# src-d/kmcuda

Measured on AMD Instinct MI355X. Metric: point-assignments/sec per Lloyd iter (8Mx256@1024), higher is better.
Workload: dtype f32

## Files before the change

kmcuda_amd/csrc/engine.cpp:

```cpp
#include "engine.hpp"

#include <math.h>
#include <stdio.h>
#include <stdlib.h>
#include <string.h>

#include <mutex>
#include <vector>

#include "../../include/kmcuda_amd.h"

namespace kmx {

int g_verbosity = 0;

namespace {
std::mutex g_stream_pool_mutex;
std::vector<std::vector<hipStream_t>> g_stream_pool;
}

hipStream_t pooled_stream_acquire(int device) {
  {
    std::lock_guard<std::mutex> lock(g_stream_pool_mutex);
    if ((size_t)device < g_stream_pool.size() && !g_stream_pool[device].empty()) {
// ... 8 lines not shown
}
void pooled_stream_release(int device, hipStream_t s) {
  if (!s) return;
  if (hipStreamSynchronize(s) != hipSuccess) {
    (void)hipGetLastError();
    (void)hipStreamDestroy(s);
    return;
  }
  std::lock_guard<std::mutex> lock(g_stream_pool_mutex);
  if (g_stream_pool.size() <= (size_t)device) g_stream_pool.resize(device + 1);
  if (g_stream_pool[device].size() < 32) g_stream_pool[device].push_back(s);
  else (void)hipStreamDestroy(s);
}

void *Engine::alloc_bytes(size_t bytes) {
  const size_t rounded = (bytes + 255u) & ~(size_t)255u;
  if (rounded <= kSlabMaxItem) {
    if (slab_used_ + rounded > kSlabBytes) {
      void *q = nullptr;
      if (hipMalloc(&q, kSlabBytes) != hipSuccess) return nullptr;
      owned_.push_back(q);
      slab_ = static_cast<char *>(q);
      slab_used_ = 0;
    }
    void *r = slab_ + slab_used_;
    slab_used_ += rounded;
    return r;
  }
  void *q = nullptr;
  if (hipMalloc(&q, bytes) != hipSuccess) return nullptr;
  owned_.push_back(q);
  return q;
}

uint32_t *Engine::pinned_words(size_t n, uint32_t **dev_addr) {
  if (!pinned_) {
    if (hipHostMalloc(reinterpret_cast<void **>(&pinned_), kPinnedWords * sizeof(uint32_t), hipHostMallocCoherent) != hipSuccess) {
      pinned_ = nullptr;
      return nullptr;
    }
    memset(pinned_, 0, kPinnedWords * sizeof(uint32_t));
    void *dp = nullptr;
    if (hipHostGetDevicePointer(&dp, pinned_, 0) != hipSuccess || dp == nullptr) {
      (void)hipHostFree(pinned_);
      pinned_ = nullptr;
      pinned_dev_ = nullptr;
      return nullptr;
    }
    pinned_dev_ = static_cast<uint32_t *>(dp);
  }
  n = (n + 3u) & ~(size_t)3u;
  if (pinned_used_ + n > kPinnedWords) return nullptr;
  uint32_t *r = pinned_ + pinned_used_;
  if (dev_addr) *dev_addr = pinned_dev_ + pinned_used_;
  pinned_used_ += n;
  return r;
}

Engine::~Engine() {
  if (device_ >= 0) (void)hipSetDevice(device_);
  for (auto &s : spans_) { (void)hipEventDestroy(s.a); (void)hipEventDestroy(s.b); }
  for (void *p : owned_) (void)hipFree(p);
  if (pinned_) (void)hipHostFree(pinned_);
  if (side_stream_ && own_side_stream_) pooled_stream_release(device_, side_stream_);
  if (ev_fork_) (void)hipEventDestroy(ev_fork_);
  if (ev_join_) (void)hipEventDestroy(ev_join_);
  for (hipEvent_t e : ev_report_)
    if (e) (void)hipEventDestroy(e);
  if (ev_rows_) (void)hipEventDestroy(ev_rows_);
  if (own_stream_ && stream_) {
    if (blocking_stream_) (void)hipStreamDestroy(stream_);
    else pooled_stream_release(device_, stream_);
  }
}

int Engine::init(int device, uint32_t n_rows, uint32_t D, uint32_t K, int metric, int fp16x2, hipStream_t stream) {
  if (getenv("KMCUDA_AMD_DEBUG")) g_verbosity = atoi(getenv("KMCUDA_AMD_DEBUG"));
  if (const char *f = getenv("KMCUDA_AMD_FILTER")) filter_mode_ = strcmp(f, "f32") == 0 ? 1 : 0;
  if (const char *c = getenv("KMCUDA_AMD_ROW_CACHE")) row_cache_allowed_ = atoi(c) != 0;
  carry_pairs_ = true;
  if (const char *c = getenv("KMCUDA_AMD_CARRY_PAIRS")) carry_pairs_ = atoi(c) != 0;
  if (const char *c = getenv("KMCUDA_AMD_SETTLE")) settle_ = atoi(c) != 0;
  if (const char *c = getenv("KMCUDA_AMD_DUO")) { duo_on_ = atoi(c) != 0; duo_always_ = atoi(c) == 2; }
  if (const char *c = getenv("KMCUDA_AMD_COARSE_MFMA")) coarse_mfma_ = atoi(c) == 32 ? 32u : 16u;
  if (const char *c = getenv("KMCUDA_AMD_WIDE")) wide_ok_ = atoi(c) != 0;
  if (const char *c = getenv("KMCUDA_AMD_GEMM")) wide_ok_ = atoi(c) != 0;
  if (const char *u = getenv("KMCUDA_AMD_UPDATE"))
    ms_.force = strcmp(u, "radix") == 0 ? 1 : (strcmp(u, "sync") == 0 ? 2 : (strcmp(u, "bucket") == 0 ? 3 : 0));
  if (D == 0 || K < 1 || K >= 0x7FFFFFFFu) return kInvalidArguments;
  if (fp16x2) return kInvalidArguments;
  int ndev = 0;
  if (hipGetDeviceCount(&ndev) != hipSuccess || device < 0 || device >= ndev) return kNoSuchDevice;
  KMX_HIP(hipSetDevice(device), kNoSuchDevice);
  device_ = device;
  if (stream == (hipStream_t)(intptr_t)-1) {
    KMX_HIP(hipStreamCreateWithFlags(&stream_, hipStreamDefault), kRuntimeError);
    own_stream_ = true;
    blocking_stream_ = true;
  } else if (stream) {
    stream_ = stream;
  } else {
    stream_ = pooled_stream_acquire(device);
    if (!stream_) return kRuntimeError;
    own_stream_ = true;
  }
  N_ = n_rows; D_ = D; K_ = K; metric_ = metric; fp16x2_ = fp16x2;
  K_pad_ = (K + 31) / 32 * 32;
  Kt_ = (K + 63) / 64 * 64;
  DP_ = lloyd_dp_for(D);
  long wide_min_d = 257;
  if (const char *c = getenv("KMCUDA_AMD_WIDE_MIN_D")) {
    const long d = atol(c);
    if (d > 0) wide_min_d = d;
  }
  if (wide_ok_ && (long)D >= wide_min_d) DP_ = 0;
  eps_ = (float)(1.02 * ((double)D + 12.0) * ldexp(1.0, -24));
  tie_slack_ = metric == 0 ? 0.f : 1e-6f;

  wide_dp_ = (DP_ == 0 && wide_ok_) ? (D + 63) / 64 * 64 : 0;
  const uint32_t dp = DP_ ? DP_ : (wide_dp_ ? wide_dp_ : 8);
  int rc;
  if ((rc = alloc(&csqr_, K))) return rc;
  if ((rc = alloc(&bias_, K_pad_))) return rc;
  if ((rc = alloc(&bias2_, K_pad_))) return rc;
  if ((rc = alloc(&cfil_, (size_t)K_pad_ * dp))) return rc;
  if ((rc = alloc(&ct_, (size_t)D * Kt_))) return rc;
  if ((rc = alloc(&stats_base_, 16))) return rc;
  stats_ = stats_base_;
  if ((rc = alloc(&mu_, dp))) return rc;
  if ((rc = alloc(&finite_, Kt_))) return rc;
  if ((rc = alloc(&flagged_, n_rows))) return rc;
  if ((rc = alloc(&pairs_, 3 * (size_t)n_rows))) return rc;
  if ((rc = alloc(&counters_, 16))) return rc;
  if ((rc = alloc(&keys_tmp_, 2 * (size_t)n_rows))) return rc;
  if ((rc = alloc(&vals_tmp_, 2 * (size_t)n_rows))) return rc;
  if ((rc = alloc(&keys_sorted_, 2 * (size_t)n_rows))) return rc;
  if ((rc = alloc(&rows_sorted_, 2 * (size_t)n_rows))) return rc;
  if ((rc = alloc(&offsets2_, 2 * (size_t)K + 2))) return rc;
  if ((rc = alloc(&move_blocks_, (size_t)n_rows / 1024 + 4))) return rc;
  if ((rc = alloc(&bucket_work_, move_bucket_words(K)))) return rc;
  KMX_HIP(hipMemsetAsync(bucket_work_, 0, move_bucket_words(K) * sizeof(uint32_t), stream_), kRuntimeError);
  bucket_cap_ = move_bucket_cap(n_rows, K);
  if ((rc = alloc(&bucket_rows_, 2 * (size_t)K * bucket_cap_))) return rc;
  KMX_HIP(hipMemsetAsync(stats_base_, 0, 16 * sizeof(uint32_t), stream_), kRuntimeError);
  host_move_count_ = pinned_words(5, &ms_.host_dev);
  if (!host_move_count_) return kMemoryAllocationFailure;
  host_move_count_[2] = 0xFFFFFFFFu;
  host_move_count_[4] = 0xFFFFFFFFu;
  ms_.host = host_move_count_;
  KMX_HIP(hipEventCreateWithFlags(&ev_rows_, hipEventDisableTiming), kRuntimeError);
  sort_temp_bytes_ = sort_temp_bytes(2 * (size_t)n_rows, 2 * K);
  {
    const size_t b2 = sort_temp_bytes(n_rows, K);
    if (b2 > sort_temp_bytes_) sort_temp_bytes_ = b2;
  }
  {
    char *t = nullptr;
    if ((rc = alloc(&t, sort_temp_bytes_ + 16))) return rc;
    sort_temp_ = t;
  }
  host_counters_ = pinned_words(8, nullptr);
  if (!host_counters_) return kMemoryAllocationFailure;
  KMX_HIP(hipMemsetAsync(counters_, 0, 16 * sizeof(uint32_t), stream_), kRuntimeError);
  return kSuccess;
}

// ... 96 lines not shown
  KMX_HIP(hipMemcpy(gfirst_, gfirst.data(), gfirst.size() * sizeof(uint32_t), hipMemcpyHostToDevice), kMemoryCopyError);
  KMX_HIP(hipMemcpy(gsecond_, gsecond.data(), gsecond.size() * sizeof(uint32_t), hipMemcpyHostToDevice), kMemoryCopyError);
  const uint32_t k_pad64 = (K_ + 63u) / 64u * 64u;
  if ((rc = alloc(&groups_, k_pad64))) return rc;
  if (!yy_stats_) {
    if ((rc = alloc(&yy_stats_, 64 * 16))) return rc;
    KMX_HIP(hipMemsetAsync(yy_stats_, 0, 64 * 16 * sizeof(uint32_t), stream_), kRuntimeError);
  }
  if ((rc = alloc(&cperm_, cperm.size()))) return rc;
  if ((rc = alloc(&gstart_, G + 1))) return rc;
  if ((rc = alloc(&pids_, pids.size()))) return rc;
  if ((rc = alloc(&pmeta_, pmeta.size()))) return rc;
  const uint32_t dp = DP_ ? DP_ : 8;
  if ((rc = alloc(&pfil_, (size_t)nslots_ * dp))) return rc;
  if ((rc = alloc(&pbias_, nslots_))) return rc;
  {
    std::vector<uint32_t> gp(k_pad64, 0xFFFFFFFFu);
    for (uint32_t c = 0; c < K_; c++) gp[c] = groups_host[c];
    KMX_HIP(hipMemcpy(groups_, gp.data(), k_pad64 * sizeof(uint32_t), hipMemcpyHostToDevice), kMemoryCopyError);
  }
  KMX_HIP(hipMemcpy(cperm_, cperm.data(), cperm.size() * sizeof(uint32_t), hipMemcpyHostToDevice), kMemoryCopyError);
  KMX_HIP(hipMemcpy(gstart_, gstart.data(), (G + 1) * sizeof(uint32_t), hipMemcpyHostToDevice), kMemoryCopyError);
  KMX_HIP(hipMemcpy(pids_, pids.data(), pids.size() * sizeof(uint32_t), hipMemcpyHostToDevice), kMemoryCopyError);
  KMX_HIP(hipMemcpy(pmeta_, pmeta.data(), pmeta.size() * sizeof(uint32_t), hipMemcpyHostToDevice), kMemoryCopyError);
  return kSuccess;
}

static void fill_yy_args(Engine &e, YyArgs &a, const float *samples, const float *centroids) {
  a.samples = samples; a.centroids = centroids;
  a.len = e.N_; a.D = e.D_; a.DP = e.DP_; a.K = e.K_; a.K_pad = e.K_pad_; a.G = e.G_;
  a.cfil = e.cfil_; a.bias = e.bias_; a.mu = e.mu_; a.stats = e.stats_; a.eps = e.eps_;
  a.groups = e.groups_; a.drifts = nullptr; a.gdrifts = nullptr; a.assignments = nullptr; a.bounds = nullptr;
  a.passed = nullptr; a.counters = e.counters_; a.count_ptr = e.counters_ + 2;
  a.panelhi = nullptr; a.hint = nullptr; a.flag_rows = nullptr; a.gfirst = e.gfirst_; a.gsecond = e.gsecond_;
  a.xcache = nullptr; a.xmeta = nullptr; a.stat_stripes = e.yy_stats_;
  a.pfil = e.pfil_; a.pbias = e.pbias_; a.pids = e.pids_; a.pmeta = e.pmeta_; a.cperm = e.cperm_;
  a.gstart = e.gstart_; a.nslots = e.nslots_;
}

int Engine::yy_init(const float *samples, const float *centroids, const uint32_t *assignments, float *bounds) {
  KMX_HIP(hipSetDevice(device_), kNoSuchDevice);
  if (N_ == 0) return kSuccess;
  if (strict_h2_) {
    KMX_HIP(launch_h2_yy_init(metric_, samples, N_, D_, K_, G_, centroids, assignments, groups_, bounds, stream_),
            kRuntimeError);
    return kSuccess;
  }
  if (DP_ && DP_ <= 256 && !yy_exact_) {
    int rc = prepare_centroids(centroids);
    if (rc) return rc;
    YyArgs a;
    fill_yy_args(*this, a, samples, centroids);
    a.assignments = const_cast<uint32_t *>(assignments);
    a.bounds = bounds;
    KMX_HIP(launch_yy_orig_panel(metric_, centroids, D_, DP_, pids_, nslots_, pfil_, pbias_, stream_), kRuntimeError);
    KMX_HIP(launch_yy_init_lds(metric_, a, stream_), kRuntimeError);
    return kSuccess;
  }
  if (!xt_) {
    int rc = alloc(&xt_, (size_t)N_ * D_);
    if (rc) return rc;
  }
  KMX_HIP(launch_transpose(samples, N_, D_, xt_, stream_), kRuntimeError);
  KMX_HIP(launch_yy_init(metric_, xt_, N_, D_, G_, centroids, assignments, cperm_, gstart_, bounds, stream_),
          kRuntimeError);
  return kSuccess;
}

int Engine::yy_drifts(const float *centroids, float *drifts, float *gdrifts) {
  KMX_HIP(hipSetDevice(device_), kNoSuchDevice);
  if (strict_h2_) {
    KMX_HIP(launch_h2_yy_drifts(metric_, centroids, K_, D_, drifts, stream_), kRuntimeError);
    KMX_HIP(launch_yy_group_max(K_, D_, G_, groups_, drifts, gdrifts, stream_), kRuntimeError);
    return kSuccess;
  }
  KMX_HIP(launch_yy_drifts(metric_, centroids, K_, D_, G_, groups_, drifts, gdrifts, stream_), kRuntimeError);
  return kSuccess;
}

int Engine::yy_filters(const float *samples, const float *centroids, const float *drifts, const float *gdrifts,
                       uint32_t *assignments, uint32_t *assignments_prev, float *bounds, uint32_t *passed) {
  KMX_HIP(hipSetDevice(device_), kNoSuchDevice);
  carry_valid_ = false;
  if (N_ == 0) return kSuccess;
  if (strict_h2_) {
    KMX_HIP(launch_h2_yy_global(metric_, samples, N_, D_, K_, G_, centroids, drifts, gdrifts, assignments,
                                assignments_prev, bounds, passed, counters_, stream_),
            kRuntimeError);
    KMX_HIP(launch_h2_yy_local(metric_, samples, N_, D_, K_, G_, passed, centroids, groups_, drifts, gdrifts,
                               assignments, bounds, counters_, stream_),
            kRuntimeError);
    return kSuccess;
  }
  KMX_HIP(launch_yy_global_filter(metric_, samples, N_, D_, K_, G_, centroids, drifts, gdrifts, assignments,
                                  assignments_prev, bounds, passed, counters_, stream_),
          kRuntimeError);
  if (DP_ && DP_ <= 256 && !yy_exact_) {
    int rc = prepare_centroids(centroids);
    if (rc) return rc;
    YyArgs a;
    fill_yy_args(*this, a, samples, centroids);
    a.drifts = drifts; a.gdrifts = gdrifts; a.assignments = assignments; a.bounds = bounds; a.passed = passed;
    if (yy_hint_ && yy_hint_supported(DP_)) {
      if (!yy_hint_buf_) {
        uint16_t *phi = nullptr;
        if ((rc = alloc(&phi, (size_t)((K_pad_ + 63u) / 64u * 64u) * (DP_ + 2)))) return rc;
        if ((rc = alloc(&yy_flag_rows_, N_))) return rc;
        if ((rc = alloc(&yy_hint_buf_, N_))) return rc;
        yy_panelhi_ = phi;
      }
      KMX_HIP(launch_centroid_panelhi(centroids, K_, D_, K_pad_, DP_, finite_, mu_, bias_, yy_panelhi_, stats_,
                                      stream_),
              kRuntimeError);
      KMX_HIP(hipMemsetAsync(counters_ + 5, 0, sizeof(uint32_t), stream_), kRuntimeError);
      a.panelhi = yy_panelhi_; a.hint = yy_hint_buf_; a.flag_rows = yy_flag_rows_;
      if (row_cache_on_ && row_cache_valid_ && mu_frozen_ && xcache_ && metric_ == 0 && D_ == DP_) {
        a.xcache = xcache_;
        a.xmeta = xmeta_;
      }
      KMX_HIP(launch_yy_hint(metric_, a, stream_), kRuntimeError);
      KMX_HIP(launch_yy_local_hint(metric_, a, stream_), kRuntimeError);
      a.passed = yy_flag_rows_;
      a.count_ptr = counters_ + 5;
    }
    KMX_HIP(launch_yy_local_mfma(metric_, a, stream_), kRuntimeError);
    return kSuccess;
  }
  KMX_HIP(launch_yy_local_filter(metric_, samples, N_, D_, K_, G_, centroids, groups_, drifts, gdrifts, assignments,
                                 bounds, passed, counters_, stream_),
          kRuntimeError);
  return kSuccess;
}

int Engine::lloyd_assign(const float *samples, const float *centroids, uint32_t *assignments,
                         uint32_t *assignments_prev, bool exact_only) {
  KMX_HIP(hipSetDevice(device_), kNoSuchDevice);
  const bool carry_was_valid = carry_valid_;
  carry_valid_ = false;
  if (strict_h2_) {
    if (!h2_sq_) {
      int rc = alloc(&h2_sq_, 2 * (size_t)K_);
      if (rc) return rc;
    }
    span_begin(1);
    KMX_HIP(launch_h2_csqr(metric_, centroids, K_, D_, h2_sq_, stream_), kRuntimeError);
    KMX_HIP(launch_h2_assign(metric_, samples, N_, D_, centroids, K_, h2_sq_, assignments, assignments_prev, counters_,
                             stream_),
            kRuntimeError);
    span_end();
    return kSuccess;
  }
  const bool two_stage = !exact_only && DP_ != 0 && filter_mode_ == 0 && lloyd_filter_f16_supported(D_, DP_);
  const bool want_cache = row_cache_on_ && two_stage && N_ != 0;
  const bool build_cache = want_cache && !row_cache_valid_;
  if (build_cache) mu_frozen_ = false;
  if (!side_stream_) {
    side_stream_ = pooled_stream_acquire(device_);
    if (!side_stream_) return kRuntimeError;
    own_side_stream_ = true;
  }
  if (!ev_fork_) {
    KMX_HIP(hipEventCreateWithFlags(&ev_fork_, hipEventDisableTiming), kRuntimeError);
    KMX_HIP(hipEventCreateWithFlags(&ev_join_, hipEventDisableTiming), kRuntimeError);
  }
  if (two_stage && !panelhi_) {
    uint16_t *phi = nullptr;
    int rc = alloc(&phi, (size_t)((K_pad_ + 63u) / 64u * 64u) * (DP_ + 2));
    if (rc) return rc;
    if (!undecided_ && ((rc = alloc(&undecided_, N_)) || (rc = alloc(&und_thr_, N_)))) return rc;
    if (duo_on_ && !duo_ && alloc(&duo_, 4 * (size_t)N_) != kSuccess) {
      (void)hipGetLastError();
      duo_ = nullptr;
      duo_on_ = false;
    }
    panelhi_ = phi;
  }
  const bool steady = steady_state(exact_only);
  const bool wide_sel = !exact_only && DP_ == 0 && wide_dp_ != 0 && !wide_failed_;
  const bool wide_steady = wide_sel && mu_frozen_ && row_cache_on_ && row_cache_valid_ && N_ != 0 && panelhi_ != nullptr &&
                           wide_rows16_ != nullptr && !strict_h2_;
  const bool prepared = steady && prepared_for_ == centroids;
  prepared_for_ = nullptr;
  bool rows_on_side = false;
  if (steady || wide_steady) {
    KMX_HIP(hipEventRecord(ev_fork_, stream_), kRuntimeError);
    KMX_HIP(hipStreamWaitEvent(side_stream_, ev_fork_, 0), kRuntimeError);
    KMX_HIP(launch_centroid_rows(metric_, centroids, K_, D_, Kt_, csqr_, ct_, side_stream_), kRuntimeError);
    KMX_HIP(hipEventRecord(ev_rows_, side_stream_), kRuntimeError);
    rows_on_side = true;
    if (!prepared) {
      uint32_t *next = stats_;
      stats_ = stats_ == stats_base_ ? stats_base_ + 8 : stats_base_;
      KMX_HIP(launch_centroid_prep_frozen(metric_, centroids, K_, D_, K_pad_, DP_ ? DP_ : wide_dp_, mu_, finite_, bias_,
                                          bias2_, cfil_, panelhi_, stats_, next, counters_ + 1, counters_ + 3, counters_ + 4,
                                          carry_on_ ? drift_ : nullptr, carry_on_ && drift_ ? counters_ + kCarryCursor : nullptr,
                                          stream_),
              kRuntimeError);
      carry_preps_++;
    }
  } else {
    int rc = prepare_centroids(centroids);
    if (rc) return rc;
  }
  LloydArgs a;
  a.samples = samples; a.N = N_; a.D = D_; a.K = K_; a.K_pad = K_pad_; a.DP = DP_; a.Kt = Kt_;
  a.cfil = cfil_; a.bias = bias_; a.mu = mu_; a.ct = ct_; a.csqr = csqr_; a.stats = stats_;
  a.eps = eps_; a.tie_slack = tie_slack_;
  a.assignments = assignments; a.assignments_prev = assignments_prev;
  a.flagged = flagged_; a.pairs = pairs_; a.counters = counters_;
  a.coarse_mfma = coarse_mfma_;
  if (N_ == 0) return kSuccess;
  if (wide_sel) {
    const int rc = lloyd_assign_wide(a, centroids, wide_steady, rows_on_side, carry_was_valid);
    if (rc != kNoSuchDevice + 100) return rc;
  }
  if (exact_only || DP_ == 0 || (DP_ > 256 && filter_mode_ != 0)) {
    span_begin(1);
    const uint32_t grid = N_ < 8192u ? N_ : 8192u;
    KMX_HIP(launch_lloyd_exact(metric_, a, nullptr, nullptr, grid, stream_), kRuntimeError);
    span_end();
    return kSuccess;
  }
  span_begin(0);
  if (two_stage) {
    const void *rows = half_rows_ ? half_rows_ : (const void *)samples;
    const bool half = half_rows_ != nullptr;
    bool duo_listed = false;
    if (!steady)
      KMX_HIP(launch_centroid_panelhi(centroids, K_, D_, K_pad_, DP_, finite_, mu_, bias_, panelhi_, stats_, stream_),
              kRuntimeError);
    if (build_cache) {
      const size_t npad = ((size_t)N_ + 255) / 256 * 256;
      if (!xcache_) {
        uint16_t *xc = nullptr;
        float *xm = nullptr;
        if (alloc(&xc, npad * DP_) == kSuccess && alloc(&xm, npad * 3 + 2) == kSuccess) {
          xcache_ = xc;
          xmeta_ = xm;
        } else {
          (void)hipGetLastError();
          row_cache_on_ = false;
        }
      }
      if (xcache_) {
        KMX_HIP(launch_row_cache(rows, half, N_, D_, DP_, mu_, xcache_, xmeta_, stream_), kRuntimeError);
        row_cache_valid_ = true;
        mu_frozen_ = true;
      }
    }
    const bool cached = row_cache_on_ && row_cache_valid_;
    bool carry = carry_on_ && steady && cached;
    if (carry && carry_policy_.paused()) {
      carry = false;
      if (getenv("KMCUDA_AMD_CARRY_TRACE")) fprintf(stderr, "[carry] paused (%u more)\n", carry_policy_.pause);
    }
    if (carry && !ub_) {
      const bool pairs = carry_pairs_;
      if (alloc(&ub_, N_) != kSuccess || alloc(&lb_, N_) != kSuccess ||
          alloc(&drift_, 2 * (size_t)K_) != kSuccess ||
          (pairs && (alloc(&l3_, N_) != kSuccess || alloc(&p1_, N_) != kSuccess || alloc(&p2_, N_) != kSuccess)) ||
          alloc(&carry_list_, N_) != kSuccess || !(host_carry_ = pinned_words(2, &host_carry_dev_))) {
        (void)hipGetLastError();
        carry_on_ = false;
        ub_ = nullptr;
        l3_ = nullptr;
      } else {
        host_carry_[0] = 0xFFFFFFFFu;
        host_carry_[1] = 0;
        if (const char *v = getenv("KMCUDA_AMD_CARRY_MAX")) carry_policy_.list_max = (float)atof(v);
      }
    }
    span_begin(3);
    duo_listed = duo_on_ && duo_;
    if (duo_listed && !duo_always_) {
      const uint32_t und_prev = host_move_count_[2], duo_prev = host_move_count_[4];
      const uint64_t listed_rows = (und_prev != 0xFFFFFFFFu && duo_prev != 0xFFFFFFFFu) ? (uint64_t)und_prev + duo_prev
                                                                                          : (uint64_t)N_ / 16u;
      duo_listed = listed_rows > 512u * 128u;
    }
    CarryArgs cy_refine;
    if (carry && carry_on_) {
      CarryArgs cy;
      cy.ub = ub_; cy.lb = lb_; cy.host_report = host_carry_dev_; cy.seq = ++carry_seq_;
      cy.angular = metric_ != 0;
      cy.l3 = l3_; cy.p1 = p1_; cy.p2 = p2_;
      cy_refine = cy;
      const bool moved = carry_was_valid && carry_preps_ == 1;
      uint32_t hint = 0xFFFFFFFFu;
      bool listed = false;
      if (moved) {
        const uint32_t last = host_carry_[0], last_seq = host_carry_[1];
        listed = carry_policy_.decide(last, last_seq, carry_seq_, N_);
        if (listed) hint = last;
        KMX_HIP(launch_carry_skip(N_, K_, assignments, assignments_prev, cy, xmeta_, drift_, stats_, tie_slack_,
                                  carry_list_, finite_, pairs_, counters_, !listed, stream_),
                kRuntimeError);
        cy.n_list = counters_ + kCarryCursor;
      }
      if (listed) cy.row_list = carry_list_;
      static const bool trace = getenv("KMCUDA_AMD_CARRY_TRACE") != nullptr;
      if (trace) {
        uint32_t w[8] = {0};
        (void)hipStreamSynchronize(stream_);
        (void)hipMemcpy(w, stats_, sizeof(w), hipMemcpyDeviceToHost);
        float f[8];
        memcpy(f, w, sizeof(f));
        fprintf(stderr, "[carry] stats: max ||c'||^2 %g, max |bias| %g, max ||c||^2 %g, max residual^2 %g, max drift %g, max bias change %g; "
                "stage 2 took %u rows of an earlier pass\n", f[0], f[1], f[2], f[5], f[6], f[7], host_move_count_[2]);
      }
      if (trace)
        fprintf(stderr, "[carry] pass %u: bounds %s, %u preparation(s) since, last reported list %u (pass %u), %s\n",
                carry_seq_, carry_was_valid ? "valid" : "void", carry_preps_, host_carry_[0], host_carry_[1],
                listed ? "listed pass" : (moved ? "whole pass, list counted" : "whole pass"));
      KMX_HIP(launch_lloyd_coarse_carry(a, rows, half, xcache_, xmeta_, panelhi_, undecided_, und_thr_, cy, hint,
                                        duo_listed ? duo_ : nullptr, stream_),
              kRuntimeError);
      carry_valid_ = true;
    } else {
      KMX_HIP(launch_lloyd_coarse(a, rows, half, cached ? xcache_ : nullptr, xmeta_, panelhi_, undecided_, und_thr_,
                                  duo_listed ? duo_ : nullptr, stream_),
              kRuntimeError);
    }
    if (duo_listed) {
      KMX_HIP(hipEventRecord(ev_fork_, stream_), kRuntimeError);
      KMX_HIP(hipStreamWaitEvent(side_stream_, ev_fork_, 0), kRuntimeError);
      KMX_HIP(launch_lloyd_duo(a, duo_, side_stream_, cy_refine.l3 ? &cy_refine : nullptr), kRuntimeError);
      KMX_HIP(hipEventRecord(ev_join_, side_stream_), kRuntimeError);
    }
    carry_preps_ = 0;
    span_end();
    last_undecided_ = host_move_count_[2];
    if (cy_refine.l3) {
      KMX_HIP(launch_lloyd_refine_carry(a, rows, half, panelhi_, undecided_, und_thr_, counters_ + 4, last_undecided_,
                                        cy_refine, stream_),
              kRuntimeError);
    } else {
      KMX_HIP(launch_lloyd_refine(a, rows, half, panelhi_, undecided_, und_thr_, counters_ + 4, last_undecided_,
                                  stream_),
              kRuntimeError);
    }
    if (duo_listed) KMX_HIP(hipStreamWaitEvent(stream_, ev_join_, 0), kRuntimeError);
  } else {
    KMX_HIP(launch_lloyd_filter(a, stream_), kRuntimeError);
  }
  span_end();
  span_begin(1);
  if (settle_ && lloyd_settle_supported(a, centroids)) {
    if (rows_on_side) KMX_HIP(hipStreamWaitEvent(stream_, ev_rows_, 0), kRuntimeError);
    KMX_HIP(launch_lloyd_settle(metric_, a, centroids, stream_), kRuntimeError);
    span_end();
    return kSuccess;
  }
  KMX_HIP(hipEventRecord(ev_fork_, stream_), kRuntimeError);
  KMX_HIP(hipStreamWaitEvent(side_stream_, ev_fork_, 0), kRuntimeError);
  const uint32_t grid = N_ < 4096u ? N_ : 4096u;
  KMX_HIP(launch_lloyd_exact(metric_, a, flagged_, counters_ + 1, grid, side_stream_), kRuntimeError);
  KMX_HIP(hipEventRecord(ev_join_, side_stream_), kRuntimeError);
  if (rows_on_side) KMX_HIP(hipStreamWaitEvent(stream_, ev_rows_, 0), kRuntimeError);
  KMX_HIP(launch_lloyd_pair(metric_, a, centroids, (N_ + 127) / 128 < 2048u ? (N_ + 127) / 128 : 2048u, stream_),
          kRuntimeError);
  KMX_HIP(hipStreamWaitEvent(stream_, ev_join_, 0), kRuntimeError);
  span_end();
  return kSuccess;
}

int Engine::lloyd_assign_wide(const LloydArgs &a0, const float *centroids, bool steady, bool rows_on_side,
                              bool carry_was_valid) {
  constexpr int kNoFilter = kNoSuchDevice + 100;
  LloydArgs a = a0;
  const uint32_t DG = wide_dp_;
  const uint32_t k_pad64 = (K_pad_ + 63u) / 64u * 64u;
  auto no_memory = [&]() {
    (void)hipGetLastError();
    if (g_verbosity > 0) printf("rows wider than 256 features: no memory for the streamed filter's buffers -- exact kernels\n");
    wide_failed_ = true;
    return kNoFilter;
  };
  if (!panelhi_) {
    uint16_t *phi = nullptr;
    if (alloc(&phi, (size_t)k_pad64 * (DG + 2))) return no_memory();
    panelhi_ = phi;
  }
  if (!wide_cont_) {
    if ((!undecided_ && (alloc(&undecided_, N_) || alloc(&und_thr_, N_))) || alloc(&wide_cont_, wide_cont_words(N_))) {
      wide_cont_ = nullptr;
      return no_memory();
    }
  }
  if (!wide_rows16_) {
    uint16_t *xg = nullptr;
    if (alloc(&xg, (size_t)N_ * DG) || alloc(&wide_meta_, ((size_t)N_ + 1) * 4)) return no_memory();
    wide_rows16_ = xg;
  }
  span_begin(0);
  if (!steady)
    KMX_HIP(launch_centroid_panelhi(centroids, K_, D_, K_pad_, DG, finite_, mu_, bias_, panelhi_, stats_, stream_),
            kRuntimeError);
  if (!(row_cache_on_ && row_cache_valid_)) {
    const void *rows = half_rows_ ? half_rows_ : (const void *)a.samples;
    KMX_HIP(launch_row_halves(rows, half_rows_ != nullptr, N_, D_, DG, mu_, wide_rows16_, wide_meta_, stream_), kRuntimeError);
    if (row_cache_on_) {
      row_cache_valid_ = true;
      mu_frozen_ = true;
    }
  }
  bool carry = carry_on_ && steady && DG <= 4096u;
  if (carry && carry_policy_.paused()) {
    carry = false;
    if (getenv("KMCUDA_AMD_CARRY_TRACE")) fprintf(stderr, "[carry] paused (%u more)\n", carry_policy_.pause);
  }
  if (carry && !ub_) {
    if (alloc(&ub_, N_) != kSuccess || alloc(&lb_, N_) != kSuccess || alloc(&drift_, 2 * (size_t)K_) != kSuccess ||
        alloc(&carry_list_, N_) != kSuccess || !(host_carry_ = pinned_words(2, &host_carry_dev_))) {
      (void)hipGetLastError();
      carry_on_ = false;
      ub_ = nullptr;
    } else {
      host_carry_[0] = 0xFFFFFFFFu;
      host_carry_[1] = 0;
      if (const char *v = getenv("KMCUDA_AMD_CARRY_MAX")) carry_policy_.list_max = (float)atof(v);
    }
  }
  span_begin(3);
  if (carry && carry_on_) {
    CarryArgs cy;
    cy.ub = ub_; cy.lb = lb_; cy.host_report = host_carry_dev_; cy.seq = ++carry_seq_;
    cy.angular = metric_ != 0;
    const bool moved = carry_was_valid && carry_preps_ == 1;
    bool listed = false;
    if (moved) {
      const uint32_t last = host_carry_[0], last_seq = host_carry_[1];
      listed = carry_policy_.decide(last, last_seq, carry_seq_, N_);
      KMX_HIP(launch_carry_skip(N_, K_, a.assignments, a.assignments_prev, cy, wide_meta_, drift_, stats_, tie_slack_,
                                carry_list_, finite_, pairs_, counters_, !listed, stream_, DG),
              kRuntimeError);
      cy.n_list = counters_ + kCarryCursor;
    }
    if (listed) cy.row_list = carry_list_;
    if (getenv("KMCUDA_AMD_CARRY_TRACE"))
      fprintf(stderr, "[carry] streamed pass %u: bounds %s, %u preparation(s) since, last reported list %u (pass %u), %s\n",
              carry_seq_, carry_was_valid ? "valid" : "void", carry_preps_, host_carry_[0], host_carry_[1],
              listed ? "listed pass" : (moved ? "whole pass, list counted" : "whole pass"));
    KMX_HIP(launch_lloyd_wide(a, wide_rows16_, wide_meta_, DG, panelhi_, undecided_, und_thr_, wide_cont_, stream_, &cy),
            kRuntimeError);
    carry_valid_ = true;
  } else {
    KMX_HIP(launch_lloyd_wide(a, wide_rows16_, wide_meta_, DG, panelhi_, undecided_, und_thr_, wide_cont_, stream_), kRuntimeError);
  }
  carry_preps_ = 0;
  span_end();
  if (rows_on_side) KMX_HIP(hipStreamWaitEvent(stream_, ev_rows_, 0), kRuntimeError);
  KMX_HIP(launch_wide_contenders(metric_, a, centroids, DG, undecided_, wide_cont_, stream_), kRuntimeError);
  span_end();
  span_begin(1);
  if (settle_ && lloyd_settle_supported(a, centroids)) {
    KMX_HIP(launch_lloyd_settle(metric_, a, centroids, stream_), kRuntimeError);
  } else {
    KMX_HIP(launch_lloyd_pair(metric_, a, centroids, (N_ + 127) / 128 < 2048u ? (N_ + 127) / 128 : 2048u, stream_),
            kRuntimeError);
    const uint32_t grid = N_ < 4096u ? N_ : 4096u;
    KMX_HIP(launch_lloyd_exact(metric_, a, flagged_, counters_ + 1, grid, stream_), kRuntimeError);
  }
  span_end();
  return kSuccess;
}

int Engine::move_deltas(const float *samples, const uint32_t *prev, const uint32_t *cur, double *delta,
                        int32_t *dcount, double *tail) {
  KMX_HIP(hipSetDevice(device_), kNoSuchDevice);
  span_begin(2);
  const MoveWeights mw{weights_, tail ? tail + K_ + 4 : wtail_, win_};
  KMX_HIP(launch_move_deltas(samples, N_, D_, K_, prev, cur, keys_tmp_, vals_tmp_, keys_sorted_, rows_sorted_,
                             offsets2_, sort_temp_, sort_temp_bytes_, bucket_rows_, bucket_cap_, delta, dcount, tail,
                             counters_, move_blocks_, bucket_work_, &ms_, stream_, weights_ ? &mw : nullptr),
          kRuntimeError);
  span_end();
  return kSuccess;
}

int Engine::apply_delta(const double *delta, const int32_t *dcount, const double *dcount_d, float *centroids,
                        uint32_t *ccounts, float stop_threshold, bool report, uint32_t seq) {
  KMX_HIP(hipSetDevice(device_), kNoSuchDevice);
  prepared_for_ = nullptr;
  StopCtl ctl;
  if (stop_threshold >= 0.f || report) {
    if (!dcount_d) return kInvalidArguments;
    int rc = stop_ctl(stop_threshold, report, seq, &ctl);
    if (rc) return rc;
  }
  span_begin(2);
  const double *wtail = weights_ ? (dcount_d ? dcount_d + K_ + 4 : wtail_) : nullptr;
  KMX_HIP(launch_apply_delta(metric_, delta, dcount, dcount_d, K_, D_, centroids, ccounts, ctl, stream_, wtail, cweights_),
          kRuntimeError);
  span_end();
  if (report) KMX_HIP(hipEventRecord(ev_report_[seq & 1u], stream_), kRuntimeError);
  return kSuccess;
}

int Engine::stop_ctl(float stop_threshold, bool report, uint32_t seq, StopCtl *ctl) {
  ctl->threshold = stop_threshold;
  ctl->counters = counters_;
  ctl->seq = seq;
  if (report) {
    if (!host_report_) {
      host_report_ = pinned_words(16, &host_report_dev_);
      if (!host_report_) return kMemoryAllocationFailure;
      memset(host_report_, 0xFF, 16 * sizeof(uint32_t));
      for (hipEvent_t &e : ev_report_) KMX_HIP(hipEventCreateWithFlags(&e, hipEventDisableTiming), kRuntimeError);
    }
    ctl->host_tail = host_report_dev_ + 8 * (seq & 1u);
  }
  return kSuccess;
}

int Engine::stop_report(uint32_t seq, uint32_t *host_out6) {
  KMX_HIP(hipSetDevice(device_), kNoSuchDevice);
  if (!host_report_) return kInvalidArguments;
  KMX_HIP(hipEventSynchronize(ev_report_[seq & 1u]), kRuntimeError);
  const volatile uint32_t *t = host_report_ + 8 * (seq & 1u);
  for (int i = 0; i < 6; i++) host_out6[i] = t[i];
  return host_out6[5] == seq ? kSuccess : kRuntimeError;
}

bool Engine::steady_state(bool exact_only) const {
  const bool two_stage = !exact_only && DP_ != 0 && filter_mode_ == 0 && lloyd_filter_f16_supported(D_, DP_) && !strict_h2_;
  return two_stage && mu_frozen_ && row_cache_on_ && row_cache_valid_ && N_ != 0 && panelhi_ != nullptr;
}

int Engine::apply_prepare(const double *delta, const double *dcount_d, float *centroids, uint32_t *ccounts,
                          float stop_threshold, bool report, uint32_t seq) {
  if (!(metric_ == 0 && steady_state(false) && dcount_d) || weights_) {
    prepared_for_ = nullptr;
    return apply_delta(delta, nullptr, dcount_d, centroids, ccounts, stop_threshold, report, seq);
  }
  KMX_HIP(hipSetDevice(device_), kNoSuchDevice);
  StopCtl ctl;
  if (stop_threshold >= 0.f || report) {
    int rc = stop_ctl(stop_threshold, report, seq, &ctl);
    if (rc) return rc;
  }
  uint32_t *next = stats_;
  stats_ = stats_ == stats_base_ ? stats_base_ + 8 : stats_base_;
  span_begin(2);
  KMX_HIP(launch_apply_prep_frozen(delta, dcount_d, centroids, ccounts, ctl, K_, D_, K_pad_, DP_, mu_, finite_, bias_,
                                   bias2_, cfil_, panelhi_, stats_, next, counters_ + 1, counters_ + 3, counters_ + 4,
                                   carry_on_ ? drift_ : nullptr, carry_on_ && drift_ ? counters_ + kCarryCursor : nullptr,
                                   stream_),
          kRuntimeError);
  carry_preps_++;
  span_end();
  if (report) KMX_HIP(hipEventRecord(ev_report_[seq & 1u], stream_), kRuntimeError);
  prepared_for_ = centroids;
  return kSuccess;
}

int Engine::carry_stats(unsigned long long *rows_spared, uint32_t *last_list) {
  KMX_HIP(hipSetDevice(device_), kNoSuchDevice);
// ... 317 lines not shown
```

kmcuda_amd/csrc/engine.hpp:

```cpp
#pragma once
#include <hip/hip_runtime.h>
#include <stdint.h>

#include <vector>

#include "kernels.hpp"

namespace kmx {

enum Result {
  kSuccess = 0, kInvalidArguments, kNoSuchDevice, kMemoryAllocationFailure, kRuntimeError, kMemoryCopyError
};

#define KMX_HIP(call, ret)                                                                   \
  do {                                                                                       \
    hipError_t e__ = (call);                                                                 \
    if (e__ != hipSuccess) {                                                                 \
      if (kmx::g_verbosity > 0)                                                              \
        printf("%s:%d -> %s (%s)\n", __FILE__, __LINE__, hipGetErrorString(e__), #call);     \
      return ret;                                                                            \
    }                                                                                        \
  } while (0)

extern int g_verbosity;
// ... 38 lines not shown
        hopeless = 0;
        backoff = 4;
        episode_list = 0;
      }
    }
    return listed;
  }
};

class Engine {
 public:
  Engine() = default;
  ~Engine();
  Engine(const Engine &) = delete;
  Engine &operator=(const Engine &) = delete;

  int init(int device, uint32_t n_rows, uint32_t D, uint32_t K, int metric, int fp16x2, hipStream_t stream);

  int lloyd_assign(const float *samples, const float *centroids, uint32_t *assignments,
                   uint32_t *assignments_prev, bool exact_only);
  int move_deltas(const float *samples, const uint32_t *prev, const uint32_t *cur, double *delta, int32_t *dcount,
                  double *tail);
  int apply_delta(const double *delta, const int32_t *dcount, const double *dcount_d, float *centroids,
                  uint32_t *ccounts, float stop_threshold = -1.f, bool report = false, uint32_t seq = 0);
  int apply_prepare(const double *delta, const double *dcount_d, float *centroids, uint32_t *ccounts,
                    float stop_threshold = -1.f, bool report = false, uint32_t seq = 0);
  int set_weights(const float *weights);
  const float *weights_ = nullptr;
  double weight_total_ = 0.0;
  double *cweights_ = nullptr;
  double *wtail_ = nullptr;
  double *win_ = nullptr;
  double *wcheck_ = nullptr;
  size_t reduce_len() const { return (size_t)K_ * D_ + K_ + 4 + (weights_ ? (size_t)K_ + 1 : 0); }
  bool steady_state(bool exact_only) const;
  int stop_ctl(float stop_threshold, bool report, uint32_t seq, StopCtl *ctl);
  const float *prepared_for_ = nullptr;
  int stop_clear();
  int stop_report(uint32_t seq, uint32_t *host_out6);
  int adjust_exact(const float *samples, const uint32_t *prev, const uint32_t *cur, float *centroids,
                   uint32_t *ccounts);
  int prepare_centroids(const float *centroids);
  int yy_configure(uint32_t G, const uint32_t *groups_host);
  int yy_init(const float *samples, const float *centroids, const uint32_t *assignments, float *bounds);
  int yy_drifts(const float *centroids, float *drifts, float *gdrifts);
  int yy_filters(const float *samples, const float *centroids, const float *drifts, const float *gdrifts,
                 uint32_t *assignments, uint32_t *assignments_prev, float *bounds, uint32_t *passed);
  int counters_read(uint32_t *host4);
  int counters_reset(int which);
  int sync();

  template <typename T>
  int alloc(T **p, size_t count) {
    void *q = alloc_bytes(count ? count * sizeof(T) : sizeof(T));
    if (!q) return kMemoryAllocationFailure;
    *p = static_cast<T *>(q);
    return kSuccess;
  }
  void *alloc_bytes(size_t bytes);
  uint32_t *pinned_words(size_t n, uint32_t **dev_addr);

  int device_ = -1;
  hipStream_t stream_ = nullptr;
  bool own_stream_ = false, blocking_stream_ = false;
  hipStream_t side_stream_ = nullptr;
  bool own_side_stream_ = false;
  hipEvent_t ev_fork_ = nullptr, ev_join_ = nullptr;
  hipEvent_t ev_rows_ = nullptr;
  uint32_t N_ = 0, D_ = 0, K_ = 0, K_pad_ = 0, Kt_ = 0, DP_ = 0;
  int metric_ = 0, fp16x2_ = 0;
  bool strict_h2_ = false;
  float *h2_sq_ = nullptr;
  float eps_ = 0, tie_slack_ = 0;

  float *csqr_ = nullptr, *bias_ = nullptr, *bias2_ = nullptr, *cfil_ = nullptr, *ct_ = nullptr, *mu_ = nullptr;
  uint32_t *finite_ = nullptr;
  const void *half_rows_ = nullptr;
  void *panelhi_ = nullptr;
  uint32_t *undecided_ = nullptr;
  float *und_thr_ = nullptr;
  uint32_t *duo_ = nullptr;
  bool duo_on_ = true;
  bool duo_always_ = false;
  uint32_t coarse_mfma_ = 16;
  int filter_mode_ = 0;
  bool settle_ = true;
  uint32_t wide_dp_ = 0;
  bool wide_ok_ = true;
  bool wide_failed_ = false;
  void *wide_rows16_ = nullptr;
  float *wide_meta_ = nullptr;
  uint32_t *wide_cont_ = nullptr;
  int lloyd_assign_wide(const LloydArgs &a, const float *centroids, bool steady, bool rows_on_side, bool carry_was_valid);
  bool row_cache_allowed_ = true;
  bool row_cache_on_ = false, row_cache_valid_ = false, mu_frozen_ = false;
  void *xcache_ = nullptr;
  float *xmeta_ = nullptr;
  bool carry_on_ = false;
  bool carry_valid_ = false;
  uint32_t carry_preps_ = 0;
  uint32_t carry_seq_ = 0;
  CarryPolicy carry_policy_;
  float *ub_ = nullptr, *lb_ = nullptr, *drift_ = nullptr;
  bool carry_pairs_ = true;
  float *l3_ = nullptr;
  uint32_t *p1_ = nullptr, *p2_ = nullptr;
  uint32_t *carry_list_ = nullptr;
  uint32_t *host_carry_ = nullptr, *host_carry_dev_ = nullptr;
  bool carry_usable() const;
  int carry_stats(unsigned long long *rows_spared, uint32_t *last_list);
  int carry_pair_stats(unsigned long long *rows_paired);
  int duo_rows(uint32_t *rows);
  uint32_t *stats_base_ = nullptr, *stats_ = nullptr, *flagged_ = nullptr, *pairs_ = nullptr, *counters_ = nullptr;
  uint32_t *keys_tmp_ = nullptr, *vals_tmp_ = nullptr, *keys_sorted_ = nullptr, *rows_sorted_ = nullptr,
           *offsets2_ = nullptr, *move_blocks_ = nullptr, *bucket_work_ = nullptr, *bucket_rows_ = nullptr;
  uint32_t bucket_cap_ = 0;
  uint32_t last_undecided_ = 0xFFFFFFFFu;
  MoveState ms_;
  uint32_t *host_move_count_ = nullptr;
  void *sort_temp_ = nullptr;
  size_t sort_temp_bytes_ = 0;
  uint32_t G_ = 0, nslots_ = 0;
  bool yy_exact_ = false;
  bool yy_hint_ = true;
  uint32_t *gfirst_ = nullptr, *gsecond_ = nullptr, *yy_flag_rows_ = nullptr;
  float *yy_hint_buf_ = nullptr;
  void *yy_panelhi_ = nullptr;
  int yy_hint_stats(uint32_t *host6);
  uint32_t *groups_ = nullptr, *cperm_ = nullptr, *gstart_ = nullptr, *pids_ = nullptr, *pmeta_ = nullptr;
  float *pfil_ = nullptr, *pbias_ = nullptr, *xt_ = nullptr;
  float *exact_work_ = nullptr;
  uint32_t *host_counters_ = nullptr;
  uint32_t *host_report_ = nullptr;
  uint32_t *host_report_dev_ = nullptr;
  hipEvent_t ev_report_[2] = {nullptr, nullptr};
  uint32_t *yy_stats_ = nullptr;

  bool profile_ = false;
  double filter_ms_ = 0, exact_ms_ = 0, update_ms_ = 0, coarse_ms_ = 0;
  uint32_t filter_launches_ = 0;
  struct Span { hipEvent_t a, b; int kind; };
  std::vector<Span> spans_;
  std::vector<size_t> open_spans_;
  void span_begin(int kind);
  void span_end();
  void profile_collect();
  void profile_reset();

 private:
  std::vector<void *> owned_;
  static constexpr size_t kSlabBytes = 4u << 20, kSlabMaxItem = 512u << 10;
  char *slab_ = nullptr;
  size_t slab_used_ = kSlabBytes;
  static constexpr size_t kPinnedWords = 64;
  uint32_t *pinned_ = nullptr, *pinned_dev_ = nullptr;
  size_t pinned_used_ = 0;
};

}
```

kmcuda_amd/csrc/filter_common.hpp:

```cpp
#pragma once
#include <hip/hip_runtime.h>
#include <stdint.h>

namespace kmx {

__device__ __forceinline__ bool commit_row(uint32_t s, uint32_t nearest, uint32_t *__restrict__ assignments,
                                           uint32_t *__restrict__ assignments_prev) {
  const uint32_t old = assignments[s];
  assignments_prev[s] = old;
  if (old != nearest) {
    assignments[s] = nearest;
    return true;
  }
  return false;
}


struct ClampLimits {
  float hi, lo;
};
__device__ __forceinline__ ClampLimits clamp_limits(bool angular, float xm, float exm, float ehalf) {
  ClampLimits l;
  if (!angular) {
    l.hi = INFINITY;
    l.lo = -INFINITY;
    return l;
  }
  const float m = (ehalf + exm) * 1.001f + 2.0e-6f + 3.0e-7f * fabsf(xm);
  l.hi = (1.0f - m) - xm;
  l.lo = (m - 1.0f) - xm;
  return l;
}
__device__ __forceinline__ float dot_error(int n, float mass) { return 6.1e-8f * (float)(n + 8) * mass; }

template <typename T>
__device__ __forceinline__ void row_dot_mu(const T *__restrict__ xr, const float *__restrict__ mu, uint32_t f0,
                                           uint32_t f1, float &dot, float &mass) {
  float d = 0.f, m = 0.f;
#pragma unroll 4
  for (uint32_t f = f0; f < f1; f++) {
    const float x = (float)xr[f], u = mu[f];
    d = fmaf(x, u, d);
    m = fmaf(fabsf(x), fabsf(u), m);
  }
  dot = d;
  mass = m;
}

__device__ __forceinline__ void filter_finish(float v1, float v2, float v3, uint32_t c1, uint32_t c2, int h, int lane,
                                              uint32_t s, uint32_t N, uint32_t K, bool insane, float thr,
                                              ClampLimits lim, uint32_t *__restrict__ assignments,
                                              uint32_t *__restrict__ assignments_prev,
                                              uint32_t *__restrict__ flagged, uint32_t *__restrict__ pairs,
                                              uint32_t *__restrict__ counters) {
  auto decode = [&](uint32_t code, int half) -> uint32_t {
    if (code == 0xFFFFFFFFu) return 0xFFFFFFFFu;
    const uint32_t r = code & 15u;
    return (code >> 4) * 32u + (r & 3u) + 8u * (r >> 2) + 4u * half;
  };
  uint32_t i1 = decode(c1, h), i2 = decode(c2, h);
  {
    const float pv1 = __shfl_xor(v1, 32), pv2 = __shfl_xor(v2, 32), pv3 = __shfl_xor(v3, 32);
    const uint32_t pi1 = __shfl_xor(i1, 32), pi2 = __shfl_xor(i2, 32);
    auto insert = [&](float v, uint32_t idx) {
      const bool g1 = v > v1, g2 = v > v2, g3 = v > v3;
      v3 = g2 ? v2 : (g3 ? v : v3);
      i2 = g1 ? i1 : (g2 ? idx : i2);
      v2 = g1 ? v1 : (g2 ? v : v2);
      i1 = g1 ? idx : i1;
      v1 = g1 ? v : v1;
    };
    insert(pv1, pi1);
    insert(pv2, pi2);
    insert(pv3, 0xFFFFFFFFu);
  }
  const bool certain = insane || (((v1 - v2) > thr) && (v2 < lim.hi) && (v1 > lim.lo));
  const bool two = !certain && ((v1 - v3) > thr) && (v3 < lim.hi) && (v1 > lim.lo) && i2 != 0xFFFFFFFFu;
  const bool mine = (h == 0) && (s < N);
  const bool commit_now = mine && certain;
  const bool pair_now = mine && two;
  const bool flag_now = mine && !certain && !two;
  bool changed = false;
  if (commit_now) changed = commit_row(s, insane ? K : i1, assignments, assignments_prev);
  const unsigned long long cm = __ballot(changed);
  const unsigned long long pm = __ballot(pair_now);
  const unsigned long long fm = __ballot(flag_now);
  if (lane == 0 && cm) atomicAdd(&counters[0], (uint32_t)__popcll(cm));
  if (pm) {
    uint32_t base = 0;
    if (lane == 0) base = atomicAdd(&counters[3], (uint32_t)__popcll(pm));
    base = __shfl(base, 0);
    if (pair_now) {
      const uint32_t slot = base + (uint32_t)__popcll(pm & ((1ull << lane) - 1ull));
      pairs[3 * (size_t)slot + 0] = s;
      pairs[3 * (size_t)slot + 1] = i1;
      pairs[3 * (size_t)slot + 2] = i2;
    }
  }
  if (fm) {
// ... 9 lines not shown
```

kmcuda_amd/csrc/kernels.hpp:

```cpp
#pragma once
#include <hip/hip_runtime.h>
#include <stdint.h>

namespace kmx {

struct LloydArgs {
  const float *samples;
  uint32_t N, D, K;
  uint32_t K_pad;
  uint32_t DP;
  uint32_t Kt;
  const float *cfil;
  const float *bias;
  const float *mu;
  const float *ct;
  const float *csqr;
  const uint32_t *stats;
  float eps;
  float tie_slack;
  uint32_t *assignments, *assignments_prev;
  uint32_t *flagged;
  uint32_t *pairs;
  uint32_t *counters;
  uint32_t coarse_mfma = 16;
};
constexpr uint32_t kWaveRowGridMax = 1u << 20;
inline uint32_t wave_row_grid(uint32_t n_rows) {
  const uint32_t g = (n_rows + 3u) / 4u;
  return g < kWaveRowGridMax ? (g ? g : 1u) : kWaveRowGridMax;
}
constexpr uint32_t kStopFlag = 8;
constexpr uint32_t kCarryCursor = 9, kCarrySkipped = 10;
constexpr uint32_t kCarryPaired = 12;
constexpr uint32_t kDuoCount = 14;
struct CarryArgs {
  float *ub = nullptr, *lb = nullptr;
  const uint32_t *row_list = nullptr;
  const uint32_t *n_list = nullptr;
  uint32_t *host_report = nullptr;
  uint32_t seq = 0;
  int angular = 0;
  float *l3 = nullptr;
  uint32_t *p1 = nullptr, *p2 = nullptr;
};
struct StopCtl {
  float threshold = -1.f;
  uint32_t *counters = nullptr;
  uint32_t *host_tail = nullptr;
  uint32_t seq = 0;
};

uint32_t filter_dp_for(uint32_t D);
uint32_t lloyd_dp_for(uint32_t D);
hipError_t launch_centroid_prep(int metric, const float *centroids, uint32_t K, uint32_t D, uint32_t K_pad,
                                uint32_t DP, uint32_t Kt, float *csqr, float *bias, float *bias2, float *cfil,
                                float *ct, float *mu, bool freeze_mu, uint32_t *finite, uint32_t *stats, uint32_t *zero_a,
                                uint32_t *zero_b, uint32_t *zero_c, hipStream_t st);
hipError_t launch_lloyd_filter(const LloydArgs &a, hipStream_t st);
hipError_t launch_lloyd_pair(int metric, const LloydArgs &a, const float *centroids, uint32_t grid, hipStream_t st);
hipError_t launch_lloyd_exact(int metric, const LloydArgs &a, const uint32_t *rows, const uint32_t *nrows,
                              uint32_t grid, hipStream_t st);
bool lloyd_settle_supported(const LloydArgs &a, const float *centroids);
hipError_t launch_lloyd_settle(int metric, const LloydArgs &a, const float *centroids, hipStream_t st);

bool lloyd_filter_f16_supported(uint32_t D, uint32_t DP);
hipError_t launch_centroid_panelhi(const float *centroids, uint32_t K, uint32_t D, uint32_t K_pad, uint32_t DP,
                                   const uint32_t *finite, const float *mu, const float *bias, void *panelhi,
                                   uint32_t *stats, hipStream_t st);
hipError_t launch_centroid_prep_frozen(int metric, const float *centroids, uint32_t K, uint32_t D, uint32_t K_pad,
                                       uint32_t DP, const float *mu, uint32_t *finite, float *bias, float *bias2,
                                       float *cfil, void *panelhi, uint32_t *stats, uint32_t *stats_next,
                                       uint32_t *zero_a, uint32_t *zero_b, uint32_t *zero_c,
                                       float *drift ,
                                       uint32_t *zero_d , hipStream_t st);
hipError_t launch_apply_prep_frozen(const double *delta, const double *dcount_d, float *centroids, uint32_t *ccounts,
                                    const StopCtl &stop, uint32_t K, uint32_t D, uint32_t K_pad, uint32_t DP,
                                    const float *mu, uint32_t *finite, float *bias, float *bias2, float *cfil,
                                    void *panelhi, uint32_t *stats, uint32_t *stats_next, uint32_t *zero_a,
                                    uint32_t *zero_b, uint32_t *zero_c, float *drift, uint32_t *zero_d, hipStream_t st);
hipError_t launch_lloyd_coarse_carry(const LloydArgs &a, const void *rows, bool half_rows, const void *xcache,
                                     const float *xmeta, const void *panelhi, uint32_t *undecided, float *und_thr,
                                     const CarryArgs &cy, uint32_t rows_hint, uint32_t *duo, hipStream_t st);
hipError_t launch_carry_skip(uint32_t N, uint32_t K, const uint32_t *assignments, uint32_t *assignments_prev,
                             const CarryArgs &cy, const float *xmeta, const float *drift, const uint32_t *stats,
                             float tie_slack, uint32_t *row_list, const uint32_t *finite, uint32_t *pairs,
                             uint32_t *counters, bool probe, hipStream_t st, uint32_t wide_dg = 0);
hipError_t launch_centroid_rows(int metric, const float *centroids, uint32_t K, uint32_t D, uint32_t Kt, float *csqr,
                                float *ct, hipStream_t st);
hipError_t launch_lloyd_coarse(const LloydArgs &a, const void *rows, bool half_rows, const void *xcache,
                               const float *xmeta, const void *panelhi, uint32_t *undecided, float *und_thr,
                               uint32_t *duo, hipStream_t st);
hipError_t launch_lloyd_duo(const LloydArgs &a, const uint32_t *duo, hipStream_t st, const CarryArgs *cy = nullptr);
hipError_t launch_lloyd_refine(const LloydArgs &a, const void *rows, bool half_rows, const void *panelhi,
                               const uint32_t *row_list, const float *thr_list, const uint32_t *n_list,
                               uint32_t rows_hint , hipStream_t st);
hipError_t launch_lloyd_refine_carry(const LloydArgs &a, const void *rows, bool half_rows, const void *panelhi,
                                     const uint32_t *row_list, const float *thr_list, const uint32_t *n_list,
                                     uint32_t rows_hint, const CarryArgs &cy, hipStream_t st);
hipError_t launch_row_cache(const void *rows, bool half_rows, uint32_t N, uint32_t D, uint32_t DP, const float *mu,
                            void *xcache, float *xmeta, hipStream_t st);

hipError_t launch_row_halves(const void *rows, bool half_rows, uint32_t N, uint32_t D, uint32_t DG, const float *mu,
                             void *xg, float *meta , hipStream_t st);
size_t wide_cont_words(uint32_t N);
hipError_t launch_lloyd_wide(const LloydArgs &a, const void *xg, const float *meta, uint32_t DG ,
                             const void *panelhi, uint32_t *undecided, float *und_thr, uint32_t *und_cont, hipStream_t st,
                             const CarryArgs *cy = nullptr);
hipError_t launch_wide_contenders(int metric, const LloydArgs &a, const float *centroids, uint32_t DG,
                                  const uint32_t *und_rows, const uint32_t *und_cont, hipStream_t st);

size_t sort_temp_bytes(size_t n, uint32_t max_key);
uint32_t move_bucket_stride(uint32_t K);
size_t move_bucket_words(uint32_t K);
uint32_t move_bucket_cap(uint32_t N, uint32_t K);
hipError_t launch_inverse_assignments(const uint32_t *assignments, uint32_t N, uint32_t K, uint32_t *keys_tmp,
                                      uint32_t *vals_tmp, uint32_t *keys_sorted, uint32_t *inv,
                                      uint32_t *offsets, void *temp, size_t temp_bytes, hipStream_t st);
struct MoveState {
  uint32_t *host = nullptr;
  uint32_t *host_dev = nullptr;
  uint32_t last_events = 0xFFFFFFFFu;
  int force = 0;
  uint32_t n_radix = 0, n_direct = 0;
};
struct MoveWeights {
  const float *weights;
  double *dweight;
  double *win;
};
hipError_t launch_move_deltas(const float *samples, uint32_t N, uint32_t D, uint32_t K, const uint32_t *prev,
                              const uint32_t *cur, uint32_t *keys_tmp, uint32_t *vals_tmp, uint32_t *keys_sorted,
                              uint32_t *rows_sorted, uint32_t *offsets2, void *temp, size_t temp_bytes,
                              uint32_t *bucket_rows, uint32_t cap, double *delta, int32_t *dcount ,
                              double *tail ,
                              const uint32_t *counters, uint32_t *blockoff, uint32_t *bucket_work, MoveState *ms,
                              hipStream_t st, const MoveWeights *mw = nullptr);
hipError_t launch_adjust_exact(int metric, const float *samples, uint32_t N, uint32_t D, uint32_t K,
                               const uint32_t *prev, const uint32_t *cur, uint32_t *keys_tmp, uint32_t *vals_tmp,
                               uint32_t *keys_sorted, uint32_t *rows_sorted, uint32_t *offsets2, void *temp,
                               size_t temp_bytes, float *work, float *centroids, uint32_t *ccounts, hipStream_t st);
hipError_t launch_apply_delta(int metric, const double *delta, const int32_t *dcount ,
                              const double *dcount_d , uint32_t K, uint32_t D,
                              float *centroids, uint32_t *ccounts, const StopCtl &stop, hipStream_t st,
                              const double *wtail = nullptr ,
                              double *cweights = nullptr );
size_t weights_check_doubles();
hipError_t launch_weights_check(const float *weights, uint32_t N, double *work, hipStream_t st);
hipError_t launch_sum_buffers(double *const *bufs_dev, uint32_t nbuf, size_t len, hipStream_t st);

hipError_t preload_update_code();
hipError_t preload_lloyd_f16_code();
hipError_t preload_lloyd_code();
hipError_t preload_lloyd_carry_code();
hipError_t preload_lloyd_duo_code();
hipError_t launch_gather_rows(const float *samples, const uint32_t *idx, uint32_t K, uint32_t D, float *out, hipStream_t st);
hipError_t launch_kmpp_step(int metric, const float *samples, uint32_t N, uint32_t D, const float *centroid,
                            uint32_t cc, float *dists, hipStream_t st);
struct KmppOutlierBuf {
  uint32_t *ecut = nullptr;
  void *outl = nullptr;
  uint32_t *outl_count = nullptr;
};
size_t kmpp_outlier_bytes();
size_t kmpp_totals_bytes();
hipError_t launch_kmpp_step2(int metric, const float *samples, uint32_t N, uint32_t D, const float *centroid,
                             uint32_t cc, float *dists, void *block_stats, double *bpre, void *totals,
                             const uint32_t *fail, const KmppOutlierBuf &out, hipStream_t st,
                             const float *weights = nullptr, float *terms = nullptr);
hipError_t launch_kmpp_weigh(const float *dists, const float *weights, uint32_t N, float *terms, const uint32_t *fail,
                             hipStream_t st);
constexpr int kKmppMaxShards = 16;
struct KmppShardPtrs {
  const float *dists;
  const double *bpre;
  void *totals;
  const float *samples;
  float *centroids;
  uint32_t *fail;
  uint32_t offset, length;
  KmppOutlierBuf out;
};
hipError_t launch_kmpp_choose(const KmppShardPtrs *shards, uint32_t nshards, uint32_t N, double choice, uint32_t log2n,
                              uint32_t step, uint32_t D, hipStream_t st);
hipError_t launch_kmpp_cache(const float *samples, uint32_t N, uint32_t D, uint32_t DP, double *part, float *mu,
                             void *xs8, float *meta, uint32_t *stats, hipStream_t st);
hipError_t launch_kmpp_step_filtered(int metric, const float *samples, uint32_t N, uint32_t D, uint32_t DP,
                                     const void *xs8, const float *meta, const float *mu, uint32_t *stats,
                                     uint32_t *list, const float *centroid, uint32_t cc, float *dists,
                                     void *block_stats, double *bpre, void *totals, const uint32_t *fail,
                                     const KmppOutlierBuf &out, hipStream_t st, const float *weights = nullptr,
                                     float *terms = nullptr);
size_t kmpp_block_stat_bytes(uint32_t N);
size_t kmpp_blocks(uint32_t N);
size_t kmpp_prefix_doubles(uint32_t N);
hipError_t launch_afk_qdist(int metric, const float *samples, uint32_t N, uint32_t D, const float *c1, float *dists,
                            hipStream_t st);
hipError_t launch_afk_q(float *q, uint32_t N, float dsum, hipStream_t st);
hipError_t launch_afk_draws(unsigned long long seed, unsigned long long offset, uint32_t threads, uint32_t n, uint32_t *out,
                            hipStream_t st);
hipError_t launch_afk_random_step(uint32_t m, uint64_t seed, uint64_t seq, const float *q, uint32_t N,
                                  uint32_t *choices, float *rand_a, hipStream_t st);
hipError_t launch_afk_min_dist(int metric, uint32_t m, uint32_t k, const float *samples, uint32_t D,
                               const uint32_t *choices, const float *centroids, float *min_dists, hipStream_t st);
hipError_t launch_member_distances(int metric, const float *samples, uint32_t N, uint32_t D,
                                   const float *centroids, const uint32_t *assignments, uint32_t K,
                                   float *dists, hipStream_t st);

hipError_t launch_yy_init(int metric, const float *xt, uint32_t len, uint32_t D, uint32_t G, const float *centroids,
                          const uint32_t *assignments, const uint32_t *cperm, const uint32_t *gstart, float *bounds,
                          hipStream_t st);
hipError_t launch_yy_group_max(uint32_t K, uint32_t D, uint32_t G, const uint32_t *groups, const float *drifts,
                               float *gdrifts, hipStream_t st);
hipError_t launch_yy_drifts(int metric, const float *centroids, uint32_t K, uint32_t D, uint32_t G,
                            const uint32_t *groups, float *drifts, float *gdrifts, hipStream_t st);

struct YyArgs {
  const float *samples;
  const float *centroids;
  uint32_t len, D, DP, K, K_pad, G;
// ... 145 lines not shown
```

kmcuda_amd/csrc/lloyd.hip:

```cpp
#include "exact.hpp"
#include "filter_common.hpp"
#include "kernels.hpp"

namespace kmx {

typedef float f32x16 __attribute__((ext_vector_type(16)));
typedef float f32x4 __attribute__((ext_vector_type(4)));

template <int METRIC>
__global__ void centroid_rows_kernel(const float *__restrict__ centroids, uint32_t K, uint32_t D, uint32_t Kt,
                                     float *__restrict__ csqr, float *__restrict__ ct,
                                     uint32_t *__restrict__ finite, uint32_t *__restrict__ stats) {
  const uint32_t c = blockIdx.x * blockDim.x + threadIdx.x;
  float plain_max = 0.f;
  if (c < Kt && c < K) {
    const float *row = centroids + (size_t)c * D;
    float ssqr = 0.f, corr = 0.f, plain = 0.f;
    uint32_t f = 0;
    if ((D & 3u) == 0 && (((uintptr_t)row) & 15u) == 0) {
      for (; f < D; f += 4) {
        const float4 v4 = *reinterpret_cast<const float4 *>(row + f);
        const float vs[4] = {v4.x, v4.y, v4.z, v4.w};
#pragma unroll
        for (int q = 0; q < 4; q++) {
// ... 228 lines not shown
  uint32_t c1 = 0xFFFFFFFFu, c2 = 0xFFFFFFFFu;

  for (uint32_t t = 0; t < ntiles; t++) {
    const int buf = t & 1;
    if (t + 1 < ntiles) stage_load(t + 1);

    f32x16 acc;
    {
      const float *bb = bias_ptr(buf) + 4 * h;
#pragma unroll
      for (int g = 0; g < 4; g++) {
        const f32x4 b4 = *reinterpret_cast<const f32x4 *>(bb + 8 * g);
        acc[4 * g + 0] = b4.x;
        acc[4 * g + 1] = b4.y;
        acc[4 * g + 2] = b4.z;
        acc[4 * g + 3] = b4.w;
      }
    }
    const float *arow = tile_ptr(buf) + col * LDW + h * NK;
    constexpr int NG = NK / 8 > 0 ? NK / 8 : 1;
    if constexpr (NK >= 16) {
      f32x4 c0 = *reinterpret_cast<const f32x4 *>(arow), c1 = *reinterpret_cast<const f32x4 *>(arow + 4);
#pragma unroll
      for (int g = 0; g < NG; g++) {
        f32x4 n0 = c0, n1 = c1;
        if (g + 1 < NG) {
          n0 = *reinterpret_cast<const f32x4 *>(arow + 8 * (g + 1));
          n1 = *reinterpret_cast<const f32x4 *>(arow + 8 * (g + 1) + 4);
        }
        __builtin_amdgcn_sched_barrier(0);
        acc = __builtin_amdgcn_mfma_f32_32x32x2f32(c0.x, xb[8 * g + 0], acc, 0, 0, 0);
        acc = __builtin_amdgcn_mfma_f32_32x32x2f32(c0.y, xb[8 * g + 1], acc, 0, 0, 0);
        acc = __builtin_amdgcn_mfma_f32_32x32x2f32(c0.z, xb[8 * g + 2], acc, 0, 0, 0);
        acc = __builtin_amdgcn_mfma_f32_32x32x2f32(c0.w, xb[8 * g + 3], acc, 0, 0, 0);
        acc = __builtin_amdgcn_mfma_f32_32x32x2f32(c1.x, xb[8 * g + 4], acc, 0, 0, 0);
        acc = __builtin_amdgcn_mfma_f32_32x32x2f32(c1.y, xb[8 * g + 5], acc, 0, 0, 0);
        acc = __builtin_amdgcn_mfma_f32_32x32x2f32(c1.z, xb[8 * g + 6], acc, 0, 0, 0);
        acc = __builtin_amdgcn_mfma_f32_32x32x2f32(c1.w, xb[8 * g + 7], acc, 0, 0, 0);
        __builtin_amdgcn_sched_barrier(0);
        c0 = n0;
        c1 = n1;
      }
    } else {
#pragma unroll
      for (int j = 0; j < NK / 4; j++) {
        const f32x4 a4 = *reinterpret_cast<const f32x4 *>(arow + 4 * j);
        acc = __builtin_amdgcn_mfma_f32_32x32x2f32(a4.x, xb[4 * j + 0], acc, 0, 0, 0);
        acc = __builtin_amdgcn_mfma_f32_32x32x2f32(a4.y, xb[4 * j + 1], acc, 0, 0, 0);
        acc = __builtin_amdgcn_mfma_f32_32x32x2f32(a4.z, xb[4 * j + 2], acc, 0, 0, 0);
        acc = __builtin_amdgcn_mfma_f32_32x32x2f32(a4.w, xb[4 * j + 3], acc, 0, 0, 0);
      }
    }
#pragma unroll
    for (int r = 0; r < 16; r++) {
      const float v = acc[r];
      const uint32_t code = t * 16u + r;
      const bool g1 = v > v1, g2 = v > v2;
      v3 = __builtin_amdgcn_fmed3f(v2, v3, v);
      c2 = g1 ? c1 : (g2 ? code : c2);
      v2 = __builtin_amdgcn_fmed3f(v1, v2, v);
      c1 = g1 ? code : c1;
      v1 = fmaxf(v1, v);
    }
    if (t + 1 < ntiles) stage_store(buf ^ 1);
    __syncthreads();
  }

  const float cmaxc = sqrtf(__uint_as_float(stats[0])) * 1.000001f;
  const float bmaxc = __uint_as_float(stats[1]);
  const float cmaxo = sqrtf(__uint_as_float(stats[2])) * 1.000001f;
  const float xn = sqrtf(xn2) * 1.0001f, xo = sqrtf(xo2) * 1.0001f;
  const float e_mfma = 2.0f * eps * (xn * cmaxc + bmaxc);
  const float e_ref = 5.9604645e-8f * (12.0f * xo * cmaxo + 4.0f * cmaxo * cmaxo);
  const float thr = 2.0f * (e_mfma + e_ref) * 1.001f + tie_slack;
  const ClampLimits lim = clamp_limits(tie_slack > 0.f, xm, dot_error(DP, xma), 0.5f * thr);
  filter_finish(v1, v2, v3, c1, c2, h, lane, s, N, K, insane, thr, lim, assignments, assignments_prev, flagged, pairs,
                counters);
}

template <int METRIC>
__global__ __launch_bounds__(128) void lloyd_pair_kernel(
    const float *__restrict__ samples, uint32_t D, const float *__restrict__ centroids,
    const float *__restrict__ csqr, const uint32_t *__restrict__ pairs, const uint32_t *__restrict__ npairs,
    uint32_t *__restrict__ assignments, uint32_t *__restrict__ assignments_prev, uint32_t *__restrict__ counters) {
  const uint32_t total = *npairs;
  for (uint32_t pi = blockIdx.x * blockDim.x + threadIdx.x; pi < total; pi += gridDim.x * blockDim.x) {
    const uint32_t s = pairs[3 * (size_t)pi], ia = pairs[3 * (size_t)pi + 1], ib = pairs[3 * (size_t)pi + 2];
    const uint32_t lo = ia < ib ? ia : ib, hi = ia < ib ? ib : ia;
    const float *x = samples + (size_t)s * D;
    const float *ca = centroids + (size_t)lo * D, *cb = centroids + (size_t)hi * D;
    float acc[4] = {0.f, 0.f, 0.f, 0.f}, corr[4] = {0.f, 0.f, 0.f, 0.f};
    uint32_t f = 0;
    const bool aligned16 = ((((uintptr_t)x) | ((uintptr_t)ca) | ((uintptr_t)cb)) & 15u) == 0;
    if ((D & 7u) == 0 && aligned16) {
      auto load8 = [&](uint32_t f0, float4 (&xv)[2], float4 (&av)[2], float4 (&bv)[2]) {
#pragma unroll
        for (int t = 0; t < 2; t++) {
          xv[t] = *reinterpret_cast<const float4 *>(x + f0 + 4 * t);
          av[t] = *reinterpret_cast<const float4 *>(ca + f0 + 4 * t);
          bv[t] = *reinterpret_cast<const float4 *>(cb + f0 + 4 * t);
        }
      };
      auto fold8 = [&](const float4 (&xv)[2], const float4 (&av)[2], const float4 (&bv)[2]) {
#pragma unroll
        for (int t = 0; t < 2; t++) {
          const float xs[4] = {xv[t].x, xv[t].y, xv[t].z, xv[t].w}, as[4] = {av[t].x, av[t].y, av[t].z, av[t].w},
                      bs[4] = {bv[t].x, bv[t].y, bv[t].z, bv[t].w};
#pragma unroll
          for (int q = 0; q < 4; q++) {
            const float cv[4] = {as[q], bs[q], 0.f, 0.f};
            float y[4];
            fma_rd4(xs[q], cv, corr, y);
            kahan_fold(y[0], acc[0], corr[0]);
            kahan_fold(y[1], acc[1], corr[1]);
          }
        }
      };
      float4 x0[2], a0[2], b0[2], x1[2], a1[2], b1[2];
      load8(0, x0, a0, b0);
      for (; f + 16 <= D; f += 16) {
        load8(f + 8, x1, a1, b1);
        fold8(x0, a0, b0);
        if (f + 24 <= D) load8(f + 16, x0, a0, b0);
        fold8(x1, a1, b1);
      }
      if (f + 8 <= D) {
        fold8(x0, a0, b0);
        f += 8;
      }
    } else if ((D & 3u) == 0 && aligned16) {
      for (; f < D; f += 4) {
        const float4 xv = *reinterpret_cast<const float4 *>(x + f);
        const float4 av = *reinterpret_cast<const float4 *>(ca + f), bv = *reinterpret_cast<const float4 *>(cb + f);
        const float xs[4] = {xv.x, xv.y, xv.z, xv.w}, as[4] = {av.x, av.y, av.z, av.w}, bs[4] = {bv.x, bv.y, bv.z, bv.w};
#pragma unroll
        for (int q = 0; q < 4; q++) {
          const float cv[4] = {as[q], bs[q], 0.f, 0.f};
          float y[4];
          fma_rd4(xs[q], cv, corr, y);
          kahan_fold(y[0], acc[0], corr[0]);
          kahan_fold(y[1], acc[1], corr[1]);
        }
      }
    }
    for (; f < D; f++) {
      const float cv[4] = {ca[f], cb[f], 0.f, 0.f};
      float y[4];
      fma_rd4(x[f], cv, corr, y);
      kahan_fold(y[0], acc[0], corr[0]);
      kahan_fold(y[1], acc[1], corr[1]);
    }
    const float da = lloyd_distance<METRIC>(csqr[lo], acc[0]);
    const float db = lloyd_distance<METRIC>(csqr[hi], acc[1]);
    float min_dist = 3.402823466e+38f;
    uint32_t nearest = 0xFFFFFFFFu;
    if (da < min_dist) { min_dist = da; nearest = lo; }
    if (db < min_dist) { min_dist = db; nearest = hi; }
    if (nearest != 0xFFFFFFFFu && commit_row(s, nearest, assignments, assignments_prev)) atomicAdd(&counters[0], 1u);
  }
}

template <int METRIC>
__global__ __launch_bounds__(256) void lloyd_exact_kernel(
    const float *__restrict__ samples, uint32_t N, uint32_t D, const float *__restrict__ ct,
    const float *__restrict__ csqr, uint32_t K, uint32_t Kt, const uint32_t *__restrict__ rows,
    const uint32_t *__restrict__ nrows, uint32_t *__restrict__ assignments,
    uint32_t *__restrict__ assignments_prev, uint32_t *__restrict__ counters) {
  constexpr int CH = 4;
  __shared__ float sh_dist[4];
  __shared__ uint32_t sh_idx[4];
  const int lane = threadIdx.x & 63, wave = threadIdx.x >> 6;
  if (counters[kStopFlag] != 0u) return;
  const uint32_t total = rows ? *nrows : N;
  for (uint32_t ri = blockIdx.x; ri < total; ri += gridDim.x) {
    const uint32_t s = rows ? rows[ri] : ri;
    const float *x = samples + (size_t)s * D;
    const bool insane = (x[0] != x[0]);
    float min_dist = 3.402823466e+38f;
    uint32_t nearest = 0xFFFFFFFFu;
    if (!insane) {
      for (uint32_t cbase = wave * 64 * CH; cbase < K; cbase += 4 * 64 * CH) {
        float acc[CH], corr[CH];
#pragma unroll
        for (int j = 0; j < CH; j++) { acc[j] = 0.f; corr[j] = 0.f; }
        const float *cp[CH];
#pragma unroll
        for (int j = 0; j < CH; j++) cp[j] = ct + ((cbase + 64 * j + lane < Kt) ? cbase + 64 * j + lane : (uint32_t)lane);
        uint32_t f = 0;
        constexpr int GF = 8;
        auto load_group = [&](uint32_t f0, float (&xf)[GF], float (&cv)[GF][CH]) {
#pragma unroll
          for (int q = 0; q < GF; q++) {
            xf[q] = x[f0 + q];
#pragma unroll
            for (int j = 0; j < CH; j++) cv[q][j] = cp[j][(size_t)(f0 + q) * Kt];
          }
        };
        auto fold_group = [&](const float (&xf)[GF], float (&cv)[GF][CH]) {
#pragma unroll
          for (int q = 0; q < GF; q++) {
            float y[CH];
            fma_rd4(xf[q], cv[q], corr, y);
#pragma unroll
            for (int j = 0; j < CH; j++) kahan_fold(y[j], acc[j], corr[j]);
          }
        };
        if (D >= GF) {
          float xa[GF], ca[GF][CH], xb[GF], cb[GF][CH];
          load_group(0, xa, ca);
          for (; f + 2 * GF <= D; f += 2 * GF) {
            load_group(f + GF, xb, cb);
            fold_group(xa, ca);
            if (f + 3 * GF <= D) load_group(f + 2 * GF, xa, ca);
            fold_group(xb, cb);
          }
          if (f + GF <= D) {
            fold_group(xa, ca);
            f += GF;
          }
        }
        for (; f < D; f++) {
          const float xf = x[f];
          float cv[CH], y[CH];
#pragma unroll
          for (int j = 0; j < CH; j++) cv[j] = cp[j][(size_t)f * Kt];
          fma_rd4(xf, cv, corr, y);
#pragma unroll
          for (int j = 0; j < CH; j++) kahan_fold(y[j], acc[j], corr[j]);
        }
#pragma unroll
        for (int j = 0; j < CH; j++) {
          const uint32_t c = cbase + 64 * j + lane;
          if (c < K) {
            const float dist = lloyd_distance<METRIC>(csqr[c], acc[j]);
            if (dist < min_dist) { min_dist = dist; nearest = c; }
          }
        }
      }
#pragma unroll
      for (int off = 32; off > 0; off >>= 1) {
        const float od = __shfl_xor(min_dist, off);
        const uint32_t oi = __shfl_xor(nearest, off);
        const bool take = (oi != 0xFFFFFFFFu) &&
                          (nearest == 0xFFFFFFFFu || od < min_dist || (od == min_dist && oi < nearest));
        if (take) { min_dist = od; nearest = oi; }
      }
    }
    if (lane == 0) {
      sh_dist[wave] = min_dist;
      sh_idx[wave] = nearest;
    }
    __syncthreads();
    if (threadIdx.x == 0) {
      for (int w = 1; w < 4; w++) {
        const float od = sh_dist[w];
        const uint32_t oi = sh_idx[w];
        const bool take = (oi != 0xFFFFFFFFu) &&
                          (nearest == 0xFFFFFFFFu || od < min_dist || (od == min_dist && oi < nearest));
        if (take) { min_dist = od; nearest = oi; }
      }
      if (nearest == 0xFFFFFFFFu && insane) nearest = K;
      if (nearest != 0xFFFFFFFFu) {
        if (commit_row(s, nearest, assignments, assignments_prev)) atomicAdd(&counters[0], 1u);
      }
    }
    __syncthreads();
  }
}

constexpr int kSettleFC = 64;
constexpr int kSettleLD = kSettleFC + 4;
constexpr int kSettleRows = 96;
constexpr uint32_t kSettlePairBlocks = 256, kSettleScanBlocks = 256;
constexpr size_t kSettleLds = (size_t)4 * (kSettleRows * kSettleLD + kSettleRows) * sizeof(float);

template <int METRIC>
__global__ __launch_bounds__(256) void lloyd_settle_kernel(
    const float *__restrict__ samples, uint32_t N, uint32_t D, const float *__restrict__ centroids,
    const float *__restrict__ ct, const float *__restrict__ csqr, uint32_t K, uint32_t Kt,
    const uint32_t *__restrict__ pairs, const uint32_t *__restrict__ npairs, const uint32_t *__restrict__ flagged,
    const uint32_t *__restrict__ nflagged, uint32_t *__restrict__ assignments,
    uint32_t *__restrict__ assignments_prev, uint32_t *__restrict__ counters) {
  extern __shared__ __attribute__((aligned(16))) float settle_lds[];
  const int lane = threadIdx.x & 63, wave = threadIdx.x >> 6;
  if (blockIdx.x < kSettlePairBlocks) {
    const uint32_t total = *npairs;
    float *tile = settle_lds + (size_t)wave * (kSettleRows * kSettleLD + kSettleRows);
    uint32_t *rowid = reinterpret_cast<uint32_t *>(tile + kSettleRows * kSettleLD);
    const uint32_t nch = (D + kSettleFC - 1) / kSettleFC;
    for (uint32_t base0 = blockIdx.x * 128u; base0 < total; base0 += kSettlePairBlocks * 128u) {
      const uint32_t p = base0 + wave * 32u + (lane & 31);
      const bool live = p < total;
      uint32_t s = 0, lo = 0, hi = 0;
      if (live) {
        s = pairs[3 * (size_t)p];
        const uint32_t ia = pairs[3 * (size_t)p + 1], ib = pairs[3 * (size_t)p + 2];
        lo = ia < ib ? ia : ib;
        hi = ia < ib ? ib : ia;
      }
      const uint32_t mine = lane < 32 ? lo : hi;
      __syncthreads();
      if (lane < 32) rowid[lane] = s;
      rowid[32 + lane] = mine;
      __syncthreads();
      float4 stage[kSettleRows / 4];
      auto fetch = [&](uint32_t ch) {
#pragma unroll
        for (int it = 0; it < kSettleRows / 4; it++) {
          const uint32_t r = it * 4 + (lane >> 4), f = ch * kSettleFC + (lane & 15) * 4;
          const float *src = (r < 32 ? samples : centroids) + (size_t)rowid[r] * D + f;
          stage[it] = f < D ? *reinterpret_cast<const float4 *>(src) : make_float4(0.f, 0.f, 0.f, 0.f);
        }
      };
      float acc = 0.f, corr = 0.f;
      fetch(0);
      for (uint32_t ch = 0; ch < nch; ch++) {
        __syncthreads();
#pragma unroll
        for (int it = 0; it < kSettleRows / 4; it++) {
          const uint32_t r = it * 4 + (lane >> 4);
          *reinterpret_cast<float4 *>(&tile[r * kSettleLD + (lane & 15) * 4]) = stage[it];
        }
        __syncthreads();
        if (ch + 1 < nch) fetch(ch + 1);
        const uint32_t fmax = D - ch * kSettleFC < (uint32_t)kSettleFC ? D - ch * kSettleFC : (uint32_t)kSettleFC;
        const float *xr = tile + (lane & 31) * kSettleLD, *cr = tile + (32 + lane) * kSettleLD;
        for (uint32_t c4 = 0; c4 * 4 < fmax; c4++) {
          const float4 xv = *reinterpret_cast<const float4 *>(xr + c4 * 4);
          const float4 cv = *reinterpret_cast<const float4 *>(cr + c4 * 4);
          kahan_fold(fma_rd(xv.x, cv.x, corr), acc, corr);
          kahan_fold(fma_rd(xv.y, cv.y, corr), acc, corr);
          kahan_fold(fma_rd(xv.z, cv.z, corr), acc, corr);
          kahan_fold(fma_rd(xv.w, cv.w, corr), acc, corr);
        }
      }
      const float dist = lloyd_distance<METRIC>(csqr[mine], acc);
      const float db = __shfl(dist, (lane & 31) + 32);
      bool changed = false;
      if (live && lane < 32) {
        float min_dist = 3.402823466e+38f;
        uint32_t nearest = 0xFFFFFFFFu;
        if (dist < min_dist) { min_dist = dist; nearest = lo; }
        if (db < min_dist) { min_dist = db; nearest = hi; }
        if (nearest != 0xFFFFFFFFu) changed = commit_row(s, nearest, assignments, assignments_prev);
      }
      const unsigned long long cm = __ballot(changed);
      if (lane == 0 && cm) atomicAdd(&counters[0], (uint32_t)__popcll(cm));
    }
    return;
  }
  constexpr int CH = 4, GF = 8, NB = 4;
  float *sh_dist = settle_lds;
  uint32_t *sh_idx = reinterpret_cast<uint32_t *>(settle_lds + 4);
  const uint32_t total = *nflagged;
  for (uint32_t ri = blockIdx.x - kSettlePairBlocks; ri < total; ri += gridDim.x - kSettlePairBlocks) {
    const uint32_t s = flagged[ri];
    const float *x = samples + (size_t)s * D;
    const bool insane = (x[0] != x[0]);
    float min_dist = 3.402823466e+38f;
    uint32_t nearest = 0xFFFFFFFFu;
    if (!insane) {
      for (uint32_t cbase = wave * 64 * CH; cbase < K; cbase += 4 * 64 * CH) {
        float acc[CH], corr[CH];
#pragma unroll
        for (int j = 0; j < CH; j++) { acc[j] = 0.f; corr[j] = 0.f; }
        const float *cp[CH];
#pragma unroll
        for (int j = 0; j < CH; j++) cp[j] = ct + ((cbase + 64 * j + lane < Kt) ? cbase + 64 * j + lane : (uint32_t)lane);
        float xg[NB][GF], cg[NB][GF][CH];
        const uint32_t ngroups = D / GF;
        auto load_group = [&](uint32_t g, float (&xf)[GF], float (&cv)[GF][CH]) {
#pragma unroll
          for (int q = 0; q < GF; q++) {
            xf[q] = x[g * GF + q];
#pragma unroll
            for (int j = 0; j < CH; j++) cv[q][j] = cp[j][(size_t)(g * GF + q) * Kt];
          }
        };
        auto fold_group = [&](const float (&xf)[GF], float (&cv)[GF][CH]) {
#pragma unroll
          for (int q = 0; q < GF; q++) {
            float y[CH];
            fma_rd4(xf[q], cv[q], corr, y);
#pragma unroll
            for (int j = 0; j < CH; j++) kahan_fold(y[j], acc[j], corr[j]);
          }
        };
#pragma unroll
        for (int b = 0; b < NB - 1; b++)
          if ((uint32_t)b < ngroups) load_group(b, xg[b], cg[b]);
        for (uint32_t g0 = 0; g0 < ngroups; g0 += NB) {
#pragma unroll
          for (int b = 0; b < NB; b++) {
            const uint32_t g = g0 + b;
            if (g < ngroups) {
              if (g + NB - 1 < ngroups) load_group(g + NB - 1, xg[(b + NB - 1) % NB], cg[(b + NB - 1) % NB]);
              fold_group(xg[b], cg[b]);
            }
          }
        }
        for (uint32_t f = ngroups * GF; f < D; f++) {
          const float xf = x[f];
          float cv[CH], y[CH];
#pragma unroll
          for (int j = 0; j < CH; j++) cv[j] = cp[j][(size_t)f * Kt];
          fma_rd4(xf, cv, corr, y);
#pragma unroll
          for (int j = 0; j < CH; j++) kahan_fold(y[j], acc[j], corr[j]);
        }
#pragma unroll
        for (int j = 0; j < CH; j++) {
          const uint32_t c = cbase + 64 * j + lane;
          if (c < K) {
            const float dist = lloyd_distance<METRIC>(csqr[c], acc[j]);
            if (dist < min_dist) { min_dist = dist; nearest = c; }
          }
        }
      }
#pragma unroll
      for (int off = 32; off > 0; off >>= 1) {
        const float od = __shfl_xor(min_dist, off);
        const uint32_t oi = __shfl_xor(nearest, off);
        const bool take = (oi != 0xFFFFFFFFu) &&
                          (nearest == 0xFFFFFFFFu || od < min_dist || (od == min_dist && oi < nearest));
        if (take) { min_dist = od; nearest = oi; }
      }
    }
    if (lane == 0) {
      sh_dist[wave] = min_dist;
      sh_idx[wave] = nearest;
    }
    __syncthreads();
    if (threadIdx.x == 0) {
      for (int w = 1; w < 4; w++) {
        const float od = sh_dist[w];
        const uint32_t oi = sh_idx[w];
        const bool take = (oi != 0xFFFFFFFFu) &&
                          (nearest == 0xFFFFFFFFu || od < min_dist || (od == min_dist && oi < nearest));
        if (take) { min_dist = od; nearest = oi; }
      }
      if (nearest == 0xFFFFFFFFu && insane) nearest = K;
      if (nearest != 0xFFFFFFFFu) {
        if (commit_row(s, nearest, assignments, assignments_prev)) atomicAdd(&counters[0], 1u);
      }
    }
    __syncthreads();
  }
}

bool lloyd_settle_supported(const LloydArgs &a, const float *centroids) {
  return (a.D & 3u) == 0 && (((uintptr_t)a.samples | (uintptr_t)centroids) & 15u) == 0;
}

hipError_t launch_lloyd_settle(int metric, const LloydArgs &a, const float *centroids, hipStream_t st) {
  static bool attr_set[2] = {false, false};
  const void *fn = metric == 0 ? (const void *)lloyd_settle_kernel<0> : (const void *)lloyd_settle_kernel<1>;
  hipError_t e = hipFuncSetAttribute(fn, hipFuncAttributeMaxDynamicSharedMemorySize, (int)kSettleLds);
  if (e != hipSuccess) return e;
  (void)attr_set;
  const dim3 grid(kSettlePairBlocks + kSettleScanBlocks);
  if (metric == 0)
    hipLaunchKernelGGL((lloyd_settle_kernel<0>), grid, dim3(256), kSettleLds, st, a.samples, a.N, a.D, centroids, a.ct,
                       a.csqr, a.K, a.Kt, a.pairs, a.counters + 3, a.flagged, a.counters + 1, a.assignments,
                       a.assignments_prev, a.counters);
  else
    hipLaunchKernelGGL((lloyd_settle_kernel<1>), grid, dim3(256), kSettleLds, st, a.samples, a.N, a.D, centroids, a.ct,
                       a.csqr, a.K, a.Kt, a.pairs, a.counters + 3, a.flagged, a.counters + 1, a.assignments,
                       a.assignments_prev, a.counters);
  return hipGetLastError();
}

uint32_t filter_dp_for(uint32_t D);
uint32_t lloyd_dp_for(uint32_t D) { return (D > 256 && D <= 512) ? 512u : filter_dp_for(D); }

uint32_t filter_dp_for(uint32_t D) {
  static const uint32_t sizes[] = {8, 16, 32, 64, 128, 256};
  for (uint32_t v : sizes)
    if (D <= v) return v;
  return 0;
}

template <int DP>
static hipError_t launch_filter_dp(const LloydArgs &a, hipStream_t st) {
  const bool fast = (a.D == (uint32_t)DP);
  const size_t lds_bytes = (2 * 32 * (DP + 4) + 64) * sizeof(float);
  const uint32_t grid = (a.N + 127) / 128;
  if (fast) {
    hipLaunchKernelGGL((lloyd_filter_kernel<DP, true>), dim3(grid), dim3(256), lds_bytes, st, a.samples, a.N,
                       a.D, a.cfil, a.bias, a.mu, a.K_pad, a.K, a.stats, a.eps, a.tie_slack, a.assignments,
                       a.assignments_prev, a.flagged, a.pairs, a.counters);
  } else {
    hipLaunchKernelGGL((lloyd_filter_kernel<DP, false>), dim3(grid), dim3(256), lds_bytes, st, a.samples, a.N,
                       a.D, a.cfil, a.bias, a.mu, a.K_pad, a.K, a.stats, a.eps, a.tie_slack, a.assignments,
                       a.assignments_prev, a.flagged, a.pairs, a.counters);
  }
  return hipGetLastError();
}

hipError_t launch_lloyd_filter(const LloydArgs &a, hipStream_t st) {
  switch (a.DP) {
    case 8: return launch_filter_dp<8>(a, st);
    case 16: return launch_filter_dp<16>(a, st);
    case 32: return launch_filter_dp<32>(a, st);
    case 64: return launch_filter_dp<64>(a, st);
    case 128: return launch_filter_dp<128>(a, st);
    case 256: return launch_filter_dp<256>(a, st);
    default: return hipErrorInvalidValue;
  }
}

hipError_t launch_centroid_prep(int metric, const float *centroids, uint32_t K, uint32_t D, uint32_t K_pad,
                                uint32_t DP, uint32_t Kt, float *csqr, float *bias, float *bias2, float *cfil,
                                float *ct, float *mu, bool freeze_mu, uint32_t *finite, uint32_t *stats,
                                uint32_t *zero_a, uint32_t *zero_b, uint32_t *zero_c, hipStream_t st) {
  const dim3 block(64);
  if (metric == 0)
    hipLaunchKernelGGL((centroid_rows_kernel<0>), dim3((Kt + 63) / 64), block, 0, st, centroids, K, D, Kt, csqr, ct,
                       finite, stats);
  else
    hipLaunchKernelGGL((centroid_rows_kernel<1>), dim3((Kt + 63) / 64), block, 0, st, centroids, K, D, Kt, csqr, ct,
                       finite, stats);
  hipLaunchKernelGGL(centroid_mean_kernel, dim3((DP + 63) / 64), dim3(1024), 0, st, centroids, K, D, DP, finite, mu,
                     freeze_mu, zero_a, zero_b, zero_c);
  if (metric == 0)
    hipLaunchKernelGGL((centroid_panel_kernel<0>), dim3((K_pad + 15) / 16), dim3(256), 0, st, centroids, K, D, K_pad, DP,
                       finite, mu, bias, bias2, cfil, stats);
  else
    hipLaunchKernelGGL((centroid_panel_kernel<1>), dim3((K_pad + 15) / 16), dim3(256), 0, st, centroids, K, D, K_pad, DP,
                       finite, mu, bias, bias2, cfil, stats);
  return hipGetLastError();
}

hipError_t launch_centroid_rows(int metric, const float *centroids, uint32_t K, uint32_t D, uint32_t Kt, float *csqr,
                                float *ct, hipStream_t st) {
  if (metric == 0)
    hipLaunchKernelGGL((centroid_rows_kernel<0>), dim3((Kt + 63) / 64), dim3(64), 0, st, centroids, K, D, Kt, csqr, ct,
                       (uint32_t *)nullptr, (uint32_t *)nullptr);
  else
    hipLaunchKernelGGL((centroid_rows_kernel<1>), dim3((Kt + 63) / 64), dim3(64), 0, st, centroids, K, D, Kt, csqr, ct,
                       (uint32_t *)nullptr, (uint32_t *)nullptr);
  return hipGetLastError();
}

hipError_t launch_lloyd_pair(int metric, const LloydArgs &a, const float *centroids, uint32_t grid, hipStream_t st) {
  if (grid == 0) return hipSuccess;
  if (metric == 0)
    hipLaunchKernelGGL((lloyd_pair_kernel<0>), dim3(grid), dim3(128), 0, st, a.samples, a.D, centroids, a.csqr,
                       a.pairs, a.counters + 3, a.assignments, a.assignments_prev, a.counters);
  else
    hipLaunchKernelGGL((lloyd_pair_kernel<1>), dim3(grid), dim3(128), 0, st, a.samples, a.D, centroids, a.csqr,
                       a.pairs, a.counters + 3, a.assignments, a.assignments_prev, a.counters);
  return hipGetLastError();
}

hipError_t launch_lloyd_exact(int metric, const LloydArgs &a, const uint32_t *rows, const uint32_t *nrows,
                              uint32_t grid, hipStream_t st) {
  if (grid == 0) return hipSuccess;
  if (metric == 0)
    hipLaunchKernelGGL((lloyd_exact_kernel<0>), dim3(grid), dim3(256), 0, st, a.samples, a.N, a.D, a.ct, a.csqr,
                       a.K, a.Kt, rows, nrows, a.assignments, a.assignments_prev, a.counters);
  else
    hipLaunchKernelGGL((lloyd_exact_kernel<1>), dim3(grid), dim3(256), 0, st, a.samples, a.N, a.D, a.ct, a.csqr,
                       a.K, a.Kt, rows, nrows, a.assignments, a.assignments_prev, a.counters);
  return hipGetLastError();
}

hipError_t preload_lloyd_code() {
  hipFuncAttributes at;
  return hipFuncGetAttributes(&at, reinterpret_cast<const void *>(&centroid_rows_kernel<0>));
}

}
```

kmcuda_amd/csrc/lloyd_carry.hip:

```cpp
#include <cstdlib>

#include "lloyd_coarse.hpp"
#include "lloyd_refine.hpp"

namespace kmx {

constexpr int kSkipRowsPerThread = 8, kSkipBlock = 256;
template <bool WIDE>
__global__ __launch_bounds__(kSkipBlock) void carry_skip_kernel(
    uint32_t N, uint32_t K, const uint32_t *__restrict__ assignments, uint32_t *__restrict__ assignments_prev,
    CarryArgs cy, const float2 *__restrict__ xmeta, const float *__restrict__ drift, const uint32_t *__restrict__ stats,
    float tie_slack, uint32_t *__restrict__ row_list, const uint32_t *__restrict__ finite, uint32_t *__restrict__ pairs,
    uint32_t *__restrict__ counters, int probe, float terms) {
  if (counters[kStopFlag] != 0u) return;
  float *__restrict__ ub = cy.ub, *__restrict__ lb = cy.lb, *__restrict__ l3 = cy.l3;
  const int angular = cy.angular;
  const float maxdrift = __uint_as_float(stats[6]);
  const float cmaxo = sqrtf(__uint_as_float(stats[2])) * 1.000001f;
  const float4 *__restrict__ wmeta = reinterpret_cast<const float4 *>(xmeta);
  const float mu_norm = WIDE ? wmeta[N].x : reinterpret_cast<const float *>(xmeta)[2 * (((size_t)N + 255) / 256 * 256)];
  const float u = 5.9604645e-8f;
  const float maxdb = __uint_as_float(stats[7]);
  const float cmaxc = sqrtf(__uint_as_float(stats[0])) * 1.000001f;
  const float eb = 4.0f * terms * u * mu_norm * (cmaxc + maxdrift);
// ... 59 lines not shown
                if (pair && !probe) {
                  ub[s] = up;
                  l3[s] = lp;
                }
              }
            }
          }
        }
      }
    }
    const bool list = live && !keep && !pair;
    const unsigned long long lm = __ballot(list), pm = __ballot(pair);
    if (list) listbits |= 1u << it;
    if (pair) pairbits |= 1u << it;
    if (lane == 0) {
      wave_cnt[it][wave] = (uint32_t)__popcll(lm);
      pair_cnt[it][wave] = (uint32_t)__popcll(pm);
    }
  }
  __syncthreads();
  if (threadIdx.x == 0) {
    uint32_t t = 0, tp = 0;
#pragma unroll
    for (int it = 0; it < kSkipRowsPerThread; it++)
#pragma unroll
      for (int w = 0; w < kSkipBlock / 64; w++) {
        const uint32_t c = wave_cnt[it][w], cp = pair_cnt[it][w];
        wave_cnt[it][w] = t;
        pair_cnt[it][w] = tp;
        t += c;
        tp += cp;
      }
    blk_base = t ? atomicAdd(&counters[kCarryCursor], t) : 0u;
    blk_pair_base = (tp && !probe) ? atomicAdd(&counters[3], tp) : 0u;
  }
  if (probe) return;
  __syncthreads();
#pragma unroll
  for (int it = 0; it < kSkipRowsPerThread; it++) {
    const bool list = (listbits >> it) & 1u, pair = (pairbits >> it) & 1u;
    const unsigned long long lm = __ballot(list), pm = __ballot(pair);
    const unsigned long long below = (1ull << lane) - 1ull;
    const uint32_t s = base + it * kSkipBlock + threadIdx.x;
    if (list) row_list[blk_base + wave_cnt[it][wave] + (uint32_t)__popcll(lm & below)] = s;
    if (pair) {
      const size_t at = blk_pair_base + pair_cnt[it][wave] + (uint32_t)__popcll(pm & below);
      pairs[3 * at + 0] = s;
      pairs[3 * at + 1] = cy.p1[s];
      pairs[3 * at + 2] = cy.p2[s];
    }
  }
}

hipError_t launch_carry_skip(uint32_t N, uint32_t K, const uint32_t *assignments, uint32_t *assignments_prev,
                             const CarryArgs &cy, const float *xmeta, const float *drift, const uint32_t *stats,
                             float tie_slack, uint32_t *row_list, const uint32_t *finite, uint32_t *pairs,
                             uint32_t *counters, bool probe, hipStream_t st, uint32_t wide_dg) {
  const uint32_t chunk = kSkipBlock * kSkipRowsPerThread;
  if (wide_dg)
    hipLaunchKernelGGL(carry_skip_kernel<true>, dim3((N + chunk - 1) / chunk), dim3(kSkipBlock), 0, st, N, K, assignments,
                       assignments_prev, cy, reinterpret_cast<const float2 *>(xmeta), drift, stats, tie_slack, row_list,
                       finite, pairs, counters, probe ? 1 : 0, (float)(wide_dg + 8u));
  else
    hipLaunchKernelGGL(carry_skip_kernel<false>, dim3((N + chunk - 1) / chunk), dim3(kSkipBlock), 0, st, N, K, assignments,
                       assignments_prev, cy, reinterpret_cast<const float2 *>(xmeta), drift, stats, tie_slack, row_list,
                       finite, pairs, counters, probe ? 1 : 0, 520.0f);
  return hipGetLastError();
}

template <int DP>
static hipError_t launch_coarse_carry_dp(const LloydArgs &a, const void *rows, bool half_rows, const void *xcache,
                                         const float *xmeta, const void *panelhi, uint32_t *undecided, float *und_thr,
                                         const CarryArgs &cy, uint32_t rows_hint, uint32_t *duo, hipStream_t st) {
  constexpr int NSET = DP <= 256 ? 2 : 1;
  const size_t lds_bytes = 2 * 64 * (size_t)(DP * 2) + 512 + 64 + (size_t)DP * 4;
  const uint32_t rows_per_block = 128u * NSET;
  uint32_t grid = (a.N + rows_per_block - 1) / rows_per_block;
  const bool fast = a.D == (uint32_t)DP;
  constexpr bool kS16 = NSET == 2 && DP >= 32;
  const bool s16 = kS16 && a.coarse_mfma != 32;
#define KMX_CARRY_LAUNCH_S(H, F, C, MODE, SRC, SHAPE)                                                                       \
  hipLaunchKernelGGL((lloyd_coarse2_kernel<DP, H, F, C, NSET, MODE, SHAPE>), dim3(grid), dim3(256), lds_bytes, st, SRC,     \
                     xmeta, a.N, a.D, reinterpret_cast<const float *>(panelhi), a.bias, a.mu, a.K_pad, a.K, a.stats,        \
                     a.eps, a.tie_slack, a.assignments, a.assignments_prev, undecided, und_thr, a.counters, cy, duo)
#define KMX_CARRY_LAUNCH(H, F, C, MODE, SRC)                           \
  do {                                                                 \
    if (s16) KMX_CARRY_LAUNCH_S(H, F, C, MODE, SRC, (kS16 && !(MODE == 2 && DP >= 256)) ? 16 : 32); \
    else KMX_CARRY_LAUNCH_S(H, F, C, MODE, SRC, 32);                   \
  } while (0)
  if (!cy.row_list) {
    KMX_CARRY_LAUNCH(false, true, true, 1, xcache);
    return hipGetLastError();
  }
  if (rows_hint != 0xFFFFFFFFu) {
    const uint32_t want = rows_hint / rows_per_block + rows_hint / (4 * rows_per_block) + 64;
    if (want < grid) grid = want;
  }
  if (const char *v = getenv("KMCUDA_AMD_CARRY_GRID")) {
    const long cap = atol(v);
    if (cap > 0 && (uint32_t)cap < grid) grid = (uint32_t)cap;
  }
  if (half_rows) {
    if (fast) KMX_CARRY_LAUNCH(true, true, false, 2, rows); else KMX_CARRY_LAUNCH(true, false, false, 2, rows);
  } else {
    if (fast) KMX_CARRY_LAUNCH(false, true, false, 2, rows); else KMX_CARRY_LAUNCH(false, false, false, 2, rows);
  }
#undef KMX_CARRY_LAUNCH
#undef KMX_CARRY_LAUNCH_S
  return hipGetLastError();
}

hipError_t launch_lloyd_coarse_carry(const LloydArgs &a, const void *rows, bool half_rows, const void *xcache,
                                     const float *xmeta, const void *panelhi, uint32_t *undecided, float *und_thr,
                                     const CarryArgs &cy, uint32_t rows_hint, uint32_t *duo, hipStream_t st) {
  switch (a.DP) {
#define KMX_CARRY_CASE(dp) \
    case dp: return launch_coarse_carry_dp<dp>(a, rows, half_rows, xcache, xmeta, panelhi, undecided, und_thr, cy, rows_hint, duo, st)
    KMX_CARRY_CASE(16); KMX_CARRY_CASE(32); KMX_CARRY_CASE(64); KMX_CARRY_CASE(128); KMX_CARRY_CASE(256); KMX_CARRY_CASE(512);
#undef KMX_CARRY_CASE
    default: return hipErrorInvalidValue;
  }
}

hipError_t launch_lloyd_refine_carry(const LloydArgs &a, const void *rows, bool half_rows, const void *panelhi,
                                     const uint32_t *row_list, const float *thr_list, const uint32_t *n_list,
                                     uint32_t rows_hint, const CarryArgs &cy, hipStream_t st) {
  return launch_lloyd_refine_t<true>(a, rows, half_rows, panelhi, row_list, thr_list, n_list, rows_hint, cy, st);
}

hipError_t preload_lloyd_carry_code() {
  hipFuncAttributes at;
  return hipFuncGetAttributes(&at, reinterpret_cast<const void *>(&carry_skip_kernel<false>));
}

}
```

kmcuda_amd/csrc/lloyd_coarse.hpp:

```cpp
#pragma once
#include <hip/hip_fp16.h>

#include "exact.hpp"
#include "filter_common.hpp"
#include "kernels.hpp"

#ifndef KMX_ABL
#define KMX_ABL 0
#endif

namespace kmx {

typedef float f32x16 __attribute__((ext_vector_type(16)));
typedef float f32x4 __attribute__((ext_vector_type(4)));
typedef _Float16 f16x8 __attribute__((ext_vector_type(8)));

template <int P>
struct TileParity { static constexpr int value = P; };
__device__ __forceinline__ f16x8 lds_frag_issue(uint32_t addr) {
  f16x8 f;
  asm volatile("ds_read_b128 %0, %1" : "=v"(f) : "v"(addr) : "memory");
  return f;
}
template <int OFF>
__device__ __forceinline__ f16x8 lds_frag_issue_off(uint32_t addr) {
  f16x8 f;
  asm volatile("ds_read_b128 %0, %1 offset:%2" : "=v"(f) : "v"(addr), "n"(OFF) : "memory");
  return f;
}
template <int N>
__device__ __forceinline__ void lds_frag_wait(f16x8 &f) {
  asm volatile("s_waitcnt lgkmcnt(%1)" : "+v"(f) : "n"(N));
}
__device__ __forceinline__ void frag_swap16(f16x8 &p, f16x8 &q) {
  typedef uint32_t u32x4 __attribute__((ext_vector_type(4)));
  u32x4 a = __builtin_bit_cast(u32x4, p), b = __builtin_bit_cast(u32x4, q);
#pragma unroll
  for (int d = 0; d < 4; d++) {
    const auto r = __builtin_amdgcn_permlane16_swap(a[d], b[d], false, false);
    a[d] = r[0];
    b[d] = r[1];
  }
  p = __builtin_bit_cast(f16x8, a);
  q = __builtin_bit_cast(f16x8, b);
}

template <int DP, bool HALF_ROWS, bool FAST, bool CACHED, int NSET, int CARRY = 0, int SHAPE = 32>
__global__ __launch_bounds__(256, 2) void lloyd_coarse2_kernel(
    const void *__restrict__ rows, const float *__restrict__ xmeta, uint32_t N, uint32_t D, const float *__restrict__ panelhi,
    const float *__restrict__ bias, const float *__restrict__ mu, uint32_t K_pad, uint32_t K,
    const uint32_t *__restrict__ stats, float eps, float tie_slack, uint32_t *__restrict__ assignments,
    uint32_t *__restrict__ assignments_prev, uint32_t *__restrict__ undecided, float *__restrict__ und_thr,
    uint32_t *__restrict__ counters, CarryArgs cy, uint32_t *__restrict__ duo = nullptr) {
  static_assert(CARRY == 0 || CARRY == 1 || CARRY == 2, "CARRY");
  static_assert(CARRY != 2 || !CACHED, "listed rows are gathered from the rows, not streamed from the row cache");
  static_assert(SHAPE == 32 || (SHAPE == 16 && NSET == 2 && DP >= 32), "16x16x32: two row sets, 32 features per k-step");
  constexpr bool S16 = SHAPE == 16;
  constexpr int NKH = DP / 2;
  constexpr int KS = NKH / 8;
  constexpr int ROWB = DP * 2;
  constexpr int SUPB = 64 * ROWB;
  constexpr int NP = SUPB / 1024;
  constexpr int SWM = (KS < 16 ? KS : 16) - 1;
  typedef __attribute__((address_space(3))) unsigned char lds_byte;
  extern __shared__ __attribute__((aligned(1024))) unsigned char lds2[];
  if (counters[kStopFlag] != 0u) return;
  const uint32_t lds0 = (uint32_t)(uintptr_t)(lds_byte *)lds2;
  if (lds0 & 1023u) __builtin_trap();
  const uint32_t bias0 = lds0 + 2 * SUPB;
  constexpr uint32_t BIASB = 512u;

  const int tid = threadIdx.x, lane = tid & 63, wave = __builtin_amdgcn_readfirstlane(tid >> 6), col = lane & 31, h = lane >> 5;
  constexpr int WV = 4;
  constexpr bool TWO = NSET == 2;
  uint32_t total = N;
  if constexpr (CARRY == 2) total = __builtin_amdgcn_readfirstlane(*cy.n_list);
  if constexpr (CARRY != 0) {
    if (blockIdx.x == 0 && threadIdx.x == 0) {
      if (cy.host_report) {
        volatile uint32_t *hr = cy.host_report;
        hr[0] = cy.n_list ? *cy.n_list : 0xFFFFFFFFu;
        hr[1] = cy.seq;
      }
      if constexpr (CARRY == 2) {
        const uint32_t paired = cy.l3 ? counters[3] : 0u;
        *reinterpret_cast<unsigned long long *>(counters + kCarrySkipped) += (unsigned long long)(N - total - paired);
        *reinterpret_cast<unsigned long long *>(counters + kCarryPaired) += (unsigned long long)paired;
      }
    }
  }
  if constexpr (CARRY == 2) {
    if (blockIdx.x * (128u * NSET) >= total) return;
  }
  for (uint32_t blk = blockIdx.x;;) {
  blk = __builtin_amdgcn_readfirstlane(blk);
  const uint32_t posA = blk * (128u * NSET) + wave * (32u * NSET) + col, posB = posA + 32u;
  const bool liveA = posA < total, liveB = TWO && posB < total;
  uint32_t sA = posA, sB = posB;
  if constexpr (CARRY == 2) {
    sA = liveA ? cy.row_list[posA] : 0u;
    sB = liveB ? cy.row_list[posB] : 0u;
  }

  f16x8 xa[KS], xb[TWO ? KS : 1];
  float xn2a = 0.f, x0a = 0.f, xn2b = 0.f, x0b = 0.f;
  float xdma = 0.f, xdmb = 0.f, xaba = 0.f, xabb = 0.f;
  auto load_chunk = [&](uint32_t s, bool live, int j, float (&xv)[8]) {
    const size_t row = (size_t)(live ? s : 0);
    if (FAST && HALF_ROWS) {
      const f16x8 raw = reinterpret_cast<const f16x8 *>(reinterpret_cast<const _Float16 *>(rows) + row * DP + h * NKH)[j];
#pragma unroll
      for (int q = 0; q < 8; q++) xv[q] = (float)raw[q];
    } else if (FAST) {
      const f32x4 *src = reinterpret_cast<const f32x4 *>(reinterpret_cast<const float *>(rows) + row * DP + h * NKH);
      const f32x4 a = src[2 * j], b = src[2 * j + 1];
      xv[0] = a.x; xv[1] = a.y; xv[2] = a.z; xv[3] = a.w;
      xv[4] = b.x; xv[5] = b.y; xv[6] = b.z; xv[7] = b.w;
    } else {
#pragma unroll
      for (int q = 0; q < 8; q++) {
        const uint32_t f = h * NKH + 8 * j + q;
        float v = 0.f;
        if (f < D) v = HALF_ROWS ? (float)reinterpret_cast<const _Float16 *>(rows)[row * D + f]
                                 : reinterpret_cast<const float *>(rows)[row * D + f];
        xv[q] = v;
      }
    }
  };
  auto centre = [&](const float (&xv)[8], const float (&mm)[8], f16x8 &hi, float &xn2) {
#pragma unroll
    for (int q = 0; q < 8; q++) {
      const float xc = xv[q] - mm[q];
      hi[q] = (_Float16)xc;
      xn2 = fmaf(xc, xc, xn2);
    }
  };
// ... 200 lines not shown
      if constexpr (TWO) accB = __builtin_amdgcn_mfma_f32_32x32x16_f16(f, xb[j], accB, 0, 0, 0);
      stage_after(j, stage, sp_next, buf_next);
    }
    const float v1a_in = v1a[PAR], v1b_in = v1b[PAR];
    if (KMX_ABL & 4) {
      v1a[PAR] = fmaxf(v1a[PAR], accA[0]); v2a[PAR] = fmaxf(v2a[PAR], accA[15]);
      if constexpr (TWO) { v1b[PAR] = fmaxf(v1b[PAR], accB[0]); v2b[PAR] = fmaxf(v2b[PAR], accB[15]); }
    } else {
#pragma unroll
      for (int r = 0; r < 16; r += 2) {
        book2(accA[r], accA[r + 1], r, v1a[PAR], v2a[PAR]);
        if constexpr (TWO) book2(accB[r], accB[r + 1], r, v1b[PAR], v2b[PAR]);
      }
    }
    tba[PAR] = (v1a[PAR] != v1a_in) ? t : tba[PAR];
    tbb[PAR] = (v1b[PAR] != v1b_in) ? t : tbb[PAR];
  };

  for (uint32_t sp = 0; sp < nsuper; sp++) {
    const int buf = sp & 1;
    const bool stage = sp + 1 < nsuper;
    const uint32_t base = buf * SUPB, bb = mybias + buf * 256;
    tile_pass(base, bb, 2 * sp, stage, sp + 1, buf ^ 1, TileParity<0>());
    tile_pass(base + 32 * ROWB, bb + 128, 2 * sp + 1, false, sp + 1, buf ^ 1, TileParity<1>());
    asm volatile("s_waitcnt vmcnt(0)" ::: "memory");
    if (!(KMX_ABL & 16)) __syncthreads();
  }
  if (KMX_ABL & 8) {
    float keep = 0.f;
    uint32_t keept = 0;
#pragma unroll
    for (int q = 0; q < (S16 ? 4 : 1); q++) { keep += w1[q] + w2[q]; keept += wt[q]; }
    if (v1a[0] + v2a[0] + v1b[0] + v2b[0] + v1a[1] + v2a[1] + v1b[1] + v2b[1] + keep == 1.2345f) assignments[0] = tba[0] + tbb[0] + tba[1] + tbb[1] + keept;
    return;
  }

  const float cmaxc = sqrtf(__uint_as_float(stats[0])) * 1.000001f;
  const float bmaxc = __uint_as_float(stats[1]);
  const float cmaxo = sqrtf(__uint_as_float(stats[2])) * 1.000001f;
  const float mu_norm = (CACHED || CARRY == 2) ? xmeta[2 * (((size_t)N + 255) / 256 * 256)] : cmaxo;
  const float dcmax = sqrtf(__uint_as_float(stats[5])) * 1.000001f;
  const float u = 5.9604645e-8f;
  uint32_t und_count = 0, changed_count = 0, duo_count = 0;
  unsigned long long uma = 0, umb = 0, dma = 0, dmb = 0;
  bool unda = false, undb = false, duoa = false, duob = false;
  uint32_t d1a = 0, d2a = 0, d1b = 0, d2b = 0;
  float dra = 0.f, drb = 0.f;
  const bool want_duo = duo != nullptr;
  const bool angular = tie_slack > 0.f;
  auto quarters32 = [&](const float (&q1)[2], const float (&q2)[2], const uint32_t (&qt)[2], float (&kq)[4],
                        uint32_t (&jq)[4], float &others) {
    auto index_of = [&](float v, uint32_t tb, uint32_t hh) {
      const uint32_t r = __float_as_uint(v) & 15u;
      return tb * 32u + (r & 3u) + 8u * (r >> 2) + 4u * hh;
    };
    kq[0] = q1[0]; kq[1] = q1[1]; kq[2] = __shfl_xor(q1[0], 32); kq[3] = __shfl_xor(q1[1], 32);
    jq[0] = index_of(kq[0], qt[0], h); jq[1] = index_of(kq[1], qt[1], h);
    jq[2] = __shfl_xor(jq[0], 32); jq[3] = __shfl_xor(jq[1], 32);
    const float mine2 = fmaxf(q2[0], q2[1]);
    others = fmaxf(mine2, __shfl_xor(mine2, 32));
  };
  auto quarters16 = [&](float (&kq)[4], uint32_t (&jq)[4], float &others) {
    const int g = lane >> 4;
    float o[4];
#pragma unroll
    for (int r = 0; r < 4; r++) {
      const int gq = g ^ r;
      auto pick = [&](const auto (&a)[4]) {
        const auto lo = (gq & 1) ? a[1] : a[0], hi = (gq & 1) ? a[3] : a[2];
        return (gq & 2) ? hi : lo;
      };
      float v = pick(w1), v2 = pick(w2);
      uint32_t tb = pick(wt);
      if (r) { v = __shfl_xor(v, 16 * r); v2 = __shfl_xor(v2, 16 * r); tb = __shfl_xor(tb, 16 * r); }
      const uint32_t ri = __float_as_uint(v) & 15u;
      kq[r] = v;
      o[r] = v2;
      jq[r] = tb * 32u + 16u * (ri >> 2) + 4u * (uint32_t)gq + (ri & 3u);
    }
    others = fmaxf(fmaxf(o[0], o[1]), fmaxf(o[2], o[3]));
  };
  auto finish = [&](uint32_t s, bool mine, const float (&kq)[4], const uint32_t (&jq)[4], float others, float xn2,
                    float x0, float dx2, float xdm, float xab, bool &und, unsigned long long &um, float &cut, bool &is_duo,
                    unsigned long long &dm, uint32_t &dc1, uint32_t &dc2, float &drest) {
    const bool insane = (x0 != x0);
    float k0 = kq[0], k1 = kq[1], k2 = kq[2], k3 = kq[3];
    uint32_t j0 = jq[0], j1 = jq[1], j2 = jq[2], j3 = jq[3];
    auto order = [](float &a, uint32_t &ia, float &b, uint32_t &ib) {
      const bool g = b > a;
      const float ta = g ? b : a, tb2 = g ? a : b;
      const uint32_t ja = g ? ib : ia, jb = g ? ia : ib;
      a = ta; b = tb2; ia = ja; ib = jb;
    };
    order(k0, j0, k1, j1); order(k2, j2, k3, j3); order(k0, j0, k2, j2); order(k1, j1, k3, j3); order(k1, j1, k2, j2);
    float v1 = k0;
    const uint32_t i1 = j0;
    const float v2 = fmaxf(k1, others);
    const float xn = sqrtf(xn2) * 1.0001f, xo = (xn + mu_norm) * 1.0001f;
    const float dx = dx2 >= 0.f ? sqrtf(dx2) * 1.0001f : 4.8829e-4f * xn;
    const float e_c = 2.0f * eps * (xn * cmaxc + bmaxc) + (xn * dcmax + dx * cmaxc + dx * dcmax) * 1.001f +
                      6e-8f * sqrtf((float)DP) * (xn + cmaxc) + 2.0e-6f * (1.001f * xn * cmaxc + bmaxc);
    const float e_ref = u * (12.0f * xo * cmaxo + 4.0f * cmaxo * cmaxo);
    const float thr = 2.0f * (e_c + e_ref) * 1.001f + tie_slack;
    const bool in_range = (xn < 6.0e4f) && (cmaxc < 6.0e4f) && (v1 > -1.0e38f) && (i1 < K);
    const ClampLimits lim = clamp_limits(angular, xdm, dot_error(DP, xab >= 0.f ? xab : xo * mu_norm), 0.5f * thr);
    const bool certain = insane || (in_range && ((v1 - v2) > thr) && (v2 < lim.hi) && (v1 > lim.lo));
    bool changed = false;
    if (mine && certain) changed = commit_row(s, insane ? K : i1, assignments, assignments_prev);
    und = mine && !certain;
    is_duo = false;
    {
      float c0 = in_range ? v1 - thr : __builtin_nanf("");
      if (angular) c0 = (lim.hi == lim.hi) ? fminf(c0, lim.hi) : __builtin_nanf("");
      is_duo = want_duo && und && (k1 >= c0) && (k2 < c0) && (others < c0) && (j1 < K);
      if (is_duo) und = false;
      dc1 = j0; dc2 = j1; drest = fmaxf(k2, others);
    }
    if constexpr (CARRY != 0) {
      if (mine && cy.angular) {
        const float e = e_c * 1.001f;
        float gapv = (certain && !insane && in_range)
                         ? fminf(fminf((v1 - e) - (v2 + e), lim.hi - v2), v1 - lim.lo) * 0.999999f : -INFINITY;
        if (!(gapv == gapv)) gapv = -INFINITY;
        cy.ub[s] = gapv;
        if (cy.l3) cy.l3[s] = 0.f;
      } else if (mine) {
        float ubv = INFINITY, lbv = 0.f;
        if (!insane && in_range) {
          const float e = e_c * 1.001f;
          const float d2u = fmaxf(xn2 * (1.0f + 2.0f * eps) - 2.0f * (v1 - e), 0.f);
          const float d2l = xn2 * (1.0f - 2.0f * eps) - 2.0f * (v2 + e);
          const float geo = 2.4e-7f * (xn + cmaxc);
          ubv = sqrtf(d2u) * 1.000001f + geo;
          if (certain && d2l > 0.f) lbv = fmaxf(sqrtf(d2l) * 0.999999f - geo, 0.f);
          if (!(ubv == ubv)) ubv = INFINITY;
          if (!(lbv == lbv)) lbv = 0.f;
        }
        cy.ub[s] = ubv;
        cy.lb[s] = lbv;
        if (cy.l3) cy.l3[s] = 0.f;
      }
    }
    cut = in_range ? v1 - thr : __builtin_nanf("");
    if (angular) cut = (lim.hi == lim.hi) ? fminf(cut, lim.hi) : __builtin_nanf("");
    const unsigned long long cm = __ballot(changed);
    um = __ballot(und);
    dm = __ballot(is_duo);
    changed_count += (uint32_t)__popcll(cm);
    und_count += (uint32_t)__popcll(um);
    duo_count += (uint32_t)__popcll(dm);
  };
  float dx2a = -2.f, dx2b = -2.f;
  if constexpr (CACHED || CARRY == 2) {
    const float2 ma = reinterpret_cast<const float2 *>(xmeta)[sA], mb = reinterpret_cast<const float2 *>(xmeta)[TWO ? sB : sA];
    xn2a = ma.x; dx2a = ma.y; xn2b = mb.x; dx2b = mb.y;
    x0a = (ma.y == -1.f) ? __builtin_nanf("") : 0.f;
    x0b = (mb.y == -1.f) ? __builtin_nanf("") : 0.f;
    xaba = xabb = -1.f;
    if (angular) {
      const float *xdot = xmeta + 2 * (((size_t)N + 255) / 256 * 256) + 2;
      xdma = xdot[sA];
      xdmb = xdot[TWO ? sB : sA];
    }
  } else if (angular) {
    const uint32_t fb = (uint32_t)(h * NKH), fe = min(fb + (uint32_t)NKH, D);
    if (fb < fe) {
      if constexpr (HALF_ROWS) {
        row_dot_mu(reinterpret_cast<const _Float16 *>(rows) + (size_t)(liveA ? sA : 0u) * D, mu, fb, fe, xdma, xaba);
        if constexpr (TWO) row_dot_mu(reinterpret_cast<const _Float16 *>(rows) + (size_t)(liveB ? sB : 0u) * D, mu, fb, fe, xdmb, xabb);
      } else {
        row_dot_mu(reinterpret_cast<const float *>(rows) + (size_t)(liveA ? sA : 0u) * D, mu, fb, fe, xdma, xaba);
        if constexpr (TWO) row_dot_mu(reinterpret_cast<const float *>(rows) + (size_t)(liveB ? sB : 0u) * D, mu, fb, fe, xdmb, xabb);
      }
    }
    xdma += __shfl_xor(xdma, 32); xaba += __shfl_xor(xaba, 32);
    xdmb += __shfl_xor(xdmb, 32); xabb += __shfl_xor(xabb, 32);
  }
  float cuta, cutb = 0.f;
  float kq[4], oth;
  uint32_t jq[4];
  if constexpr (S16) {
    quarters16(kq, jq, oth);
    const bool mine = h ? liveB : liveA;
    sA = h ? sB : sA;
    finish(sA, mine, kq, jq, oth, h ? xn2b : xn2a, h ? x0b : x0a, h ? dx2b : dx2a, h ? xdmb : xdma, h ? xabb : xaba, unda, uma,
           cuta, duoa, dma, d1a, d2a, dra);
  } else {
    quarters32(v1a, v2a, tba, kq, jq, oth);
    finish(sA, h == 0 && liveA, kq, jq, oth, xn2a, x0a, dx2a, xdma, xaba, unda, uma, cuta, duoa, dma, d1a, d2a, dra);
    if constexpr (TWO) {
      quarters32(v1b, v2b, tbb, kq, jq, oth);
      finish(sB, h == 0 && liveB, kq, jq, oth, xn2b, x0b, dx2b, xdmb, xabb, undb, umb, cutb, duob, dmb, d1b, d2b, drb);
    }
  }
  __shared__ uint32_t blk_und[WV], blk_changed[WV], blk_duo[WV], blk_base, blk_duo_base;
  if (lane == 0) {
    blk_und[wave] = und_count;
    blk_changed[wave] = changed_count;
    blk_duo[wave] = duo_count;
  }
  __syncthreads();
  if (threadIdx.x == 0) {
    uint32_t tu = 0, tc = 0, td = 0;
#pragma unroll
    for (int w = 0; w < WV; w++) {
      tu += blk_und[w];
      tc += blk_changed[w];
      td += blk_duo[w];
    }
    if (tc) atomicAdd(&counters[0], tc);
    blk_base = tu ? atomicAdd(&counters[4], tu) : 0u;
    blk_duo_base = td ? atomicAdd(&counters[kDuoCount], td) : 0u;
  }
  __syncthreads();
  if (duo_count) {
    uint32_t base = blk_duo_base;
    for (int w = 0; w < wave; w++) base += blk_duo[w];
    const unsigned long long below = (1ull << lane) - 1ull;
    if (duoa) {
      const uint32_t at = base + (uint32_t)__popcll(dma & below);
      reinterpret_cast<uint4 *>(duo)[at] = make_uint4(sA, d1a, d2a, __float_as_uint(dra));
    }
    if (duob) {
      const uint32_t at = base + (uint32_t)__popcll(dma) + (uint32_t)__popcll(dmb & below);
      reinterpret_cast<uint4 *>(duo)[at] = make_uint4(sB, d1b, d2b, __float_as_uint(drb));
    }
  }
  if (und_count) {
    uint32_t base = blk_base;
    for (int w = 0; w < wave; w++) base += blk_und[w];
    const unsigned long long below = (1ull << lane) - 1ull;
    if (unda) {
      const uint32_t at = base + (uint32_t)__popcll(uma & below);
      undecided[at] = sA;
      und_thr[at] = cuta;
    }
    if (undb) {
      const uint32_t at = base + (uint32_t)__popcll(uma) + (uint32_t)__popcll(umb & below);
      undecided[at] = sB;
      und_thr[at] = cutb;
    }
  }
  if constexpr (CARRY != 2) {
    break;
  } else {
    blk += gridDim.x;
    if ((uint64_t)blk * (128u * NSET) >= total) break;
    __syncthreads();
  }
  }
}

}
```

kmcuda_amd/csrc/lloyd_duo.hip:

```cpp
#include <hip/hip_runtime.h>

#include "filter_common.hpp"
#include "kernels.hpp"

namespace kmx {

typedef float f32x4 __attribute__((ext_vector_type(4)));

__device__ __forceinline__ float row16_sum(float v) {
  v += __int_as_float(__builtin_amdgcn_update_dpp(0, __float_as_int(v), 0xB1, 0xF, 0xF, true));
  v += __int_as_float(__builtin_amdgcn_update_dpp(0, __float_as_int(v), 0x4E, 0xF, 0xF, true));
  v += __int_as_float(__builtin_amdgcn_update_dpp(0, __float_as_int(v), 0x141, 0xF, 0xF, true));
  v += __int_as_float(__builtin_amdgcn_update_dpp(0, __float_as_int(v), 0x140, 0xF, 0xF, true));
  return v;
}

constexpr uint32_t kDuoPend = 64;

template <int NI, bool FAST, bool BOUNDS = false>
__global__ __launch_bounds__(256, NI >= 4 ? 2 : 4) void lloyd_duo_kernel(
    const float *__restrict__ samples, uint32_t D, uint32_t DP, uint32_t K, const float *__restrict__ cfil,
    const float *__restrict__ bias, const float *__restrict__ mu, const uint32_t *__restrict__ stats, float eps,
    float tie_slack, const uint4 *__restrict__ duo, uint32_t *__restrict__ assignments,
    uint32_t *__restrict__ assignments_prev, uint32_t *__restrict__ flagged, uint32_t *__restrict__ pairs,
    uint32_t *__restrict__ counters, CarryArgs cy) {
  if (counters[kStopFlag] != 0u) return;
  constexpr int SLOTS = NI >= 8 ? 1 : 2;
  const uint32_t total = counters[kDuoCount];
  const uint32_t lane = threadIdx.x & 63, wave = threadIdx.x >> 6, g = lane >> 4, l = lane & 15;
  const float cmaxc = sqrtf(__uint_as_float(stats[0])) * 1.000001f;
  const float bmaxc = __uint_as_float(stats[1]);
  const float cmaxo = sqrtf(__uint_as_float(stats[2])) * 1.000001f;
  const float u = 5.9604645e-8f;
  const bool angular = tie_slack > 0.f;
  float mreg[NI][4];
#pragma unroll
  for (int i = 0; i < NI; i++) {
    const uint32_t f = 64u * i + 4u * l;
#pragma unroll
    for (int e = 0; e < 4; e++) mreg[i][e] = f + e < DP ? mu[f + e] : 0.f;
  }
  __shared__ uint32_t pbuf[4][kDuoPend * 3], fbuf[4][kDuoPend], blk_n[4][3], blk_base[2];
  uint32_t *mypairs = pbuf[wave], *myflags = fbuf[wave];
  uint32_t np = 0, nf = 0, nchg = 0;
  auto flush = [&](uint32_t *list_counter, uint32_t *list, const uint32_t *buf, uint32_t words_each, uint32_t &n) {
    if (n == 0) return;
    uint32_t base = 0;
    if (lane == 0) base = atomicAdd(list_counter, n);
    base = __shfl(base, 0);
    for (uint32_t i = lane; i < n * words_each; i += 64) list[words_each * (size_t)base + i] = buf[i];
    n = 0;
  };
    const uint32_t per_iter = 4u * SLOTS;
  uint4 rec_next[SLOTS];
  auto request = [&](uint32_t base) {
#pragma unroll
    for (int k = 0; k < SLOTS; k++) {
      const uint32_t p = base + 4u * k + g;
      rec_next[k] = p < total ? duo[p] : make_uint4(0u, 0u, 0u, 0u);
    }
  };
  request((blockIdx.x * 4u + wave) * per_iter);
  for (uint32_t base = (blockIdx.x * 4u + wave) * per_iter; base < total; base += gridDim.x * 4u * per_iter) {
    uint4 rec[SLOTS];
    bool live[SLOTS];
    f32x4 xv[SLOTS][NI], c1v[SLOTS][NI], c2v[SLOTS][NI];
    uint32_t old_asg[SLOTS];
    float bias_a[SLOTS], bias_b[SLOTS];
#pragma unroll
    for (int k = 0; k < SLOTS; k++) {
      live[k] = base + 4u * k + g < total;
      rec[k] = rec_next[k];
    }
    request(base + gridDim.x * 4u * per_iter);
#pragma unroll
    for (int k = 0; k < SLOTS; k++) {
      old_asg[k] = assignments[rec[k].x];
      bias_a[k] = bias[rec[k].y];
      bias_b[k] = bias[rec[k].z];
    }
#pragma unroll
    for (int k = 0; k < SLOTS; k++) {
      const float *xr = samples + (size_t)rec[k].x * D;
      const float *r1 = cfil + (size_t)rec[k].y * DP, *r2 = cfil + (size_t)rec[k].z * DP;
#pragma unroll
      for (int i = 0; i < NI; i++) {
        const uint32_t f = 64u * i + 4u * l;
        f32x4 x = {0.f, 0.f, 0.f, 0.f}, a = x, b = x;
        if (f < DP) {
          if (FAST) {
            x = __builtin_nontemporal_load(reinterpret_cast<const f32x4 *>(xr + f));
          } else {
            x.x = f + 0 < D ? xr[f + 0] : 0.f; x.y = f + 1 < D ? xr[f + 1] : 0.f;
            x.z = f + 2 < D ? xr[f + 2] : 0.f; x.w = f + 3 < D ? xr[f + 3] : 0.f;
          }
          a = *reinterpret_cast<const f32x4 *>(r1 + f);
          b = *reinterpret_cast<const f32x4 *>(r2 + f);
        }
        xv[k][i] = x; c1v[k][i] = a; c2v[k][i] = b;
      }
    }
#pragma unroll
    for (int k = 0; k < SLOTS; k++) {
      float xn2 = 0.f, xo2 = 0.f, p1 = 0.f, p2 = 0.f, xdm = 0.f, xab = 0.f, nan0 = 0.f;
#pragma unroll
      for (int i = 0; i < NI; i++) {
        const float x4[4] = {xv[k][i].x, xv[k][i].y, xv[k][i].z, xv[k][i].w};
        const float a4[4] = {c1v[k][i].x, c1v[k][i].y, c1v[k][i].z, c1v[k][i].w};
        const float b4[4] = {c2v[k][i].x, c2v[k][i].y, c2v[k][i].z, c2v[k][i].w};
#pragma unroll
        for (int e = 0; e < 4; e++) {
          const float xc = x4[e] - mreg[i][e];
          xn2 = fmaf(xc, xc, xn2);
          xo2 = fmaf(x4[e], x4[e], xo2);
          p1 = fmaf(xc, a4[e], p1);
          p2 = fmaf(xc, b4[e], p2);
          if (angular) {
            xdm = fmaf(x4[e], mreg[i][e], xdm);
            xab = fmaf(fabsf(x4[e]), fabsf(mreg[i][e]), xab);
          }
        }
        if (i == 0 && l == 0 && x4[0] != x4[0]) nan0 = 1.f;
      }
      xn2 = row16_sum(xn2); xo2 = row16_sum(xo2); p1 = row16_sum(p1); p2 = row16_sum(p2); nan0 = row16_sum(nan0);
      if (angular) { xdm = row16_sum(xdm); xab = row16_sum(xab); }
      const uint32_t s = rec[k].x, ca = rec[k].y, cb = rec[k].z;
      const float va = p1 + bias_a[k], vb = p2 + bias_b[k];
      float v1 = va, v2 = -INFINITY;
      const float v3 = -INFINITY;
      uint32_t i1 = ca, i2 = 0xFFFFFFFFu;
      if (!(va > -INFINITY)) { v1 = -INFINITY; i1 = 0xFFFFFFFFu; }
      {
        const bool g1 = vb > v1, g2 = vb > v2;
        i2 = g1 ? i1 : (g2 ? cb : i2);
        v2 = g1 ? v1 : (g2 ? vb : v2);
        i1 = g1 ? cb : i1;
        v1 = g1 ? vb : v1;
      }
      const bool insane = nan0 > 0.f;
      const float xn = sqrtf(xn2) * 1.0001f, xo = sqrtf(xo2) * 1.0001f;
      const float e_mfma = 2.0f * eps * (xn * cmaxc + bmaxc);
      const float e_ref = u * (12.0f * xo * cmaxo + 4.0f * cmaxo * cmaxo);
      const float thr = 2.0f * (e_mfma + e_ref) * 1.001f + tie_slack;
      const bool in_range = (xn < 6.0e4f) && (cmaxc < 6.0e4f) && i1 < K;
      const ClampLimits lim = clamp_limits(angular, xdm, dot_error((int)DP, xab), 0.5f * thr);
      const bool certain = insane || (in_range && ((v1 - v2) > thr) && (v2 < lim.hi) && (v1 > lim.lo));
      const bool two = !certain && in_range && ((v1 - v3) > thr) && (v3 < lim.hi) && (v1 > lim.lo) && i2 < K;
      const bool mine = live[k] && l == 0;
      const bool pair_now = mine && two, flag_now = mine && !certain && !two;
      if (mine && certain) {
        const uint32_t nearest = insane ? K : i1;
        assignments_prev[s] = old_asg[k];
        if (old_asg[k] != nearest) {
          assignments[s] = nearest;
          nchg++;
        }
      }
      if constexpr (BOUNDS) {
        if (mine) {
          const float rest = __uint_as_float(rec[k].w);
          const bool ok = !insane && in_range && (certain || two);
          const float e = e_mfma * 1.001f;
          const float dcmax = sqrtf(__uint_as_float(stats[5])) * 1.000001f, dxw = 4.8829e-4f * xn;
          const float e_c = 2.0f * eps * (xn * cmaxc + bmaxc) + (xn * dcmax + dxw * cmaxc + dxw * dcmax) * 1.001f +
                            6e-8f * sqrtf((float)DP) * (xn + cmaxc) + 2.0e-6f * (1.001f * xn * cmaxc + bmaxc);
          const float w = fmaxf(rest + e_c * 1.001f, v3 + e);
          if (cy.angular) {
            float pairg = 0.f;
            if (ok && i2 < K) pairg = fminf(fminf((v2 - e) - w, lim.hi - w), v2 - lim.lo) * 0.999999f;
            if (!(pairg > 0.f)) pairg = 0.f;
            cy.ub[s] = -INFINITY;
            cy.l3[s] = pairg;
            if (pairg > 0.f) { cy.p1[s] = i1; cy.p2[s] = i2; }
          } else {
            float ubv = INFINITY, l3v = 0.f;
            if (ok) {
              const float geo = 2.4e-7f * (xn + cmaxc);
              const float d2l = xn2 * (1.0f - 2.0f * eps) - 2.0f * w;
              float low = d2l > 0.f ? fmaxf(sqrtf(d2l) * 0.999999f - geo, 0.f) : 0.f;
              if (!(low == low)) low = 0.f;
              ubv = sqrtf(fmaxf(xn2 * (1.0f + 2.0f * eps) - 2.0f * (v2 - e), 0.f)) * 1.000001f + geo;
              if (!(ubv == ubv)) ubv = INFINITY;
              if (i2 < K) l3v = low;
            }
            cy.ub[s] = ubv;
            cy.lb[s] = 0.f;
            cy.l3[s] = l3v;
            if (l3v > 0.f) { cy.p1[s] = i1; cy.p2[s] = i2; }
          }
        }
      }
      const unsigned long long pm = __ballot(pair_now), fm = __ballot(flag_now);
      if (pm) {
        if (np + 4 > kDuoPend) flush(&counters[3], pairs, mypairs, 3, np);
        if (pair_now) {
          const uint32_t at = np + (uint32_t)__popcll(pm & ((1ull << lane) - 1ull));
          mypairs[3 * at + 0] = s; mypairs[3 * at + 1] = i1; mypairs[3 * at + 2] = i2;
        }
        np += (uint32_t)__popcll(pm);
      }
      if (fm) {
        if (nf + 4 > kDuoPend) flush(&counters[1], flagged, myflags, 1, nf);
        if (flag_now) myflags[nf + (uint32_t)__popcll(fm & ((1ull << lane) - 1ull))] = s;
        nf += (uint32_t)__popcll(fm);
      }
    }
  }
#pragma unroll
  for (int off = 32; off > 0; off >>= 1) nchg += __shfl_xor(nchg, off);
  if (lane == 0) { blk_n[wave][0] = np; blk_n[wave][1] = nf; blk_n[wave][2] = nchg; }
  __syncthreads();
  if (threadIdx.x == 0) {
    uint32_t tp = 0, tf = 0, tc = 0;
    for (int w = 0; w < 4; w++) { tp += blk_n[w][0]; tf += blk_n[w][1]; tc += blk_n[w][2]; }
    blk_base[0] = tp ? atomicAdd(&counters[3], tp) : 0u;
    blk_base[1] = tf ? atomicAdd(&counters[1], tf) : 0u;
    if (tc) atomicAdd(&counters[0], tc);
  }
  __syncthreads();
  uint32_t bp = blk_base[0], bf = blk_base[1];
  for (uint32_t w = 0; w < wave; w++) { bp += blk_n[w][0]; bf += blk_n[w][1]; }
  for (uint32_t i = lane; i < np * 3; i += 64) pairs[3 * (size_t)bp + i] = mypairs[i];
  for (uint32_t i = lane; i < nf; i += 64) flagged[bf + i] = myflags[i];
}

template <int NI>
static hipError_t launch_duo_ni(const LloydArgs &a, const uint32_t *duo, hipStream_t st, const CarryArgs *cy) {
  const bool fast = a.D == a.DP && (((uintptr_t)a.samples) & 15u) == 0 && a.DP % 4 == 0;
  const uint32_t want = (a.N + 31u) / 32u, full = NI >= 4 ? 512u : 1024u;
  const dim3 grid(want < full ? (want ? want : 1u) : full);
#define KMX_DUO_LAUNCH(F, B, CY)                                                                                      \
  hipLaunchKernelGGL((lloyd_duo_kernel<NI, F, B>), grid, dim3(256), 0, st, a.samples, a.D, a.DP, a.K, a.cfil, a.bias,    \
                     a.mu, a.stats, a.eps, a.tie_slack, reinterpret_cast<const uint4 *>(duo), a.assignments,          \
                     a.assignments_prev, a.flagged, a.pairs, a.counters, CY)
  if (cy && cy->l3) {
    if (fast) KMX_DUO_LAUNCH(true, true, *cy); else KMX_DUO_LAUNCH(false, true, *cy);
  } else {
    if (fast) KMX_DUO_LAUNCH(true, false, CarryArgs()); else KMX_DUO_LAUNCH(false, false, CarryArgs());
  }
#undef KMX_DUO_LAUNCH
  return hipGetLastError();
}

hipError_t launch_lloyd_duo(const LloydArgs &a, const uint32_t *duo, hipStream_t st, const CarryArgs *cy) {
  if (a.N == 0) return hipSuccess;
  switch (a.DP) {
    case 16: case 32: case 64: return launch_duo_ni<1>(a, duo, st, cy);
    case 128: return launch_duo_ni<2>(a, duo, st, cy);
    case 256: return launch_duo_ni<4>(a, duo, st, cy);
    case 512: return launch_duo_ni<8>(a, duo, st, cy);
    default: return hipErrorInvalidValue;
  }
}

hipError_t preload_lloyd_duo_code() {
  hipFuncAttributes at;
  return hipFuncGetAttributes(&at, reinterpret_cast<const void *>(&lloyd_duo_kernel<4, true>));
}

}
```

kmcuda_amd/csrc/lloyd_f16.hip:

```cpp
#include <hip/hip_fp16.h>

#include "exact.hpp"
#include "filter_common.hpp"
#include "kernels.hpp"
#include "lloyd_coarse.hpp"
#include "lloyd_refine.hpp"

namespace kmx {

__global__ __launch_bounds__(256) void centroid_panelhi_kernel(
    const float *__restrict__ centroids, uint32_t K, uint32_t D, uint32_t K_pad, uint32_t DP,
    const uint32_t *__restrict__ finite, const float *__restrict__ mu, const float *__restrict__ bias,
    _Float16 *__restrict__ panelhi, uint32_t K_pad64, uint32_t *__restrict__ stats) {
  const uint32_t lane = threadIdx.x & 63, wave = threadIdx.x >> 6;
  const uint32_t c = blockIdx.x * 4 + wave;
  uint32_t res_bits = 0;
  if (c < K_pad64) {
    const bool real = c < K_pad;
    const bool ok = c < K && finite[c];
    float res2 = 0.f;
    for (uint32_t f = lane; f < DP; f += 64) {
      float v = 0.f;
      if (ok && f < D) v = centroids[(size_t)c * D + f] - mu[f];
      const _Float16 hi = (_Float16)v;
// ... 122 lines not shown
      s2 = max(s2, __float_as_uint(plain * 1.0001f));
      s3 = max(s3, __float_as_uint(m2 * 1.0001f));
      s4 = max(s4, __float_as_uint(mag2 * 1.0001f));
    }
    s5 = max(s5, ((res2 - res2) == 0.f) ? __float_as_uint(res2 * 1.0001f) : 0x7F800000u);
    if (lane == 0) {
      if (METRIC != 0 && drift && c < K) {
        const float db = b - bias[c];
        drift[K + c] = db;
        if (ok && (db - db) == 0.f && db > 0.f) s7 = max(s7, __float_as_uint(db * 1.000001f));
        else if (ok && !((db - db) == 0.f)) s7 = 0x7F800000u;
      }
      if (real) { bias[c] = b; bias2[c] = b2; }
      reinterpret_cast<float *>(panelhi + (size_t)K_pad64 * DP)[c] = real ? fmaxf(b, -3.0e38f) : -3.0e38f;
    }
  }
  __shared__ uint32_t red[4][8];
  if (lane == 0) { red[wave][0] = s0; red[wave][1] = s1; red[wave][2] = s2; red[wave][3] = s3; red[wave][4] = s4; red[wave][5] = s5; red[wave][6] = s6; red[wave][7] = s7; }
  __syncthreads();
  if (threadIdx.x < 8) {
    const uint32_t m = max(max(red[0][threadIdx.x], red[1][threadIdx.x]), max(red[2][threadIdx.x], red[3][threadIdx.x]));
    if (m) atomicMax(&stats[threadIdx.x], m);
  }
}

hipError_t launch_centroid_prep_frozen(int metric, const float *centroids, uint32_t K, uint32_t D, uint32_t K_pad,
                                       uint32_t DP, const float *mu, uint32_t *finite, float *bias, float *bias2,
                                       float *cfil, void *panelhi, uint32_t *stats, uint32_t *stats_next,
                                       uint32_t *zero_a, uint32_t *zero_b, uint32_t *zero_c, float *drift,
                                       uint32_t *zero_d, hipStream_t st) {
  const uint32_t K_pad64 = (K_pad + 63u) / 64u * 64u;
  float *cen = const_cast<float *>(centroids);
  if (metric == 0)
    hipLaunchKernelGGL((centroid_prep_frozen_kernel<0, false>), dim3(K_pad64 / 16), dim3(256), 0, st, cen, K, D, K_pad,
                       DP, K_pad64, mu, finite, bias, bias2, cfil, reinterpret_cast<_Float16 *>(panelhi), stats,
                       stats_next, zero_a, zero_b, zero_c, (const double *)nullptr, (const double *)nullptr,
                       (uint32_t *)nullptr, StopCtl(), drift, zero_d);
  else
    hipLaunchKernelGGL((centroid_prep_frozen_kernel<1, false>), dim3(K_pad64 / 16), dim3(256), 0, st, cen, K, D, K_pad,
                       DP, K_pad64, mu, finite, bias, bias2, cfil, reinterpret_cast<_Float16 *>(panelhi), stats,
                       stats_next, zero_a, zero_b, zero_c, (const double *)nullptr, (const double *)nullptr,
                       (uint32_t *)nullptr, StopCtl(), drift, zero_d);
  return hipGetLastError();
}

hipError_t launch_apply_prep_frozen(const double *delta, const double *dcount_d, float *centroids, uint32_t *ccounts,
                                    const StopCtl &stop, uint32_t K, uint32_t D, uint32_t K_pad, uint32_t DP,
                                    const float *mu, uint32_t *finite, float *bias, float *bias2, float *cfil,
                                    void *panelhi, uint32_t *stats, uint32_t *stats_next, uint32_t *zero_a,
                                    uint32_t *zero_b, uint32_t *zero_c, float *drift, uint32_t *zero_d, hipStream_t st) {
  const uint32_t K_pad64 = (K_pad + 63u) / 64u * 64u;
  hipLaunchKernelGGL((centroid_prep_frozen_kernel<0, true>), dim3(K_pad64 / 16), dim3(256), 0, st, centroids, K, D, K_pad,
                     DP, K_pad64, mu, finite, bias, bias2, cfil, reinterpret_cast<_Float16 *>(panelhi), stats, stats_next,
                     zero_a, zero_b, zero_c, delta, dcount_d, ccounts, stop, drift, zero_d);
  return hipGetLastError();
}


hipError_t launch_centroid_panelhi(const float *centroids, uint32_t K, uint32_t D, uint32_t K_pad, uint32_t DP,
                                   const uint32_t *finite, const float *mu, const float *bias, void *panelhi,
                                   uint32_t *stats, hipStream_t st) {
  const uint32_t K_pad64 = (K_pad + 63u) / 64u * 64u;
  hipLaunchKernelGGL(centroid_panelhi_kernel, dim3(K_pad64 / 4), dim3(256), 0, st, centroids, K, D, K_pad, DP, finite,
                     mu, bias, reinterpret_cast<_Float16 *>(panelhi), K_pad64, stats);
  return hipGetLastError();
}

bool lloyd_filter_f16_supported(uint32_t D, uint32_t DP) { return DP >= 16 && D <= DP; }

template <int DP>
static hipError_t launch_coarse2_dp(const LloydArgs &a, const void *rows, bool half_rows, const void *xcache,
                                    const float *xmeta, const void *panelhi, uint32_t *undecided, float *und_thr,
                                    uint32_t *duo, hipStream_t st) {
  constexpr int NSET = DP <= 256 ? 2 : 1;
  const size_t lds_bytes = 2 * 64 * (size_t)(DP * 2) + 512 + 64 + (size_t)DP * 4;
  const uint32_t rows_per_block = 128u * NSET;
  const uint32_t grid = (a.N + rows_per_block - 1) / rows_per_block;
  const bool fast = a.D == (uint32_t)DP;
  constexpr bool kS16 = NSET == 2 && DP >= 32;
  const bool s16 = kS16 && a.coarse_mfma != 32;
#define KMX_CRS2_LAUNCH_S(H, F, C, SRC, SHAPE)                                                                            \
  hipLaunchKernelGGL((lloyd_coarse2_kernel<DP, H, F, C, NSET, 0, SHAPE>), dim3(grid), dim3(256), lds_bytes, st, SRC, xmeta, \
                     a.N, a.D, reinterpret_cast<const float *>(panelhi), a.bias, a.mu, a.K_pad, a.K, a.stats,             \
                     a.eps, a.tie_slack, a.assignments, a.assignments_prev, undecided, und_thr, a.counters, CarryArgs(), duo)
#define KMX_CRS2_LAUNCH(H, F, C, SRC)                       \
  do {                                                      \
    if (s16) KMX_CRS2_LAUNCH_S(H, F, C, SRC, kS16 ? 16 : 32); \
    else KMX_CRS2_LAUNCH_S(H, F, C, SRC, 32);               \
  } while (0)
  if (xcache) {
    KMX_CRS2_LAUNCH(false, true, true, xcache);
  } else if (half_rows) {
    if (fast) KMX_CRS2_LAUNCH(true, true, false, rows); else KMX_CRS2_LAUNCH(true, false, false, rows);
  } else {
    if (fast) KMX_CRS2_LAUNCH(false, true, false, rows); else KMX_CRS2_LAUNCH(false, false, false, rows);
  }
#undef KMX_CRS2_LAUNCH
#undef KMX_CRS2_LAUNCH_S
  return hipGetLastError();
}

hipError_t launch_lloyd_coarse(const LloydArgs &a, const void *rows, bool half_rows, const void *xcache,
                               const float *xmeta, const void *panelhi, uint32_t *undecided, float *und_thr,
                               uint32_t *duo, hipStream_t st) {
  switch (a.DP) {
    case 16: return launch_coarse2_dp<16>(a, rows, half_rows, xcache, xmeta, panelhi, undecided, und_thr, duo, st);
    case 32: return launch_coarse2_dp<32>(a, rows, half_rows, xcache, xmeta, panelhi, undecided, und_thr, duo, st);
    case 64: return launch_coarse2_dp<64>(a, rows, half_rows, xcache, xmeta, panelhi, undecided, und_thr, duo, st);
    case 128: return launch_coarse2_dp<128>(a, rows, half_rows, xcache, xmeta, panelhi, undecided, und_thr, duo, st);
    case 256: return launch_coarse2_dp<256>(a, rows, half_rows, xcache, xmeta, panelhi, undecided, und_thr, duo, st);
    case 512: return launch_coarse2_dp<512>(a, rows, half_rows, xcache, xmeta, panelhi, undecided, und_thr, duo, st);
    default: return hipErrorInvalidValue;
  }
}

hipError_t launch_lloyd_refine(const LloydArgs &a, const void *rows, bool half_rows, const void *panelhi,
                               const uint32_t *row_list, const float *thr_list, const uint32_t *n_list,
                               uint32_t rows_hint, hipStream_t st) {
  return launch_lloyd_refine_t<false>(a, rows, half_rows, panelhi, row_list, thr_list, n_list, rows_hint, CarryArgs(), st);
}

template <int DP, bool HALF_ROWS, bool FAST>
__global__ __launch_bounds__(256) void row_cache_kernel(const void *__restrict__ rows, uint32_t N, uint32_t D,
                                                        const float *__restrict__ mu, f16x8 *__restrict__ xcache,
                                                        float2 *__restrict__ xmeta, uint32_t nblocks32) {
  float *__restrict__ xdot = reinterpret_cast<float *>(xmeta) + 2 * ((size_t)nblocks32 * 32) + 2;
  constexpr int NKH = DP / 2, KS = NKH / 8;
  const int lane = threadIdx.x & 63, col = lane & 31, h = lane >> 5;
  for (uint32_t b = blockIdx.x * 4u + (threadIdx.x >> 6); b < nblocks32; b += gridDim.x * 4u) {
  if (b == 0) {
    float m2 = 0.f;
    for (uint32_t f = lane; f < (uint32_t)DP; f += 64) m2 = fmaf(mu[f], mu[f], m2);
#pragma unroll
    for (int o = 32; o > 0; o >>= 1) m2 += __shfl_xor(m2, o);
    if (lane == 0) xmeta[(size_t)nblocks32 * 32] = make_float2(sqrtf(m2) * 1.00001f, 0.f);
  }
  const uint32_t s = b * 32u + col;
  const bool live = s < N;
  const size_t row = (size_t)(live ? s : 0);
  float xn2 = 0.f, dx2 = 0.f, x0 = 0.f, xdm = 0.f;
#pragma unroll
  for (int j = 0; j < KS; j++) {
    float xv[8];
    if (FAST && HALF_ROWS) {
      const f16x8 raw = reinterpret_cast<const f16x8 *>(reinterpret_cast<const _Float16 *>(rows) + row * DP + h * NKH)[j];
#pragma unroll
      for (int q = 0; q < 8; q++) xv[q] = (float)raw[q];
    } else if (FAST) {
      const f32x4 *src = reinterpret_cast<const f32x4 *>(reinterpret_cast<const float *>(rows) + row * DP + h * NKH);
      const f32x4 a = src[2 * j], c = src[2 * j + 1];
      xv[0] = a.x; xv[1] = a.y; xv[2] = a.z; xv[3] = a.w;
      xv[4] = c.x; xv[5] = c.y; xv[6] = c.z; xv[7] = c.w;
    } else {
#pragma unroll
      for (int q = 0; q < 8; q++) {
        const uint32_t f = h * NKH + 8 * j + q;
        float v = 0.f;
        if (f < D) v = HALF_ROWS ? (float)reinterpret_cast<const _Float16 *>(rows)[row * D + f]
                                 : reinterpret_cast<const float *>(rows)[row * D + f];
        xv[q] = v;
      }
    }
    f16x8 hi;
#pragma unroll
    for (int q = 0; q < 8; q++) {
      const float mq = mu[h * NKH + 8 * j + q];
      const float xc = live ? xv[q] - mq : 0.f;
// ... 55 lines not shown
```

kmcuda_amd/csrc/lloyd_refine.hpp:

```cpp
#pragma once
#include "lloyd_coarse.hpp"

namespace kmx {

constexpr int kRefineCap = 8;
template <int DP, bool HALF_ROWS, bool FAST, int NSET, bool PAIRS = false>
__global__ __launch_bounds__(256, 2) void lloyd_refine_kernel(
    const void *__restrict__ rows, const float *__restrict__ samples, uint32_t N, uint32_t D,
    const float *__restrict__ panelhi, const float *__restrict__ cfil, const float *__restrict__ bias,
    const float *__restrict__ mu, uint32_t K_pad, uint32_t K, const uint32_t *__restrict__ stats, float eps,
    float tie_slack, uint32_t *__restrict__ assignments, uint32_t *__restrict__ assignments_prev,
    const uint32_t *__restrict__ row_list, const float *__restrict__ thr_list, const uint32_t *__restrict__ n_list,
    uint32_t *__restrict__ flagged, uint32_t *__restrict__ pairs, uint32_t *__restrict__ counters, CarryArgs cy) {
  constexpr int NKH = DP / 2;
  constexpr int KS = NKH / 8;
  constexpr int ROWB = DP * 2;
  constexpr int SUPB = 64 * ROWB;
  constexpr int NP = SUPB / 1024;
  constexpr int SWM = (KS < 16 ? KS : 16) - 1;
  const uint32_t total = *n_list;
  constexpr bool want_rest = PAIRS;
  constexpr bool TWO = NSET == 2;
  typedef __attribute__((address_space(3))) unsigned char lds_byte;
  extern __shared__ __attribute__((aligned(1024))) unsigned char lds2[];
  const uint32_t lds0 = (uint32_t)(uintptr_t)(lds_byte *)lds2;
  if (lds0 & 1023u) __builtin_trap();
  const uint32_t bias0 = lds0 + 2 * SUPB;
  const uint32_t mu_lds = bias0 + 512 + 64;
  const uint32_t cnt_lds = mu_lds + DP * 4;
  const uint32_t list_lds = cnt_lds + 1024;
  auto lds_u32 = [](uint32_t addr) { return reinterpret_cast<__attribute__((address_space(3))) uint32_t *>((uintptr_t)addr); };
  for (uint32_t blk = blockIdx.x; (size_t)blk * (128u * NSET) < total; blk += gridDim.x) {

  const int tid = threadIdx.x, lane = tid & 63, wave = __builtin_amdgcn_readfirstlane(tid >> 6), col = lane & 31, h = lane >> 5;
  const uint32_t posA = blk * (128u * NSET) + wave * (32u * NSET) + col, posB = posA + 32u;
  const bool liveA = posA < total, liveB = TWO && posB < total;
  const uint32_t sA = liveA ? row_list[posA] : 0u, sB = liveB ? row_list[posB] : 0u;
  const float cutA = liveA ? thr_list[posA] : INFINITY, cutB = liveB ? thr_list[posB] : INFINITY;
  const uint32_t rlA = wave * (32u * NSET) + col, rlB = rlA + 32u;
  *lds_u32(cnt_lds + tid * 4) = 0u;

  f16x8 xa[KS], xb[TWO ? KS : 1];
  auto load_chunk = [&](uint32_t s, int j, float (&xv)[8]) {
    const size_t row = (size_t)s;
    if (FAST && HALF_ROWS) {
      const f16x8 raw = reinterpret_cast<const f16x8 *>(reinterpret_cast<const _Float16 *>(rows) + row * DP + h * NKH)[j];
#pragma unroll
      for (int q = 0; q < 8; q++) xv[q] = (float)raw[q];
    } else if (FAST) {
      const f32x4 *src = reinterpret_cast<const f32x4 *>(reinterpret_cast<const float *>(rows) + row * DP + h * NKH);
      const f32x4 a = src[2 * j], b = src[2 * j + 1];
      xv[0] = a.x; xv[1] = a.y; xv[2] = a.z; xv[3] = a.w;
      xv[4] = b.x; xv[5] = b.y; xv[6] = b.z; xv[7] = b.w;
    } else {
#pragma unroll
      for (int q = 0; q < 8; q++) {
        const uint32_t f = h * NKH + 8 * j + q;
        float v = 0.f;
        if (f < D) v = HALF_ROWS ? (float)reinterpret_cast<const _Float16 *>(rows)[row * D + f]
                                 : reinterpret_cast<const float *>(rows)[row * D + f];
        xv[q] = v;
      }
    }
  };
  const uint32_t nsuper = (K_pad + 63) / 64;
  const float *biashi = reinterpret_cast<const float *>(reinterpret_cast<const unsigned char *>(panelhi) + (size_t)nsuper * SUPB);
  auto stage_piece = [&](uint32_t sp, int buf, int p) {
    uint32_t P0 = (uint32_t)lane * 16u;
    asm volatile("" : "+v"(P0));
    const unsigned char *src = reinterpret_cast<const unsigned char *>(panelhi) + (size_t)sp * SUPB;
    const uint32_t P = (uint32_t)p * 1024u + P0;
    const uint32_t from = P ^ (((P / ROWB) & SWM) << 4);
    __builtin_amdgcn_global_load_lds((const __attribute__((address_space(1))) void *)(src + from),
                                     (__attribute__((address_space(3))) void *)(uintptr_t)(lds0 + buf * SUPB + p * 1024), 16, 0, 0);
  };
  auto stage_bias = [&](uint32_t sp, int buf) {
    __builtin_amdgcn_global_load_lds((const __attribute__((address_space(1))) void *)(biashi + sp * 64u + lane),
                                     (__attribute__((address_space(3))) void *)(uintptr_t)(bias0 + buf * 256), 4, 0, 0);
  };
  {
    constexpr int MUP = (DP * 4 + 1023) / 1024;
    if (wave < MUP && lane * 16 < DP * 4 - wave * 1024)
      __builtin_amdgcn_global_load_lds((const __attribute__((address_space(1))) void *)(reinterpret_cast<const unsigned char *>(mu) + wave * 1024 + lane * 16),
                                       (__attribute__((address_space(3))) void *)(uintptr_t)(mu_lds + wave * 1024), 16, 0, 0);
  }
  for (int p = wave; p < NP; p += 4) stage_piece(0, 0, p);
  if (wave == 0) stage_bias(0, 0);
  {
    constexpr int BJ = KS > 8 ? 8 : KS;
#pragma unroll
    for (int j0 = 0; j0 < KS; j0 += BJ) {
      float va[BJ][8], vb[TWO ? BJ : 1][8];
#pragma unroll
      for (int jj = 0; jj < BJ; jj++) load_chunk(sA, j0 + jj, va[jj]);
#pragma unroll
      for (int jj = 0; jj < (TWO ? BJ : 0); jj++) load_chunk(sB, j0 + jj, vb[jj]);
// ... 132 lines not shown
      const uint32_t m_lds = mu_lds + (uint32_t)(h * NKH + f0) * 4u;
#pragma unroll
      for (int f = 0; f < FC; f += 4) {
        float x4[4], m4[4];
        if (FAST) {
          const f32x4 a = *reinterpret_cast<const f32x4 *>(xr + f);
          const f32x4 b = *reinterpret_cast<const __attribute__((address_space(3))) f32x4 *>((uintptr_t)(m_lds + f * 4));
          x4[0] = a.x; x4[1] = a.y; x4[2] = a.z; x4[3] = a.w;
          m4[0] = b.x; m4[1] = b.y; m4[2] = b.z; m4[3] = b.w;
        } else {
#pragma unroll
          for (int q = 0; q < 4; q++) {
            const uint32_t ff = h * NKH + f0 + f + q;
            x4[q] = ff < D ? xr[f + q] : 0.f;
            m4[q] = m[f + q];
          }
        }
#pragma unroll
        for (int q = 0; q < 4; q++) {
          const float xc = x4[q] - m4[q];
          xv[f + q] = xc;
          xn2 = fmaf(xc, xc, xn2);
          xo2 = fmaf(x4[q], x4[q], xo2);
        }
        if (f == 0 && ch == 0) x0 = x4[0];
      }
#pragma unroll
      for (int i = 0; i < kRefineCap; i++) {
        if ((uint32_t)i < nmax) {
          const bool on = usable && (uint32_t)i < n;
          const uint32_t c = on ? *lds_u32(list_lds + (rl * kRefineCap + i) * 4) : 0u;
          const float *cr = cfil + (size_t)c * DP + h * NKH + f0;
          float a0 = 0.f, a1 = 0.f, a2 = 0.f, a3 = 0.f;
#pragma unroll
          for (int f = 0; f < FC; f += 4) {
            const f32x4 c4 = *reinterpret_cast<const f32x4 *>(cr + f);
            a0 = fmaf(xv[f + 0], c4.x, a0);
            a1 = fmaf(xv[f + 1], c4.y, a1);
            a2 = fmaf(xv[f + 2], c4.z, a2);
            a3 = fmaf(xv[f + 3], c4.w, a3);
          }
          part[i] += (a0 + a1) + (a2 + a3);
        }
      }
    }
#pragma unroll
    for (int i = 0; i < kRefineCap; i++) {
      if ((uint32_t)i < nmax) {
        const bool on = usable && (uint32_t)i < n;
        const uint32_t c = on ? *lds_u32(list_lds + (rl * kRefineCap + i) * 4) : 0u;
        const float v = (part[i] + __shfl_xor(part[i], 32)) + bias[c];
        if (on) {
          const bool g1 = v > v1, g2 = v > v2, g3 = v > v3;
          v3 = g2 ? v2 : (g3 ? v : v3);
          i2 = g1 ? i1 : (g2 ? c : i2);
          v2 = g1 ? v1 : (g2 ? v : v2);
          i1 = g1 ? c : i1;
          v1 = g1 ? v : v1;
        }
      }
    }
    xn2 += __shfl_xor(xn2, 32);
    xo2 += __shfl_xor(xo2, 32);
    if (tie_slack > 0.f) {
      const uint32_t fb = (uint32_t)(h * NKH), fe = min(fb + (uint32_t)NKH, D);
      if (fb < fe) row_dot_mu(samples + (size_t)s * D, mu, fb, fe, xdm, xab);
      xdm += __shfl_xor(xdm, 32);
      xab += __shfl_xor(xab, 32);
    }
    x0 = __shfl(x0, col);
    const bool insane = (x0 != x0);
    const float xn = sqrtf(xn2) * 1.0001f, xo = sqrtf(xo2) * 1.0001f;
    const float e_mfma = 2.0f * eps * (xn * cmaxc + bmaxc);
    const float e_ref = u * (12.0f * xo * cmaxo + 4.0f * cmaxo * cmaxo);
    const float thr = 2.0f * (e_mfma + e_ref) * 1.001f + tie_slack;
    const bool in_range = usable && (xn < 6.0e4f) && (cmaxc < 6.0e4f) && i1 < K;
    const ClampLimits lim = clamp_limits(tie_slack > 0.f, xdm, dot_error(DP, xab), 0.5f * thr);
    const bool certain = insane || (in_range && ((v1 - v2) > thr) && (v2 < lim.hi) && (v1 > lim.lo));
    const bool two = !certain && in_range && ((v1 - v3) > thr) && (v3 < lim.hi) && (v1 > lim.lo) && i2 < K;
    const bool mine = (h == 0) && live;
    const bool pair_now = mine && two, flag_now = mine && !certain && !two;
    bool changed = false;
    if (mine && certain) changed = commit_row(s, insane ? K : i1, assignments, assignments_prev);
    if constexpr (want_rest) {
      rest = fmaxf(rest, __shfl_xor(rest, 32));
      if (mine && cy.angular) {
        float gapv = -INFINITY, pairg = 0.f;
        if (!insane && in_range && (certain || two)) {
          const float e = e_mfma * 1.001f;
          const float dcmax = sqrtf(__uint_as_float(stats[5])) * 1.000001f, dxw = 4.8829e-4f * xn;
          const float e_c = 2.0f * eps * (xn * cmaxc + bmaxc) + (xn * dcmax + dxw * cmaxc + dxw * dcmax) * 1.001f +
                            6e-8f * sqrtf((float)DP) * (xn + cmaxc) + 2.0e-6f * (1.001f * xn * cmaxc + bmaxc);
          const float w = fmaxf(rest + e_c * 1.001f, v3 + e);
          const float room_hi = lim.hi - w;
          if (n == 1) gapv = fminf(fminf((v1 - e) - w, room_hi), v1 - lim.lo) * 0.999999f;
          else if (i2 < K) pairg = fminf(fminf((v2 - e) - w, room_hi), v2 - lim.lo) * 0.999999f;
          if (!(gapv == gapv)) gapv = -INFINITY;
          if (!(pairg > 0.f)) pairg = 0.f;
        }
        cy.ub[s] = gapv;
        cy.l3[s] = pairg;
        if (pairg > 0.f) {
          cy.p1[s] = i1;
          cy.p2[s] = i2;
        }
      } else if (mine) {
        float ubv = INFINITY, lbv = 0.f, l3v = 0.f;
        if (!insane && in_range && (certain || two)) {
          const float e = e_mfma * 1.001f;
          const float dcmax = sqrtf(__uint_as_float(stats[5])) * 1.000001f, dxw = 4.8829e-4f * xn;
          const float e_c = 2.0f * eps * (xn * cmaxc + bmaxc) + (xn * dcmax + dxw * cmaxc + dxw * dcmax) * 1.001f +
                            6e-8f * sqrtf((float)DP) * (xn + cmaxc) + 2.0e-6f * (1.001f * xn * cmaxc + bmaxc);
          const float geo = 2.4e-7f * (xn + cmaxc);
          const float w = fmaxf(rest + e_c * 1.001f, v3 + e);
          const float d2l = xn2 * (1.0f - 2.0f * eps) - 2.0f * w;
          float low = d2l > 0.f ? fmaxf(sqrtf(d2l) * 0.999999f - geo, 0.f) : 0.f;
          if (!(low == low)) low = 0.f;
          const bool single = n == 1;
          const float vu = single ? v1 : v2;
          ubv = sqrtf(fmaxf(xn2 * (1.0f + 2.0f * eps) - 2.0f * (vu - e), 0.f)) * 1.000001f + geo;
          if (!(ubv == ubv)) ubv = INFINITY;
          if (single) lbv = low;
          else if (i2 < K) l3v = low;
        }
        cy.ub[s] = ubv;
        cy.lb[s] = lbv;
        cy.l3[s] = l3v;
        if (l3v > 0.f) {
          cy.p1[s] = i1;
          cy.p2[s] = i2;
        }
      }
    }
    const unsigned long long cm = __ballot(changed), pm = __ballot(pair_now), fm = __ballot(flag_now);
    if (lane == 0 && cm) atomicAdd(&counters[0], (uint32_t)__popcll(cm));
    if (pm) {
      uint32_t base = 0;
      if (lane == 0) base = atomicAdd(&counters[3], (uint32_t)__popcll(pm));
      base = __shfl(base, 0);
      if (pair_now) {
        const uint32_t slot = base + (uint32_t)__popcll(pm & ((1ull << lane) - 1ull));
        pairs[3 * (size_t)slot + 0] = s;
        pairs[3 * (size_t)slot + 1] = i1;
        pairs[3 * (size_t)slot + 2] = i2;
      }
    }
    if (fm) {
      uint32_t base = 0;
      if (lane == 0) base = atomicAdd(&counters[1], (uint32_t)__popcll(fm));
      base = __shfl(base, 0);
      if (flag_now) flagged[base + (uint32_t)__popcll(fm & ((1ull << lane) - 1ull))] = s;
    }
  };
  settle(sA, liveA, rlA, restA);
  if constexpr (TWO) settle(sB, liveB, rlB, restB);
  __syncthreads();
  }
}


template <int DP, int NSET, bool PAIRS>
static hipError_t launch_refine_dp_n(const LloydArgs &a, const void *rows, bool half_rows, const void *panelhi,
                                     const uint32_t *row_list, const float *thr_list, const uint32_t *n_list,
                                     uint32_t rows_hint, const CarryArgs &cy, hipStream_t st) {
  const size_t lds_bytes = 2 * 64 * (size_t)(DP * 2) + 512 + 64 + (size_t)DP * 4 + 1024 + 256 * kRefineCap * 4;
  const uint32_t rows_per_block = 128u * NSET;
  uint32_t grid = (a.N + rows_per_block - 1) / rows_per_block;
  if (rows_hint != 0xFFFFFFFFu) {
    uint32_t want = rows_hint / rows_per_block + rows_hint / (4 * rows_per_block) + 64;
    if (want < 512u) want = 512u;
    if (want < grid) grid = want;
  }
  const bool fast = a.D == (uint32_t)DP;
#define KMX_RFN_LAUNCH(H, F)                                                                                       \
  hipLaunchKernelGGL((lloyd_refine_kernel<DP, H, F, NSET, PAIRS>), dim3(grid), dim3(256), lds_bytes, st, rows, a.samples,  \
                     a.N, a.D, reinterpret_cast<const float *>(panelhi), a.cfil, a.bias, a.mu, a.K_pad, a.K,        \
                     a.stats, a.eps, a.tie_slack, a.assignments, a.assignments_prev, row_list, thr_list, n_list,    \
                     a.flagged, a.pairs, a.counters, cy)
  if (half_rows) {
    if (fast) KMX_RFN_LAUNCH(true, true); else KMX_RFN_LAUNCH(true, false);
  } else {
    if (fast) KMX_RFN_LAUNCH(false, true); else KMX_RFN_LAUNCH(false, false);
  }
#undef KMX_RFN_LAUNCH
  return hipGetLastError();
}

template <int DP, bool PAIRS>
static hipError_t launch_refine_dp(const LloydArgs &a, const void *rows, bool half_rows, const void *panelhi,
                                   const uint32_t *row_list, const float *thr_list, const uint32_t *n_list,
                                   uint32_t rows_hint, const CarryArgs &cy, hipStream_t st) {
  if constexpr (DP > 256) {
    return launch_refine_dp_n<DP, 1, PAIRS>(a, rows, half_rows, panelhi, row_list, thr_list, n_list, rows_hint, cy, st);
  } else if constexpr (DP >= 64) {
    if (rows_hint != 0xFFFFFFFFu && rows_hint <= 128u * 500u)
      return launch_refine_dp_n<DP, 1, PAIRS>(a, rows, half_rows, panelhi, row_list, thr_list, n_list, rows_hint, cy, st);
    return launch_refine_dp_n<DP, 2, PAIRS>(a, rows, half_rows, panelhi, row_list, thr_list, n_list, rows_hint, cy, st);
  } else {
    return launch_refine_dp_n<DP, 2, PAIRS>(a, rows, half_rows, panelhi, row_list, thr_list, n_list, rows_hint, cy, st);
  }
}

template <bool PAIRS>
static hipError_t launch_lloyd_refine_t(const LloydArgs &a, const void *rows, bool half_rows, const void *panelhi,
                               const uint32_t *row_list, const float *thr_list, const uint32_t *n_list,
                               uint32_t rows_hint, const CarryArgs &cy, hipStream_t st) {
  switch (a.DP) {
    case 16: return launch_refine_dp<16, PAIRS>(a, rows, half_rows, panelhi, row_list, thr_list, n_list, rows_hint, cy, st);
    case 32: return launch_refine_dp<32, PAIRS>(a, rows, half_rows, panelhi, row_list, thr_list, n_list, rows_hint, cy, st);
    case 64: return launch_refine_dp<64, PAIRS>(a, rows, half_rows, panelhi, row_list, thr_list, n_list, rows_hint, cy, st);
    case 128: return launch_refine_dp<128, PAIRS>(a, rows, half_rows, panelhi, row_list, thr_list, n_list, rows_hint, cy, st);
    case 256: return launch_refine_dp<256, PAIRS>(a, rows, half_rows, panelhi, row_list, thr_list, n_list, rows_hint, cy, st);
    case 512: return launch_refine_dp<512, PAIRS>(a, rows, half_rows, panelhi, row_list, thr_list, n_list, rows_hint, cy, st);
    default: return hipErrorInvalidValue;
  }
}


}
```

kmcuda_amd/csrc/update.hip:

```cpp
#include <stdio.h>
#include <stdlib.h>
#include <string.h>

#include <algorithm>

#include <rocprim/device/device_radix_sort.hpp>

#include "exact.hpp"
#include "kernels.hpp"

namespace kmx {

static unsigned bits_for(uint64_t maxval) {
  unsigned b = 1;
  while (b < 32 && (1ull << b) <= maxval) b++;
  return b;
}

size_t sort_temp_bytes(size_t n, uint32_t max_key) {
  size_t bytes = 0;
  (void)rocprim::radix_sort_pairs(nullptr, bytes, (const uint32_t *)nullptr, (uint32_t *)nullptr,
                                  (const uint32_t *)nullptr, (uint32_t *)nullptr, n, 0u, bits_for(max_key),
                                  (hipStream_t)0);
  return bytes;
// ... 524 lines not shown
__global__ __launch_bounds__(kSumThreads) void cluster_sums_w_kernel(SumArgs a, SumWeightArgs wa) {
  cluster_sums_body<DIRECT, VEC4, true>(a, wa);
}

__global__ __launch_bounds__(256) void weight_changed_kernel(const double *__restrict__ win, uint32_t K,
                                                             double *__restrict__ out) {
  __shared__ double red[256];
  double t = 0.0;
  for (uint32_t c = threadIdx.x; c < K; c += 256) t += win[c];
  red[threadIdx.x] = t;
  __syncthreads();
  for (uint32_t s = 128; s > 0; s >>= 1) {
    if (threadIdx.x < s) red[threadIdx.x] += red[threadIdx.x + s];
    __syncthreads();
  }
  if (threadIdx.x == 0) out[0] = red[0];
}

constexpr uint32_t kWeightBlocks = 1024;
__global__ __launch_bounds__(256) void weights_check_kernel(const float *__restrict__ w, uint32_t N, uint32_t chunk,
                                                            double *__restrict__ part) {
  __shared__ double red[256], bad[256];
  const uint32_t lo = blockIdx.x * chunk, hi = min(N, lo + chunk);
  double t = 0.0, b = 0.0;
  for (uint32_t s = lo + threadIdx.x; s < hi; s += 256) {
    const float v = w[s];
    if (v > 0.f && v < INFINITY) t += (double)v; else b += 1.0;
  }
  red[threadIdx.x] = t; bad[threadIdx.x] = b;
  __syncthreads();
  for (uint32_t s = 128; s > 0; s >>= 1) {
    if (threadIdx.x < s) { red[threadIdx.x] += red[threadIdx.x + s]; bad[threadIdx.x] += bad[threadIdx.x + s]; }
    __syncthreads();
  }
  if (threadIdx.x == 0) { part[2 * blockIdx.x] = red[0]; part[2 * blockIdx.x + 1] = bad[0]; }
}
__global__ __launch_bounds__(256) void weights_total_kernel(const double *__restrict__ part, uint32_t nb,
                                                            double *__restrict__ out) {
  __shared__ double red[256], bad[256];
  double t = 0.0, b = 0.0;
  for (uint32_t i = threadIdx.x; i < nb; i += 256) { t += part[2 * i]; b += part[2 * i + 1]; }
  red[threadIdx.x] = t; bad[threadIdx.x] = b;
  __syncthreads();
  for (uint32_t s = 128; s > 0; s >>= 1) {
    if (threadIdx.x < s) { red[threadIdx.x] += red[threadIdx.x + s]; bad[threadIdx.x] += bad[threadIdx.x + s]; }
    __syncthreads();
  }
  if (threadIdx.x == 0) { out[0] = red[0]; out[1] = bad[0]; }
}
size_t weights_check_doubles() { return 2 * (size_t)kWeightBlocks + 2; }
hipError_t launch_weights_check(const float *weights, uint32_t N, double *work, hipStream_t st) {
  const uint32_t chunk = ((N + kWeightBlocks - 1) / kWeightBlocks + 255u) / 256u * 256u;
  const uint32_t nb = chunk ? (N + chunk - 1) / chunk : 0;
  if (nb) hipLaunchKernelGGL(weights_check_kernel, dim3(nb), dim3(256), 0, st, weights, N, chunk, work + 2);
  hipLaunchKernelGGL(weights_total_kernel, dim3(1), dim3(256), 0, st, work + 2, nb, work);
  return hipGetLastError();
}

uint32_t move_bucket_stride(uint32_t K) {
  uint32_t s = 32;
  while (s > 1 && 2ull * K * s > 262144ull) s >>= 1;
  return s;
}
size_t move_bucket_words(uint32_t K) { return 2 * (size_t)K * move_bucket_stride(K) + 4; }

__global__ __launch_bounds__(256) void move_scatter_kernel(const uint32_t *__restrict__ prev,
                                                           const uint32_t *__restrict__ cur, uint32_t N, uint32_t K,
                                                           uint32_t *__restrict__ cursors, uint32_t stride,
                                                           uint32_t *__restrict__ bucket_rows, uint32_t cap) {
  const uint32_t s = blockIdx.x * 256u + threadIdx.x;
  uint32_t p, a;
  bool ein, eout;
  move_flags(prev, cur, s, N, K, p, a, ein, eout);
  if (ein) {
    const uint32_t at = atomicAdd(&cursors[(size_t)(2u * a) * stride], 1u);
    if (at < cap) bucket_rows[(size_t)(2u * a) * cap + at] = s;
  }
  if (eout) {
    const uint32_t at = atomicAdd(&cursors[(size_t)(2u * p + 1u) * stride], 1u);
    if (at < cap) bucket_rows[(size_t)(2u * p + 1u) * cap + at] = s;
  }
}

hipError_t launch_move_deltas(const float *samples, uint32_t N, uint32_t D, uint32_t K, const uint32_t *prev,
                              const uint32_t *cur, uint32_t *keys_tmp, uint32_t *vals_tmp, uint32_t *keys_sorted,
                              uint32_t *rows_sorted, uint32_t *offsets2, void *temp, size_t temp_bytes,
                              uint32_t *bucket_rows, uint32_t cap, double *delta, int32_t *dcount, double *tail,
                              const uint32_t *counters, uint32_t *blockoff, uint32_t *bucket_work, MoveState *ms,
                              hipStream_t st, const MoveWeights *mw) {
  const uint32_t stride = move_bucket_stride(K);
  SumArgs a;
  a.samples = samples; a.N = N; a.D = D; a.K = K; a.prev = prev; a.cur = cur;
  a.cursors = bucket_work; a.stride = stride; a.bucket_rows = bucket_rows; a.cap = cap;
  a.overflow = rows_sorted; a.rows_sorted = rows_sorted; a.offsets2 = offsets2;
  a.delta = delta; a.dcount = dcount; a.tail = tail; a.counters = counters;
  a.res = bucket_work + 2 * (size_t)K * stride; a.host = ms->host_dev;
  hipError_t e = hipSuccess;
  const bool vec4 = (D & 3u) == 0 && (((uintptr_t)samples) & 15u) == 0;
  const size_t sums_lds = kSumThreads * 4 * sizeof(double) + 2 * kBucketCapMax * sizeof(uint32_t);
  auto launch_sums = [&](bool direct) {
    if (mw) {
      const SumWeightArgs wa{mw->weights, mw->dweight, mw->win};
      const void *fn = direct ? (vec4 ? (const void *)cluster_sums_w_kernel<true, true> : (const void *)cluster_sums_w_kernel<true, false>)
                              : (vec4 ? (const void *)cluster_sums_w_kernel<false, true> : (const void *)cluster_sums_w_kernel<false, false>);
      if (hipFuncSetAttribute(fn, hipFuncAttributeMaxDynamicSharedMemorySize, (int)sums_lds) != hipSuccess) return;
      if (direct) {
        if (vec4) hipLaunchKernelGGL((cluster_sums_w_kernel<true, true>), dim3(K), dim3(kSumThreads), sums_lds, st, a, wa);
        else hipLaunchKernelGGL((cluster_sums_w_kernel<true, false>), dim3(K), dim3(kSumThreads), sums_lds, st, a, wa);
      } else {
        if (vec4) hipLaunchKernelGGL((cluster_sums_w_kernel<false, true>), dim3(K), dim3(kSumThreads), sums_lds, st, a, wa);
        else hipLaunchKernelGGL((cluster_sums_w_kernel<false, false>), dim3(K), dim3(kSumThreads), sums_lds, st, a, wa);
      }
      hipLaunchKernelGGL(weight_changed_kernel, dim3(1), dim3(256), 0, st, mw->win, K, mw->dweight + K);
      return;
    }
    const void *fn = direct ? (vec4 ? (const void *)cluster_sums_kernel<true, true> : (const void *)cluster_sums_kernel<true, false>)
                            : (vec4 ? (const void *)cluster_sums_kernel<false, true> : (const void *)cluster_sums_kernel<false, false>);
    if (hipFuncSetAttribute(fn, hipFuncAttributeMaxDynamicSharedMemorySize, (int)sums_lds) != hipSuccess) return;
    if (direct) {
      if (vec4) hipLaunchKernelGGL((cluster_sums_kernel<true, true>), dim3(K), dim3(kSumThreads), sums_lds, st, a);
      else hipLaunchKernelGGL((cluster_sums_kernel<true, false>), dim3(K), dim3(kSumThreads), sums_lds, st, a);
    } else {
      if (vec4) hipLaunchKernelGGL((cluster_sums_kernel<false, true>), dim3(K), dim3(kSumThreads), sums_lds, st, a);
      else hipLaunchKernelGGL((cluster_sums_kernel<false, false>), dim3(K), dim3(kSumThreads), sums_lds, st, a);
    }
  };
  const bool force_radix = ms->force == 1, force_sync = ms->force == 2, force_direct = ms->force == 3;
  const uint32_t est_max = std::max((uint32_t)ms->host[1] , ms->last_events / K);
  const bool radix = N != 0 && !force_direct &&
                     (force_radix || ms->last_events > N / 2 || est_max > cap - cap / 4);
  if (N == 0) {
    e = hipMemsetAsync(offsets2, 0, (2 * (size_t)K + 1) * sizeof(uint32_t), st);
    if (e != hipSuccess) return e;
    launch_sums(false);
  } else if (radix) {
    ms->n_radix++;
    const uint32_t nb = (N + kMoveRows - 1) / kMoveRows;
    hipLaunchKernelGGL(move_count_kernel, dim3(nb), dim3(256), 0, st, prev, cur, N, K, blockoff);
    hipLaunchKernelGGL(move_scan_kernel, dim3(1), dim3(1024), 0, st, blockoff, nb, blockoff + nb + 1);
    hipLaunchKernelGGL(move_write_kernel, dim3(nb), dim3(256), 0, st, prev, cur, N, K, blockoff, keys_tmp, vals_tmp);
    e = hipGetLastError();
    if (e != hipSuccess) return e;
    e = hipMemcpyAsync(ms->host + 3, blockoff + nb + 1, sizeof(uint32_t), hipMemcpyDeviceToHost, st);
    if (e == hipSuccess) e = hipStreamSynchronize(st);
    if (e != hipSuccess) return e;
    const uint32_t m = ms->host[3];
    if (m) {
      e = rocprim::radix_sort_pairs(temp, temp_bytes, (const uint32_t *)keys_tmp, keys_sorted,
                                    (const uint32_t *)vals_tmp, rows_sorted, (size_t)m, 0u, bits_for(2ull * K), st);
      if (e != hipSuccess) return e;
    }
    hipLaunchKernelGGL(offsets_kernel, dim3((2 * K + 1 + 255) / 256), dim3(256), 0, st, keys_sorted, m, 2 * K, offsets2);
    ms->last_events = m;
    ms->host[0] = m;
    launch_sums(false);
  } else {
    ms->n_direct++;
    hipLaunchKernelGGL(move_scatter_kernel, dim3((N + 255) / 256), dim3(256), 0, st, prev, cur, N, K, bucket_work,
                       stride, bucket_rows, cap);
    launch_sums(true);
    e = hipGetLastError();
    if (e != hipSuccess) return e;
    if (force_sync) {
      e = hipStreamSynchronize(st);
      if (e != hipSuccess) return e;
    }
    ms->last_events = ms->host[0];
  }
  return hipGetLastError();
}

template <int METRIC, bool WEIGHTED>
__device__ __forceinline__ void apply_delta_body(const double *__restrict__ delta, const int32_t *__restrict__ dcount,
                                                 const double *__restrict__ dcount_d, uint32_t D,
                                                 float *__restrict__ centroids, uint32_t *__restrict__ ccounts,
                                                 const StopCtl &ctl, const double *__restrict__ wtail,
                                                 double *__restrict__ cweights) {
  const uint32_t c = blockIdx.x;
  if (ctl.counters) {
    bool stop = ctl.counters[kStopFlag] != 0u;
    if constexpr (WEIGHTED) {
      if (ctl.threshold >= 0.f && dcount_d) stop = stop || (float)wtail[gridDim.x] <= ctl.threshold;
    } else {
      if (ctl.threshold >= 0.f && dcount_d) stop = stop || (float)(uint32_t)dcount_d[gridDim.x] <= ctl.threshold;
    }
    if (c == 0 && threadIdx.x == 0) {
      if (stop) ctl.counters[kStopFlag] = 1u;
      else if (ctl.threshold >= 0.f) ctl.counters[0] = 0u;
      if (ctl.host_tail) {
        volatile uint32_t *ht = ctl.host_tail;
        for (uint32_t i = 0; i < 4; i++) ht[i] = dcount_d ? (uint32_t)dcount_d[gridDim.x + i] : 0u;
        ht[4] = stop ? 1u : 0u;
        __threadfence_system();
        ht[5] = ctl.seq;
      }
    }
    if (stop) return;
  }
  const double *d = delta + (size_t)c * D;
  float *cen = centroids + (size_t)c * D;
  const uint32_t cnt_old = ccounts[c];
  const uint32_t cnt_new = cnt_old + (uint32_t)(dcount_d ? (int32_t)dcount_d[c] : dcount[c]);
  double w, cn;
  if constexpr (WEIGHTED) {
    w = cnt_old ? cweights[c] : 0.0;
    cn = w + wtail[c];
  } else {
    w = (double)cnt_old;
    cn = (double)cnt_new;
  }
  if (cnt_new == 0) {
    for (uint32_t f = threadIdx.x; f < D; f += blockDim.x) cen[f] = __builtin_nanf("");
  } else if (METRIC == 0) {
    for (uint32_t f = threadIdx.x; f < D; f += blockDim.x) cen[f] = (float)(((double)cen[f] * w + d[f]) / cn);
  } else {
    __shared__ double red[256];
    double a = 0;
    for (uint32_t f = threadIdx.x; f < D; f += blockDim.x) {
      const double v = (double)cen[f] * w + d[f];
      a += v * v;
    }
    red[threadIdx.x] = a;
    __syncthreads();
    for (uint32_t s = blockDim.x / 2; s > 0; s >>= 1) {
      if (threadIdx.x < s) red[threadIdx.x] += red[threadIdx.x + s];
      __syncthreads();
    }
    const double nrm = sqrt(red[0]);
    for (uint32_t f = threadIdx.x; f < D; f += blockDim.x) cen[f] = (float)(((double)cen[f] * w + d[f]) / nrm);
  }
  __syncthreads();
  if (threadIdx.x == 0) {
    ccounts[c] = cnt_new;
    if constexpr (WEIGHTED) cweights[c] = cnt_new ? cn : 0.0;
  }
}

template <int METRIC>
__global__ void apply_delta_kernel(const double *__restrict__ delta, const int32_t *__restrict__ dcount,
                                   const double *__restrict__ dcount_d, uint32_t D, float *__restrict__ centroids,
                                   uint32_t *__restrict__ ccounts, StopCtl ctl) {
  apply_delta_body<METRIC, false>(delta, dcount, dcount_d, D, centroids, ccounts, ctl, nullptr, nullptr);
// ... 148 lines not shown
```

Baseline: 2.207 billion.

## Track moved rows in a bitmask so the update scatter only visits candidates

Adds a per-row bitmask that the assignment kernels (coarse cached path, refine, pair, exact, settle, duo) fill with rows that changed or were left undecided. The coarse kernel writes whole wave ballots directly, and the later kernels set bits with atomicOr. The move-delta scatter then walks set bits instead of reading prev/cur for all N rows, which cuts the full-N scan of two assignment arrays in steady state. The cost is extra atomics and mask writes in the assignment kernels. Correctness depends on every kernel that can change a row marking it, and on mask words no longer written by the coarse path still holding their initial all-ones state.

```diff
diff --git a/kmcuda_amd/csrc/engine.cpp b/kmcuda_amd/csrc/engine.cpp
--- a/kmcuda_amd/csrc/engine.cpp
+++ b/kmcuda_amd/csrc/engine.cpp
@@ -114,6 +114,7 @@
   if (const char *c = getenv("KMCUDA_AMD_CARRY_PAIRS")) carry_pairs_ = atoi(c) != 0;
   if (const char *c = getenv("KMCUDA_AMD_SETTLE")) settle_ = atoi(c) != 0;
   if (const char *c = getenv("KMCUDA_AMD_DUO")) { duo_on_ = atoi(c) != 0; duo_always_ = atoi(c) == 2; }
+  if (const char *c = getenv("KMCUDA_AMD_MOVE_MASK")) move_mask_on_ = atoi(c) != 0;
   if (const char *c = getenv("KMCUDA_AMD_COARSE_MFMA")) coarse_mfma_ = atoi(c) == 32 ? 32u : 16u;
   if (const char *c = getenv("KMCUDA_AMD_WIDE")) wide_ok_ = atoi(c) != 0;
   if (const char *c = getenv("KMCUDA_AMD_GEMM")) wide_ok_ = atoi(c) != 0;
@@ -376,6 +377,7 @@
                        uint32_t *assignments, uint32_t *assignments_prev, float *bounds, uint32_t *passed) {
   KMX_HIP(hipSetDevice(device_), kNoSuchDevice);
   carry_valid_ = false;
+  mask_prev_ = mask_cur_ = nullptr;
   if (N_ == 0) return kSuccess;
   if (strict_h2_) {
     KMX_HIP(launch_h2_yy_global(metric_, samples, N_, D_, K_, G_, centroids, drifts, gdrifts, assignments,
@@ -431,6 +433,7 @@
   KMX_HIP(hipSetDevice(device_), kNoSuchDevice);
   const bool carry_was_valid = carry_valid_;
   carry_valid_ = false;
+  mask_prev_ = mask_cur_ = nullptr;
   if (strict_h2_) {
     if (!h2_sq_) {
       int rc = alloc(&h2_sq_, 2 * (size_t)K_);
@@ -466,6 +469,15 @@
       (void)hipGetLastError();
       duo_ = nullptr;
       duo_on_ = false;
+    }
+    if (move_mask_on_ && !moved_mask_ && N_ != 0) {
+      const size_t words = ((size_t)N_ + 255) / 256 * 4;
+      if (alloc(&moved_mask_, words) != kSuccess ||
+          hipMemsetAsync(moved_mask_, 0xFF, words * sizeof(unsigned long long), stream_) != hipSuccess) {
+        (void)hipGetLastError();
+        moved_mask_ = nullptr;
+        move_mask_on_ = false;
+      }
     }
     panelhi_ = phi;
   }
@@ -592,6 +604,7 @@
         cy.n_list = counters_ + kCarryCursor;
       }
       if (listed) cy.row_list = carry_list_;
+      else if (steady) a.moved_mask = moved_mask_;
       static const bool trace = getenv("KMCUDA_AMD_CARRY_TRACE") != nullptr;
       if (trace) {
         uint32_t w[8] = {0};
@@ -611,6 +624,7 @@
               kRuntimeError);
       carry_valid_ = true;
     } else {
+      if (steady && cached && xcache_) a.moved_mask = moved_mask_;
       KMX_HIP(launch_lloyd_coarse(a, rows, half, cached ? xcache_ : nullptr, xmeta_, panelhi_, undecided_, und_thr_,
                                   duo_listed ? duo_ : nullptr, stream_),
               kRuntimeError);
@@ -638,6 +652,7 @@
     KMX_HIP(launch_lloyd_filter(a, stream_), kRuntimeError);
   }
   span_end();
+  if (a.moved_mask) { mask_prev_ = assignments_prev; mask_cur_ = assignments; }
   span_begin(1);
   if (settle_ && lloyd_settle_supported(a, centroids)) {
     if (rows_on_side) KMX_HIP(hipStreamWaitEvent(stream_, ev_rows_, 0), kRuntimeError);
@@ -766,7 +781,8 @@
   const MoveWeights mw{weights_, tail ? tail + K_ + 4 : wtail_, win_};
   KMX_HIP(launch_move_deltas(samples, N_, D_, K_, prev, cur, keys_tmp_, vals_tmp_, keys_sorted_, rows_sorted_,
                              offsets2_, sort_temp_, sort_temp_bytes_, bucket_rows_, bucket_cap_, delta, dcount, tail,
-                             counters_, move_blocks_, bucket_work_, &ms_, stream_, weights_ ? &mw : nullptr),
+                             counters_, move_blocks_, bucket_work_, &ms_, stream_, weights_ ? &mw : nullptr,
+                             (moved_mask_ && mask_prev_ == prev && mask_cur_ == cur) ? moved_mask_ : nullptr),
           kRuntimeError);
   span_end();
   return kSuccess;
diff --git a/kmcuda_amd/csrc/engine.hpp b/kmcuda_amd/csrc/engine.hpp
--- a/kmcuda_amd/csrc/engine.hpp
+++ b/kmcuda_amd/csrc/engine.hpp
@@ -144,6 +144,9 @@
   uint32_t *duo_ = nullptr;
   bool duo_on_ = true;
   bool duo_always_ = false;
+  bool move_mask_on_ = true;
+  unsigned long long *moved_mask_ = nullptr;
+  const uint32_t *mask_prev_ = nullptr, *mask_cur_ = nullptr;
   uint32_t coarse_mfma_ = 16;
   int filter_mode_ = 0;
   bool settle_ = true;
diff --git a/kmcuda_amd/csrc/filter_common.hpp b/kmcuda_amd/csrc/filter_common.hpp
--- a/kmcuda_amd/csrc/filter_common.hpp
+++ b/kmcuda_amd/csrc/filter_common.hpp
@@ -14,7 +14,9 @@
   }
   return false;
 }
-
+__device__ __forceinline__ void mark_moved(unsigned long long *__restrict__ mask, uint32_t s) {
+  if (mask) atomicOr(&mask[s >> 6], 1ull << (s & 63u));
+}
 
 struct ClampLimits {
   float hi, lo;
diff --git a/kmcuda_amd/csrc/kernels.hpp b/kmcuda_amd/csrc/kernels.hpp
--- a/kmcuda_amd/csrc/kernels.hpp
+++ b/kmcuda_amd/csrc/kernels.hpp
@@ -23,6 +23,7 @@
   uint32_t *pairs;
   uint32_t *counters;
   uint32_t coarse_mfma = 16;
+  unsigned long long *moved_mask = nullptr;
 };
 constexpr uint32_t kWaveRowGridMax = 1u << 20;
 inline uint32_t wave_row_grid(uint32_t n_rows) {
@@ -134,7 +135,8 @@
                               uint32_t *bucket_rows, uint32_t cap, double *delta, int32_t *dcount ,
                               double *tail ,
                               const uint32_t *counters, uint32_t *blockoff, uint32_t *bucket_work, MoveState *ms,
-                              hipStream_t st, const MoveWeights *mw = nullptr);
+                              hipStream_t st, const MoveWeights *mw = nullptr,
+                              const unsigned long long *moved_mask = nullptr );
 hipError_t launch_adjust_exact(int metric, const float *samples, uint32_t N, uint32_t D, uint32_t K,
                                const uint32_t *prev, const uint32_t *cur, uint32_t *keys_tmp, uint32_t *vals_tmp,
                                uint32_t *keys_sorted, uint32_t *rows_sorted, uint32_t *offsets2, void *temp,
diff --git a/kmcuda_amd/csrc/lloyd.hip b/kmcuda_amd/csrc/lloyd.hip
--- a/kmcuda_amd/csrc/lloyd.hip
+++ b/kmcuda_amd/csrc/lloyd.hip
@@ -334,7 +334,8 @@
 __global__ __launch_bounds__(128) void lloyd_pair_kernel(
     const float *__restrict__ samples, uint32_t D, const float *__restrict__ centroids,
     const float *__restrict__ csqr, const uint32_t *__restrict__ pairs, const uint32_t *__restrict__ npairs,
-    uint32_t *__restrict__ assignments, uint32_t *__restrict__ assignments_prev, uint32_t *__restrict__ counters) {
+    uint32_t *__restrict__ assignments, uint32_t *__restrict__ assignments_prev, uint32_t *__restrict__ counters,
+    unsigned long long *__restrict__ moved) {
   const uint32_t total = *npairs;
   for (uint32_t pi = blockIdx.x * blockDim.x + threadIdx.x; pi < total; pi += gridDim.x * blockDim.x) {
     const uint32_t s = pairs[3 * (size_t)pi], ia = pairs[3 * (size_t)pi + 1], ib = pairs[3 * (size_t)pi + 2];
@@ -408,7 +409,12 @@
     uint32_t nearest = 0xFFFFFFFFu;
     if (da < min_dist) { min_dist = da; nearest = lo; }
     if (db < min_dist) { min_dist = db; nearest = hi; }
-    if (nearest != 0xFFFFFFFFu && commit_row(s, nearest, assignments, assignments_prev)) atomicAdd(&counters[0], 1u);
+    if (nearest == 0xFFFFFFFFu) {
+      mark_moved(moved, s);
+    } else if (commit_row(s, nearest, assignments, assignments_prev)) {
+      atomicAdd(&counters[0], 1u);
+      mark_moved(moved, s);
+    }
   }
 }
 
@@ -417,7 +423,8 @@
     const float *__restrict__ samples, uint32_t N, uint32_t D, const float *__restrict__ ct,
     const float *__restrict__ csqr, uint32_t K, uint32_t Kt, const uint32_t *__restrict__ rows,
     const uint32_t *__restrict__ nrows, uint32_t *__restrict__ assignments,
-    uint32_t *__restrict__ assignments_prev, uint32_t *__restrict__ counters) {
+    uint32_t *__restrict__ assignments_prev, uint32_t *__restrict__ counters,
+    unsigned long long *__restrict__ moved) {
   constexpr int CH = 4;
   __shared__ float sh_dist[4];
   __shared__ uint32_t sh_idx[4];
@@ -513,7 +520,12 @@
       }
       if (nearest == 0xFFFFFFFFu && insane) nearest = K;
       if (nearest != 0xFFFFFFFFu) {
-        if (commit_row(s, nearest, assignments, assignments_prev)) atomicAdd(&counters[0], 1u);
+        if (commit_row(s, nearest, assignments, assignments_prev)) {
+          atomicAdd(&counters[0], 1u);
+          mark_moved(moved, s);
+        }
+      } else {
+        mark_moved(moved, s);
       }
     }
     __syncthreads();
@@ -532,7 +544,7 @@
     const float *__restrict__ ct, const float *__restrict__ csqr, uint32_t K, uint32_t Kt,
     const uint32_t *__restrict__ pairs, const uint32_t *__restrict__ npairs, const uint32_t *__restrict__ flagged,
     const uint32_t *__restrict__ nflagged, uint32_t *__restrict__ assignments,
-    uint32_t *__restrict__ assignments_prev, uint32_t *__restrict__ counters) {
+    uint32_t *__restrict__ assignments_prev, uint32_t *__restrict__ counters, unsigned long long *__restrict__ moved) {
   extern __shared__ __attribute__((aligned(16))) float settle_lds[];
   const int lane = threadIdx.x & 63, wave = threadIdx.x >> 6;
   if (blockIdx.x < kSettlePairBlocks) {
@@ -595,6 +607,7 @@
         if (dist < min_dist) { min_dist = dist; nearest = lo; }
         if (db < min_dist) { min_dist = db; nearest = hi; }
         if (nearest != 0xFFFFFFFFu) changed = commit_row(s, nearest, assignments, assignments_prev);
+        if (changed || nearest == 0xFFFFFFFFu) mark_moved(moved, s);
       }
       const unsigned long long cm = __ballot(changed);
       if (lane == 0 && cm) atomicAdd(&counters[0], (uint32_t)__popcll(cm));
@@ -693,7 +706,12 @@
       }
       if (nearest == 0xFFFFFFFFu && insane) nearest = K;
       if (nearest != 0xFFFFFFFFu) {
-        if (commit_row(s, nearest, assignments, assignments_prev)) atomicAdd(&counters[0], 1u);
+        if (commit_row(s, nearest, assignments, assignments_prev)) {
+          atomicAdd(&counters[0], 1u);
+          mark_moved(moved, s);
+        }
+      } else {
+        mark_moved(moved, s);
       }
     }
     __syncthreads();
@@ -714,11 +732,11 @@
   if (metric == 0)
     hipLaunchKernelGGL((lloyd_settle_kernel<0>), grid, dim3(256), kSettleLds, st, a.samples, a.N, a.D, centroids, a.ct,
                        a.csqr, a.K, a.Kt, a.pairs, a.counters + 3, a.flagged, a.counters + 1, a.assignments,
-                       a.assignments_prev, a.counters);
+                       a.assignments_prev, a.counters, a.moved_mask);
   else
     hipLaunchKernelGGL((lloyd_settle_kernel<1>), grid, dim3(256), kSettleLds, st, a.samples, a.N, a.D, centroids, a.ct,
                        a.csqr, a.K, a.Kt, a.pairs, a.counters + 3, a.flagged, a.counters + 1, a.assignments,
-                       a.assignments_prev, a.counters);
+                       a.assignments_prev, a.counters, a.moved_mask);
   return hipGetLastError();
 }
 
@@ -798,10 +816,10 @@
   if (grid == 0) return hipSuccess;
   if (metric == 0)
     hipLaunchKernelGGL((lloyd_pair_kernel<0>), dim3(grid), dim3(128), 0, st, a.samples, a.D, centroids, a.csqr,
-                       a.pairs, a.counters + 3, a.assignments, a.assignments_prev, a.counters);
+                       a.pairs, a.counters + 3, a.assignments, a.assignments_prev, a.counters, a.moved_mask);
   else
     hipLaunchKernelGGL((lloyd_pair_kernel<1>), dim3(grid), dim3(128), 0, st, a.samples, a.D, centroids, a.csqr,
-                       a.pairs, a.counters + 3, a.assignments, a.assignments_prev, a.counters);
+                       a.pairs, a.counters + 3, a.assignments, a.assignments_prev, a.counters, a.moved_mask);
   return hipGetLastError();
 }
 
@@ -810,10 +828,12 @@
   if (grid == 0) return hipSuccess;
   if (metric == 0)
     hipLaunchKernelGGL((lloyd_exact_kernel<0>), dim3(grid), dim3(256), 0, st, a.samples, a.N, a.D, a.ct, a.csqr,
-                       a.K, a.Kt, rows, nrows, a.assignments, a.assignments_prev, a.counters);
+                       a.K, a.Kt, rows, nrows, a.assignments, a.assignments_prev, a.counters,
+                       rows ? a.moved_mask : nullptr);
   else
     hipLaunchKernelGGL((lloyd_exact_kernel<1>), dim3(grid), dim3(256), 0, st, a.samples, a.N, a.D, a.ct, a.csqr,
-                       a.K, a.Kt, rows, nrows, a.assignments, a.assignments_prev, a.counters);
+                       a.K, a.Kt, rows, nrows, a.assignments, a.assignments_prev, a.counters,
+                       rows ? a.moved_mask : nullptr);
   return hipGetLastError();
 }
 
diff --git a/kmcuda_amd/csrc/lloyd_carry.hip b/kmcuda_amd/csrc/lloyd_carry.hip
--- a/kmcuda_amd/csrc/lloyd_carry.hip
+++ b/kmcuda_amd/csrc/lloyd_carry.hip
@@ -165,7 +165,8 @@
 #define KMX_CARRY_LAUNCH_S(H, F, C, MODE, SRC, SHAPE)                                                                       \
   hipLaunchKernelGGL((lloyd_coarse2_kernel<DP, H, F, C, NSET, MODE, SHAPE>), dim3(grid), dim3(256), lds_bytes, st, SRC,     \
                      xmeta, a.N, a.D, reinterpret_cast<const float *>(panelhi), a.bias, a.mu, a.K_pad, a.K, a.stats,        \
-                     a.eps, a.tie_slack, a.assignments, a.assignments_prev, undecided, und_thr, a.counters, cy, duo)
+                     a.eps, a.tie_slack, a.assignments, a.assignments_prev, undecided, und_thr, a.counters, cy, duo,        \
+                     a.moved_mask)
 #define KMX_CARRY_LAUNCH(H, F, C, MODE, SRC)                           \
   do {                                                                 \
     if (s16) KMX_CARRY_LAUNCH_S(H, F, C, MODE, SRC, (kS16 && !(MODE == 2 && DP >= 256)) ? 16 : 32); \
diff --git a/kmcuda_amd/csrc/lloyd_coarse.hpp b/kmcuda_amd/csrc/lloyd_coarse.hpp
--- a/kmcuda_amd/csrc/lloyd_coarse.hpp
+++ b/kmcuda_amd/csrc/lloyd_coarse.hpp
@@ -51,7 +51,8 @@
     const float *__restrict__ bias, const float *__restrict__ mu, uint32_t K_pad, uint32_t K,
     const uint32_t *__restrict__ stats, float eps, float tie_slack, uint32_t *__restrict__ assignments,
     uint32_t *__restrict__ assignments_prev, uint32_t *__restrict__ undecided, float *__restrict__ und_thr,
-    uint32_t *__restrict__ counters, CarryArgs cy, uint32_t *__restrict__ duo = nullptr) {
+    uint32_t *__restrict__ counters, CarryArgs cy, uint32_t *__restrict__ duo = nullptr,
+    unsigned long long *__restrict__ moved = nullptr ) {
   static_assert(CARRY == 0 || CARRY == 1 || CARRY == 2, "CARRY");
   static_assert(CARRY != 2 || !CACHED, "listed rows are gathered from the rows, not streamed from the row cache");
   static_assert(SHAPE == 32 || (SHAPE == 16 && NSET == 2 && DP >= 32), "16x16x32: two row sets, 32 features per k-step");
@@ -418,7 +419,7 @@
   };
   auto finish = [&](uint32_t s, bool mine, const float (&kq)[4], const uint32_t (&jq)[4], float others, float xn2,
                     float x0, float dx2, float xdm, float xab, bool &und, unsigned long long &um, float &cut, bool &is_duo,
-                    unsigned long long &dm, uint32_t &dc1, uint32_t &dc2, float &drest) {
+                    unsigned long long &dm, uint32_t &dc1, uint32_t &dc2, float &drest, unsigned long long &cm) {
     const bool insane = (x0 != x0);
     float k0 = kq[0], k1 = kq[1], k2 = kq[2], k3 = kq[3];
     uint32_t j0 = jq[0], j1 = jq[1], j2 = jq[2], j3 = jq[3];
@@ -479,7 +480,7 @@
     }
     cut = in_range ? v1 - thr : __builtin_nanf("");
     if (angular) cut = (lim.hi == lim.hi) ? fminf(cut, lim.hi) : __builtin_nanf("");
-    const unsigned long long cm = __ballot(changed);
+    cm = __ballot(changed);
     um = __ballot(und);
     dm = __ballot(is_duo);
     changed_count += (uint32_t)__popcll(cm);
@@ -513,6 +514,7 @@
     xdmb += __shfl_xor(xdmb, 32); xabb += __shfl_xor(xabb, 32);
   }
   float cuta, cutb = 0.f;
+  unsigned long long cma = 0, cmb = 0;
   float kq[4], oth;
   uint32_t jq[4];
   if constexpr (S16) {
@@ -520,13 +522,19 @@
     const bool mine = h ? liveB : liveA;
     sA = h ? sB : sA;
     finish(sA, mine, kq, jq, oth, h ? xn2b : xn2a, h ? x0b : x0a, h ? dx2b : dx2a, h ? xdmb : xdma, h ? xabb : xaba, unda, uma,
-           cuta, duoa, dma, d1a, d2a, dra);
+           cuta, duoa, dma, d1a, d2a, dra, cma);
   } else {
     quarters32(v1a, v2a, tba, kq, jq, oth);
-    finish(sA, h == 0 && liveA, kq, jq, oth, xn2a, x0a, dx2a, xdma, xaba, unda, uma, cuta, duoa, dma, d1a, d2a, dra);
+    finish(sA, h == 0 && liveA, kq, jq, oth, xn2a, x0a, dx2a, xdma, xaba, unda, uma, cuta, duoa, dma, d1a, d2a, dra, cma);
     if constexpr (TWO) {
       quarters32(v1b, v2b, tbb, kq, jq, oth);
-      finish(sB, h == 0 && liveB, kq, jq, oth, xn2b, x0b, dx2b, xdmb, xabb, undb, umb, cutb, duob, dmb, d1b, d2b, drb);
+      finish(sB, h == 0 && liveB, kq, jq, oth, xn2b, x0b, dx2b, xdmb, xabb, undb, umb, cutb, duob, dmb, d1b, d2b, drb, cmb);
+    }
+  }
+  if constexpr (CACHED) {
+    if (moved != nullptr && lane == 0) {
+      if constexpr (TWO) moved[(size_t)blk * 4u + wave] = S16 ? cma : (cma | (cmb << 32));
+      else reinterpret_cast<uint32_t *>(moved)[(size_t)blk * 4u + wave] = (uint32_t)cma;
     }
   }
   __shared__ uint32_t blk_und[WV], blk_changed[WV], blk_duo[WV], blk_base, blk_duo_base;
diff --git a/kmcuda_amd/csrc/lloyd_duo.hip b/kmcuda_amd/csrc/lloyd_duo.hip
--- a/kmcuda_amd/csrc/lloyd_duo.hip
+++ b/kmcuda_amd/csrc/lloyd_duo.hip
@@ -23,7 +23,7 @@
     const float *__restrict__ bias, const float *__restrict__ mu, const uint32_t *__restrict__ stats, float eps,
     float tie_slack, const uint4 *__restrict__ duo, uint32_t *__restrict__ assignments,
     uint32_t *__restrict__ assignments_prev, uint32_t *__restrict__ flagged, uint32_t *__restrict__ pairs,
-    uint32_t *__restrict__ counters, CarryArgs cy) {
+    uint32_t *__restrict__ counters, CarryArgs cy, unsigned long long *__restrict__ moved) {
   if (counters[kStopFlag] != 0u) return;
   constexpr int SLOTS = NI >= 8 ? 1 : 2;
   const uint32_t total = counters[kDuoCount];
@@ -154,6 +154,7 @@
         if (old_asg[k] != nearest) {
           assignments[s] = nearest;
           nchg++;
+          mark_moved(moved, s);
         }
       }
       if constexpr (BOUNDS) {
@@ -232,7 +233,7 @@
 #define KMX_DUO_LAUNCH(F, B, CY)                                                                                      \
   hipLaunchKernelGGL((lloyd_duo_kernel<NI, F, B>), grid, dim3(256), 0, st, a.samples, a.D, a.DP, a.K, a.cfil, a.bias,    \
                      a.mu, a.stats, a.eps, a.tie_slack, reinterpret_cast<const uint4 *>(duo), a.assignments,          \
-                     a.assignments_prev, a.flagged, a.pairs, a.counters, CY)
+                     a.assignments_prev, a.flagged, a.pairs, a.counters, CY, a.moved_mask)
   if (cy && cy->l3) {
     if (fast) KMX_DUO_LAUNCH(true, true, *cy); else KMX_DUO_LAUNCH(false, true, *cy);
   } else {
diff --git a/kmcuda_amd/csrc/lloyd_f16.hip b/kmcuda_amd/csrc/lloyd_f16.hip
--- a/kmcuda_amd/csrc/lloyd_f16.hip
+++ b/kmcuda_amd/csrc/lloyd_f16.hip
@@ -228,7 +228,8 @@
 #define KMX_CRS2_LAUNCH_S(H, F, C, SRC, SHAPE)                                                                            \
   hipLaunchKernelGGL((lloyd_coarse2_kernel<DP, H, F, C, NSET, 0, SHAPE>), dim3(grid), dim3(256), lds_bytes, st, SRC, xmeta, \
                      a.N, a.D, reinterpret_cast<const float *>(panelhi), a.bias, a.mu, a.K_pad, a.K, a.stats,             \
-                     a.eps, a.tie_slack, a.assignments, a.assignments_prev, undecided, und_thr, a.counters, CarryArgs(), duo)
+                     a.eps, a.tie_slack, a.assignments, a.assignments_prev, undecided, und_thr, a.counters, CarryArgs(), duo,  \
+                     a.moved_mask)
 #define KMX_CRS2_LAUNCH(H, F, C, SRC)                       \
   do {                                                      \
     if (s16) KMX_CRS2_LAUNCH_S(H, F, C, SRC, kS16 ? 16 : 32); \
diff --git a/kmcuda_amd/csrc/lloyd_refine.hpp b/kmcuda_amd/csrc/lloyd_refine.hpp
--- a/kmcuda_amd/csrc/lloyd_refine.hpp
+++ b/kmcuda_amd/csrc/lloyd_refine.hpp
@@ -11,7 +11,8 @@
     const float *__restrict__ mu, uint32_t K_pad, uint32_t K, const uint32_t *__restrict__ stats, float eps,
     float tie_slack, uint32_t *__restrict__ assignments, uint32_t *__restrict__ assignments_prev,
     const uint32_t *__restrict__ row_list, const float *__restrict__ thr_list, const uint32_t *__restrict__ n_list,
-    uint32_t *__restrict__ flagged, uint32_t *__restrict__ pairs, uint32_t *__restrict__ counters, CarryArgs cy) {
+    uint32_t *__restrict__ flagged, uint32_t *__restrict__ pairs, uint32_t *__restrict__ counters, CarryArgs cy,
+    unsigned long long *__restrict__ moved) {
   constexpr int NKH = DP / 2;
   constexpr int KS = NKH / 8;
   constexpr int ROWB = DP * 2;
@@ -310,6 +311,7 @@
     const bool pair_now = mine && two, flag_now = mine && !certain && !two;
     bool changed = false;
     if (mine && certain) changed = commit_row(s, insane ? K : i1, assignments, assignments_prev);
+    if (changed) mark_moved(moved, s);
     if constexpr (want_rest) {
       rest = fmaxf(rest, __shfl_xor(rest, 32));
       if (mine && cy.angular) {
@@ -404,7 +406,7 @@
   hipLaunchKernelGGL((lloyd_refine_kernel<DP, H, F, NSET, PAIRS>), dim3(grid), dim3(256), lds_bytes, st, rows, a.samples,  \
                      a.N, a.D, reinterpret_cast<const float *>(panelhi), a.cfil, a.bias, a.mu, a.K_pad, a.K,        \
                      a.stats, a.eps, a.tie_slack, a.assignments, a.assignments_prev, row_list, thr_list, n_list,    \
-                     a.flagged, a.pairs, a.counters, cy)
+                     a.flagged, a.pairs, a.counters, cy, a.moved_mask)
   if (half_rows) {
     if (fast) KMX_RFN_LAUNCH(true, true); else KMX_RFN_LAUNCH(true, false);
   } else {
diff --git a/kmcuda_amd/csrc/update.hip b/kmcuda_amd/csrc/update.hip
--- a/kmcuda_amd/csrc/update.hip
+++ b/kmcuda_amd/csrc/update.hip
@@ -630,12 +630,38 @@
   }
 }
 
+__global__ __launch_bounds__(256) void move_scatter_masked_kernel(const unsigned long long *__restrict__ mask,
+                                                                  uint32_t nwords, const uint32_t *__restrict__ prev,
+                                                                  const uint32_t *__restrict__ cur, uint32_t N,
+                                                                  uint32_t K, uint32_t *__restrict__ cursors,
+                                                                  uint32_t stride, uint32_t *__restrict__ bucket_rows,
+                                                                  uint32_t cap) {
+  const uint32_t w = blockIdx.x * 256u + threadIdx.x;
+  if (w >= nwords) return;
+  unsigned long long m = mask[w];
+  while (m) {
+    const uint32_t s = w * 64u + (uint32_t)__builtin_ctzll(m);
+    m &= m - 1ull;
+    uint32_t p, a;
+    bool ein, eout;
+    move_flags(prev, cur, s, N, K, p, a, ein, eout);
+    if (ein) {
+      const uint32_t at = atomicAdd(&cursors[(size_t)(2u * a) * stride], 1u);
+      if (at < cap) bucket_rows[(size_t)(2u * a) * cap + at] = s;
+    }
+    if (eout) {
+      const uint32_t at = atomicAdd(&cursors[(size_t)(2u * p + 1u) * stride], 1u);
+      if (at < cap) bucket_rows[(size_t)(2u * p + 1u) * cap + at] = s;
+    }
+  }
+}
+
 hipError_t launch_move_deltas(const float *samples, uint32_t N, uint32_t D, uint32_t K, const uint32_t *prev,
                               const uint32_t *cur, uint32_t *keys_tmp, uint32_t *vals_tmp, uint32_t *keys_sorted,
                               uint32_t *rows_sorted, uint32_t *offsets2, void *temp, size_t temp_bytes,
                               uint32_t *bucket_rows, uint32_t cap, double *delta, int32_t *dcount, double *tail,
                               const uint32_t *counters, uint32_t *blockoff, uint32_t *bucket_work, MoveState *ms,
-                              hipStream_t st, const MoveWeights *mw) {
+                              hipStream_t st, const MoveWeights *mw, const unsigned long long *moved_mask) {
   const uint32_t stride = move_bucket_stride(K);
   SumArgs a;
   a.samples = samples; a.N = N; a.D = D; a.K = K; a.prev = prev; a.cur = cur;
@@ -704,8 +730,14 @@
     launch_sums(false);
   } else {
     ms->n_direct++;
-    hipLaunchKernelGGL(move_scatter_kernel, dim3((N + 255) / 256), dim3(256), 0, st, prev, cur, N, K, bucket_work,
-                       stride, bucket_rows, cap);
+    if (moved_mask) {
+      const uint32_t nwords = (N + 63u) / 64u;
+      hipLaunchKernelGGL(move_scatter_masked_kernel, dim3((nwords + 255) / 256), dim3(256), 0, st, moved_mask, nwords,
+                         prev, cur, N, K, bucket_work, stride, bucket_rows, cap);
+    } else {
+      hipLaunchKernelGGL(move_scatter_kernel, dim3((N + 255) / 256), dim3(256), 0, st, prev, cur, N, K, bucket_work,
+                         stride, bucket_rows, cap);
+    }
     launch_sums(true);
     e = hipGetLastError();
     if (e != hipSuccess) return e;
```

Result: no change. 2.209 billion (median of 2 runs) (+0.1%).
